# guxm2021/SVT_SpeechBrain

Hardware: AMD Instinct MI355X
Metric: 10s@16kHz clips/sec encoder+CTC forward, wav2vec2-base, 1/2/4/8 MI355X (higher is better)
Workload: dtype bf16; 1 GPU; wav2vec2-base audio-only AMT forward (encoder + 20-way head + frame decode), 32 x 10 s @16 kHz mono clips per GPU; global_batch=32, per_gpu_batch=32, samples_per_clip=160000, frames_per_clip=499, parallelism=clips sharded over 1 rank(s), streams=2, inputs=resident in HBM

## Files before the change

include/svt_mi355.h:

```cpp
#ifndef SVT_MI355_H
#define SVT_MI355_H

#include <stddef.h>
#include <stdint.h>

#ifdef __cplusplus
extern "C" {
#endif

#define SVT_ABI_VERSION 1
#define SVT_MAX_CONV_LAYERS 8

typedef enum {
  SVT_OK = 0,
  SVT_ERR_INVALID = -1,
  SVT_ERR_KEY = -2,
  SVT_ERR_STATE = -3,
  SVT_ERR_WORKSPACE = -4,
  SVT_ERR_HIP = -5,
  SVT_ERR_NO_DEVICE = -6
} svt_status;

typedef enum { SVT_PREC_FP32 = 0, SVT_PREC_BF16 = 1, SVT_PREC_BF16X3 = 2, SVT_PREC_FP16X3 = 3 } svt_precision;
typedef enum { SVT_NORM_GROUP = 0, SVT_NORM_LAYER = 1 } svt_feat_norm;
// ... 90 lines not shown
                          float* out_dev, void* workspace_dev, size_t workspace_bytes, void* stream);
int svt_rca_backward(svt_rca* r, const float* dout_dev, int32_t batch, int32_t t_audio, float* const* grads_dev, void* workspace_dev,
                     size_t workspace_bytes, void* stream);

int svt_ctc_greedy(const float* probs_dev, int32_t batch, int32_t t, int32_t v, const float* rel_lens_dev,
                   int32_t blank, int32_t* tokens_dev, int32_t* out_lens_dev, int device, void* stream);

int64_t svt_fbank_workspace_bytes(int32_t batch, int64_t n_samples, int32_t n_fft, int32_t hop, int32_t n_mels);
int svt_fbank(const float* wav_dev, int32_t batch, int64_t n_samples, int32_t sample_rate, int32_t n_fft,
              int32_t win_length, int32_t hop_length, int32_t n_mels, float f_min, float f_max, float top_db,
              float* out_dev, void* workspace_dev, size_t workspace_bytes, int device, void* stream);

#define SVT_NOISE_AMP_WORKGROUPS 256
#define SVT_NOISE_MIX_MAX_WORKGROUPS 2048
int64_t svt_noise_mix_workspace_bytes(int64_t n_samples, int32_t n_snr);
int svt_noise_mix(const float* clean_dev, const float* noise_dev, int64_t n_samples, const float* snr_db_host, int32_t n_snr,
                  float* out_dev, int64_t ld_out, double* amps_out_dev, void* workspace_dev, int64_t workspace_bytes, int device,
                  void* stream);

#define SVT_RESAMPLE_LDS_BYTES 65536
#define SVT_RESAMPLE_TILE_OUTPUTS 1024
#define SVT_RESAMPLE_MAX_WORKGROUPS 768
int64_t svt_resample_output_samples(int64_t n_in, int32_t orig_freq, int32_t new_freq);
int svt_resample(const float* in_dev, int32_t rows, int64_t n_in, int64_t ld_in, const float* weights_dev, const int32_t* first_dev,
                 int32_t P, int32_t W, int32_t S, float* out_dev, int64_t n_out, int64_t ld_out, int32_t downmix, int device,
                 void* stream);

int svt_debug_gemm(int32_t precision, const void* a_dev, const void* w_dev, void* c_dev, const float* bias_dev,
                   const float* resid_dev, int32_t m, int32_t n, int32_t k, int32_t a_rpb, int64_t a_bstride,
                   int64_t a_rstride, int64_t ldw, int32_t act, int32_t out_f32, int device, void* stream);

int svt_debug_gemm_pairs(int32_t precision, const float* a_dev, int64_t a_elems, const float* w_dev, float* c_dev, const float* bias_dev,
                         int32_t m, int32_t n, int32_t k, int32_t a_rpb, int64_t a_bstride, int64_t a_rstride, int32_t act,
                         int32_t out_kind, int device, void* stream, int32_t time_iters, float* ms_out);

typedef struct svt_debug_gemm_desc {
  int32_t struct_size;
  const void* a;
  const void* w;
  void* c;
  const float* bias;
  const float* resid;
  int32_t m, n, k;
  int32_t a_rpb;
  int64_t a_bstride, a_rstride;
  int64_t ldw, ldc;
  int32_t nz, nz2;
  int64_t a_z1, a_z2, w_z1, w_z2, c_z1, c_z2, bias_z2;
  float alpha;
  int32_t act, out_f32;
} svt_debug_gemm_desc;
int svt_debug_gemm_batched(int32_t precision, const svt_debug_gemm_desc* d, int device, void* stream);

typedef struct svt_debug_layernorm_desc {
  int32_t struct_size;
  int32_t form;
  int32_t prec, x_is_f32;
  int64_t rows;
  int32_t D, gelu;
  float eps;
  int32_t pair_kind;
  const float* gamma;
  const float* beta;
  const void* x;
  void* yT;
  float* yF;
  const float* add;
  float* sumF;
  void* yP;
  const void* addP;
  const void* branch;
  const void* rh;
  const void* rl;
  const float* x32;
  void* yh;
  void* yl;
  const float* parts;
  const float* pbias;
  int64_t part_stride;
  int32_t nparts;
} svt_debug_layernorm_desc;
int svt_debug_layernorm(const svt_debug_layernorm_desc* d, int device, void* stream);

typedef struct svt_video svt_video;
int svt_video_create(int32_t embed_dim, int32_t precision, int device, svt_video** out);
void svt_video_destroy(svt_video* v);
int svt_video_load_param(svt_video* v, const char* key, const void* data_host, int dtype, const int64_t* shape, int ndim);
int svt_video_finalize(svt_video* v);
int64_t svt_video_workspace_bytes(const svt_video* v, int32_t batch, int32_t t, int32_t h, int32_t w);
int svt_video_keep_workspace(svt_video* v, int keep);
int svt_video_forward(svt_video* v, const float* video_dev, int32_t batch, int32_t t, int32_t h, int32_t w, float* out_dev,
                      void* workspace_dev, size_t workspace_bytes, void* stream);
int svt_video_forward_ex(svt_video* v, const float* video_dev, int32_t batch, int32_t t, int32_t h, int32_t w, float* out_dev, int64_t out_ld,
                         int32_t zero_left, void* workspace_dev, size_t workspace_bytes, void* stream);
typedef struct svt_video_transform { double sub0, div0, mean, std; int32_t crop_h, crop_w; } svt_video_transform;
int svt_video_forward_u8(svt_video* v, const uint8_t* roi_dev, int32_t batch, int32_t t, int32_t h_in, int32_t w_in,
                         const svt_video_transform* tf, float* out_dev, int64_t out_ld, int32_t zero_left, void* workspace_dev,
                         size_t workspace_bytes, void* stream);

int svt_deltas(const float* x_dev, int64_t ldx, int32_t batch, int32_t t, int32_t c, int32_t window_length, float* out_dev,
               int64_t ldo, int device, void* stream);
int svt_context_window(const float* x_dev, int32_t batch, int32_t t, int32_t c, int32_t left_frames, int32_t right_frames,
                       float* out_dev, int device, void* stream);

int svt_bce_loss(const float* logits_dev, int64_t batch, int64_t t_pred, const float* targets_dev, int64_t t_tgt,
                 const float* rel_len_dev, const float* pos_weight_dev, int32_t allowed_len_diff, int32_t reduction,
                 float* out_dev, void* workspace_dev, size_t workspace_bytes, int device, void* stream);
int svt_nll_loss(const float* log_probs_dev, int64_t batch, int64_t t_pred, int32_t n_class, const int64_t* targets_dev,
                 int64_t t_tgt, const float* rel_len_dev, float label_smoothing, int32_t allowed_len_diff,
                 int32_t reduction, float* out_dev, void* workspace_dev, size_t workspace_bytes, int device, void* stream);
int svt_softmax(const float* x_dev, int64_t rows, int32_t n, int32_t apply_log, float* y_dev, int device, void* stream);

int svt_amt_objective_grad(const float* logits_dev, int64_t batch, int64_t t_pred, int32_t n_out, int32_t pitch_octave_num,
                           const float* onset_targets_dev, const float* offset_targets_dev, const int64_t* octave_targets_dev,
                           const int64_t* class_targets_dev, int64_t t_tgt, const float* rel_len_dev, float onset_pos_weight,
                           int32_t allowed_len_diff, float label_smoothing, float* terms_dev, float* terms_host, float* dlogits_dev,
                           void* workspace_dev, size_t* workspace_bytes, int device, void* stream);
int svt_linear_backward(const float* x_dev, const float* dy_dev, int64_t rows, int32_t in_features, int32_t out_features,
                        float* dweight_dev, float* dbias_dev, void* workspace_dev, size_t* workspace_bytes, int device, void* stream);
int svt_linear_backward_data(const float* dy_dev, const float* weight_dev, int64_t rows, int32_t in_features, int32_t out_features,
                             float* dx_dev, int device, void* stream);
int svt_clip_adadelta_step(int32_t n_tensors, float* const* params_dev, float* const* grads_dev, float* const* square_avg_dev,
                           float* const* acc_delta_dev, const int64_t* numels, float lr, double rho, float eps, float weight_decay,
                           int32_t maximize, float max_norm, float* total_norm_dev, void* workspace_dev, size_t* workspace_bytes,
                           int device, void* stream);

int svt_debug_attention(int32_t precision, const void* q, const void* k, const void* v, void* o, int32_t batch, int32_t t,
                        int32_t heads, int32_t head_dim, int64_t ldq, int64_t ldkv, int64_t ldo, float scale, int device,
                        void* stream);
int svt_debug_attention_bias(const void* q, const void* k, const void* v, void* o, int32_t batch, int32_t t, int32_t heads, int64_t ldq,
                             int64_t ldkv, int64_t ldo, float scale, const float* gate_dev, const float* pos_bias_dev, int device,
                             void* stream);
int svt_debug_attention_scores(int32_t precision, const void* q, const void* k, const void* v, void* o, int32_t batch, int32_t t,
                               int32_t heads, int32_t head_dim, int64_t ldq, int64_t ldkv, int64_t ldo, float scale,
                               const float* gate_dev, const float* pos_bias_dev, int device, void* stream);
int svt_debug_rca_wgrad(int32_t precision, const float* dy0, int64_t ldy0, const void* x0, const float* dy1, int64_t ldy1, const void* x1,
                        int64_t rows, int32_t n_out, int32_t n_in, float* dw, float* db, void* workspace_dev, size_t* workspace_bytes,
                        int device, void* stream);
int svt_debug_rca_attn_bwd(int32_t precision, const void* qkv, const void* qc, const void* o_self, const void* o_cross,
                           const float* dblend, float alpha, int32_t batch, int32_t t, int32_t heads, int32_t head_dim, float* dqkv,
                           float* dqc, void* workspace_dev, size_t* workspace_bytes, int device, void* stream);
int svt_debug_set(int key, int value);

int svt_prof_enable(int on);
int svt_prof_reset(void);
int svt_prof_read(int kind, int64_t* launches, double* total_ms, double* total_flops, double* total_bytes);
int svt_debug_clock(int64_t* out_dev, int device, void* stream);
int svt_debug_alloc(void** out, size_t bytes, int device);
int svt_debug_encoder_layout(const svt_encoder* e, int32_t batch, int64_t n_samples, int64_t* offsets, int n);
int svt_debug_free(void* p, int device);

#ifdef __cplusplus
}
#endif
#endif
```

svt_speechbrain_amd/_lib.py:

```python
from __future__ import annotations

import ctypes as C
import os
from typing import Optional

_HERE = os.path.dirname(os.path.abspath(__file__))
LIB_PATH = os.environ.get("SVT_LIB_PATH") or os.path.join(_HERE, "libsvt_mi355.so")
MAX_CONV = 8


class SvtError(RuntimeError):
    pass


class EncoderConfigC(C.Structure):
    _fields_ = [
        ("struct_size", C.c_int32),
        ("hidden_size", C.c_int32),
        ("num_layers", C.c_int32),
        ("num_heads", C.c_int32),
        ("intermediate_size", C.c_int32),
        ("num_conv_layers", C.c_int32),
        ("conv_dim", C.c_int32 * MAX_CONV),
        ("conv_kernel", C.c_int32 * MAX_CONV),
# ... 23 lines not shown
    _fields_ = [
        ("struct_size", C.c_int32),
        ("a", C.c_void_p), ("w", C.c_void_p), ("c", C.c_void_p), ("bias", C.c_void_p), ("resid", C.c_void_p),
        ("m", C.c_int32), ("n", C.c_int32), ("k", C.c_int32),
        ("a_rpb", C.c_int32),
        ("a_bstride", C.c_int64), ("a_rstride", C.c_int64),
        ("ldw", C.c_int64), ("ldc", C.c_int64),
        ("nz", C.c_int32), ("nz2", C.c_int32),
        ("a_z1", C.c_int64), ("a_z2", C.c_int64), ("w_z1", C.c_int64), ("w_z2", C.c_int64), ("c_z1", C.c_int64), ("c_z2", C.c_int64),
        ("bias_z2", C.c_int64),
        ("alpha", C.c_float),
        ("act", C.c_int32), ("out_f32", C.c_int32),
    ]


class LayerNormDescC(C.Structure):
    _fields_ = [
        ("struct_size", C.c_int32),
        ("form", C.c_int32),
        ("prec", C.c_int32), ("x_is_f32", C.c_int32),
        ("rows", C.c_int64),
        ("D", C.c_int32), ("gelu", C.c_int32),
        ("eps", C.c_float),
        ("pair_kind", C.c_int32),
        ("gamma", C.c_void_p), ("beta", C.c_void_p),
        ("x", C.c_void_p), ("yT", C.c_void_p), ("yF", C.c_void_p), ("add", C.c_void_p), ("sumF", C.c_void_p), ("yP", C.c_void_p), ("addP", C.c_void_p),
        ("branch", C.c_void_p), ("rh", C.c_void_p), ("rl", C.c_void_p), ("x32", C.c_void_p), ("yh", C.c_void_p), ("yl", C.c_void_p),
        ("parts", C.c_void_p), ("pbias", C.c_void_p),
        ("part_stride", C.c_int64),
        ("nparts", C.c_int32),
    ]


class FrameC(C.Structure):
    _fields_ = [("p_on", C.c_float), ("p_off", C.c_float), ("octave", C.c_int32), ("pitch_class", C.c_int32)]


_P = C.c_void_p
_I64P = C.POINTER(C.c_int64)
NORM_REDUCE_FN = C.CFUNCTYPE(C.c_int, C.c_void_p, C.c_int32, C.c_void_p, C.c_void_p)

SYMBOLS = {
    "svt_last_error": (C.c_char_p, []),
    "svt_abi_version": (C.c_int, []),
    "svt_device_count": (C.c_int, []),
    "svt_encoder_create": (C.c_int, [C.POINTER(EncoderConfigC), C.c_int, C.POINTER(_P)]),
    "svt_encoder_destroy": (None, [_P]),
    "svt_encoder_load_param": (C.c_int, [_P, C.c_char_p, _P, C.c_int, _I64P, C.c_int]),
    "svt_encoder_finalize": (C.c_int, [_P]),
    "svt_encoder_get_param": (C.c_int, [_P, C.c_char_p, _P, C.c_int64]),
    "svt_encoder_num_frames": (C.c_int64, [_P, C.c_int64]),
    "svt_encoder_workspace_bytes": (C.c_int64, [_P, C.c_int32, C.c_int64]),
    "svt_encoder_forward": (C.c_int, [_P, _P, C.c_int32, C.c_int64, _P, _P, C.c_size_t, _P]),
    "svt_encoder_forward_ex": (C.c_int, [_P, _P, C.c_int32, C.c_int64, _P, _P, C.c_size_t, _P, C.c_int32]),
    "svt_encoder_forward_head": (C.c_int, [_P, _P, _P, C.c_int32, C.c_int64, _P, _P, C.c_int32, C.c_int32, _P, C.c_size_t, _P, C.c_int32]),
    "svt_linear_create": (C.c_int, [C.c_int32, C.c_int32, C.c_int, C.c_int, C.POINTER(_P)]),
    "svt_linear_destroy": (None, [_P]),
    "svt_linear_load": (C.c_int, [_P, _P, _P]),
    "svt_linear_forward": (C.c_int, [_P, _P, C.c_int64, _P, _P]),
    "svt_decode_frames": (C.c_int, [_P, C.c_int64, C.c_int32, C.c_int32, C.c_int32, _P, C.c_int, _P]),
    "svt_rca_create": (C.c_int, [C.c_int32, C.c_int32, C.c_int32, C.c_float, C.c_int32, C.c_int32, C.c_int, C.POINTER(_P)]),
    "svt_rca_destroy": (None, [_P]),
    "svt_rca_load_param": (C.c_int, [_P, C.c_char_p, _P, C.c_int, _I64P, C.c_int]),
    "svt_rca_finalize": (C.c_int, [_P]),
    "svt_rca_workspace_bytes": (C.c_int64, [_P, C.c_int32, C.c_int32]),
    "svt_rca_forward": (C.c_int, [_P, _P, C.c_int32, _P, C.c_int32, C.c_int32, _P, _P, C.c_size_t, _P]),
    "svt_rca_refresh_params": (C.c_int, [_P, C.POINTER(_P), C.c_int32, _P]),
    "svt_rca_train_workspace_bytes": (C.c_int64, [_P, C.c_int32, C.c_int32]),
    "svt_rca_forward_train": (C.c_int, [_P, _P, C.c_int32, _P, C.c_int32, C.c_int32, _P, _P, C.c_size_t, _P]),
    "svt_rca_backward": (C.c_int, [_P, _P, C.c_int32, C.c_int32, C.POINTER(_P), _P, C.c_size_t, _P]),
    "svt_ctc_greedy": (C.c_int, [_P, C.c_int32, C.c_int32, C.c_int32, _P, C.c_int32, _P, _P, C.c_int, _P]),
    "svt_fbank_workspace_bytes": (C.c_int64, [C.c_int32, C.c_int64, C.c_int32, C.c_int32, C.c_int32]),
    "svt_fbank": (C.c_int, [_P, C.c_int32, C.c_int64, C.c_int32, C.c_int32, C.c_int32, C.c_int32, C.c_int32,
                            C.c_float, C.c_float, C.c_float, _P, _P, C.c_size_t, C.c_int, _P]),
    "svt_noise_mix_workspace_bytes": (C.c_int64, [C.c_int64, C.c_int32]),
    "svt_noise_mix": (C.c_int, [_P, _P, C.c_int64, C.POINTER(C.c_float), C.c_int32, _P, C.c_int64, _P, _P, C.c_int64, C.c_int, _P]),
    "svt_resample_output_samples": (C.c_int64, [C.c_int64, C.c_int32, C.c_int32]),
    "svt_resample": (C.c_int, [_P, C.c_int32, C.c_int64, C.c_int64, _P, _P, C.c_int32, C.c_int32, C.c_int32, _P, C.c_int64, C.c_int64,
                               C.c_int32, C.c_int, _P]),
    "svt_debug_gemm": (C.c_int, [C.c_int32, _P, _P, _P, _P, _P, C.c_int32, C.c_int32, C.c_int32, C.c_int32, C.c_int64,
                                 C.c_int64, C.c_int64, C.c_int32, C.c_int32, C.c_int, _P]),
    "svt_debug_gemm_batched": (C.c_int, [C.c_int32, C.POINTER(GemmDescC), C.c_int, _P]),
    "svt_debug_layernorm": (C.c_int, [C.POINTER(LayerNormDescC), C.c_int, _P]),
    "svt_debug_attention_scores": (C.c_int, [C.c_int32, _P, _P, _P, _P, C.c_int32, C.c_int32, C.c_int32, C.c_int32, C.c_int64, C.c_int64,
                                             C.c_int64, C.c_float, _P, _P, C.c_int, _P]),
    "svt_debug_gemm_pairs": (C.c_int, [C.c_int32, _P, C.c_int64, _P, _P, _P, C.c_int32, C.c_int32, C.c_int32, C.c_int32, C.c_int64,
                                       C.c_int64, C.c_int32, C.c_int32, C.c_int, _P, C.c_int32, C.POINTER(C.c_float)]),
    "svt_video_create": (C.c_int, [C.c_int32, C.c_int32, C.c_int, C.POINTER(C.c_void_p)]),
    "svt_video_destroy": (None, [C.c_void_p]),
    "svt_video_load_param": (C.c_int, [C.c_void_p, C.c_char_p, C.c_void_p, C.c_int, C.POINTER(C.c_int64), C.c_int]),
    "svt_video_finalize": (C.c_int, [C.c_void_p]),
    "svt_video_keep_workspace": (C.c_int, [C.c_void_p, C.c_int]),
    "svt_video_workspace_bytes": (C.c_int64, [C.c_void_p, C.c_int32, C.c_int32, C.c_int32, C.c_int32]),
    "svt_video_forward": (C.c_int, [C.c_void_p, C.c_void_p, C.c_int32, C.c_int32, C.c_int32, C.c_int32, C.c_void_p, C.c_void_p,
                                    C.c_size_t, C.c_void_p]),
    "svt_video_forward_ex": (C.c_int, [C.c_void_p, C.c_void_p, C.c_int32, C.c_int32, C.c_int32, C.c_int32, C.c_void_p, C.c_int64, C.c_int32,
                                       C.c_void_p, C.c_size_t, C.c_void_p]),
    "svt_video_forward_u8": (C.c_int, [C.c_void_p, C.c_void_p, C.c_int32, C.c_int32, C.c_int32, C.c_int32, C.POINTER(VideoTransformC),
                                       C.c_void_p, C.c_int64, C.c_int32, C.c_void_p, C.c_size_t, C.c_void_p]),
    "svt_deltas": (C.c_int, [C.c_void_p, C.c_int64, C.c_int32, C.c_int32, C.c_int32, C.c_int32, C.c_void_p, C.c_int64, C.c_int, C.c_void_p]),
    "svt_context_window": (C.c_int, [C.c_void_p, C.c_int32, C.c_int32, C.c_int32, C.c_int32, C.c_int32, C.c_void_p, C.c_int, C.c_void_p]),
    "svt_bce_loss": (C.c_int, [C.c_void_p, C.c_int64, C.c_int64, C.c_void_p, C.c_int64, C.c_void_p, C.c_void_p, C.c_int32,
                               C.c_int32, C.c_void_p, C.c_void_p, C.c_size_t, C.c_int, C.c_void_p]),
    "svt_nll_loss": (C.c_int, [C.c_void_p, C.c_int64, C.c_int64, C.c_int32, C.c_void_p, C.c_int64, C.c_void_p, C.c_float,
                               C.c_int32, C.c_int32, C.c_void_p, C.c_void_p, C.c_size_t, C.c_int, C.c_void_p]),
    "svt_softmax": (C.c_int, [C.c_void_p, C.c_int64, C.c_int32, C.c_int32, C.c_void_p, C.c_int, C.c_void_p]),
    "svt_amt_objective_grad": (C.c_int, [_P, C.c_int64, C.c_int64, C.c_int32, C.c_int32, _P, _P, _P, _P, C.c_int64, _P, C.c_float,
                                         C.c_int32, C.c_float, _P, C.POINTER(C.c_float), _P, _P, C.POINTER(C.c_size_t), C.c_int, _P]),
    "svt_linear_backward": (C.c_int, [_P, _P, C.c_int64, C.c_int32, C.c_int32, _P, _P, _P, C.POINTER(C.c_size_t), C.c_int, _P]),
    "svt_linear_backward_data": (C.c_int, [_P, _P, C.c_int64, C.c_int32, C.c_int32, _P, C.c_int, _P]),
    "svt_clip_adadelta_step": (C.c_int, [C.c_int32, C.POINTER(_P), C.POINTER(_P), C.POINTER(_P), C.POINTER(_P), _I64P, C.c_float,
                                         C.c_double, C.c_float, C.c_float, C.c_int32, C.c_float, _P, _P, C.POINTER(C.c_size_t), C.c_int,
                                         _P]),
    "svt_debug_attention": (C.c_int, [C.c_int32, C.c_void_p, C.c_void_p, C.c_void_p, C.c_void_p, C.c_int32, C.c_int32,
                                      C.c_int32, C.c_int32, C.c_int64, C.c_int64, C.c_int64, C.c_float, C.c_int, C.c_void_p]),
    "svt_debug_attention_bias": (C.c_int, [C.c_void_p, C.c_void_p, C.c_void_p, C.c_void_p, C.c_int32, C.c_int32, C.c_int32, C.c_int64,
                                           C.c_int64, C.c_int64, C.c_float, C.c_void_p, C.c_void_p, C.c_int, C.c_void_p]),
    "svt_debug_rca_wgrad": (C.c_int, [C.c_int32, _P, C.c_int64, _P, _P, C.c_int64, _P, C.c_int64, C.c_int32, C.c_int32, _P, _P, _P,
                                      C.POINTER(C.c_size_t), C.c_int, _P]),
    "svt_debug_rca_attn_bwd": (C.c_int, [C.c_int32, _P, _P, _P, _P, _P, C.c_float, C.c_int32, C.c_int32, C.c_int32, C.c_int32, _P, _P,
                                         _P, C.POINTER(C.c_size_t), C.c_int, _P]),
    "svt_debug_set": (C.c_int, [C.c_int, C.c_int]),
    "svt_debug_clock": (C.c_int, [C.c_void_p, C.c_int, C.c_void_p]),
    "svt_debug_encoder_layout": (C.c_int, [C.c_void_p, C.c_int32, C.c_int64, C.POINTER(C.c_int64), C.c_int]),
    "svt_operand_type": (C.c_int, []),
    "svt_encoder_set_norm_reduce": (C.c_int, [_P, C.c_void_p, C.c_void_p, C.c_int64]),
    "svt_frames_to_notes": (C.c_int, [C.c_void_p, C.c_int32, C.c_int64, C.c_void_p, C.c_float, C.c_float, C.c_double, C.c_int32, C.c_int32,
                                      C.c_void_p, C.c_void_p, C.c_void_p, C.c_void_p, C.c_void_p, C.c_int64, C.c_void_p]),
    "svt_debug_alloc": (C.c_int, [C.POINTER(C.c_void_p), C.c_size_t, C.c_int]),
    "svt_debug_free": (C.c_int, [C.c_void_p, C.c_int]),
    "svt_prof_enable": (C.c_int, [C.c_int]),
    "svt_prof_reset": (C.c_int, []),
    "svt_prof_read": (C.c_int, [C.c_int, _I64P, C.POINTER(C.c_double), C.POINTER(C.c_double), C.POINTER(C.c_double)]),
}

_lib: Optional[C.CDLL] = None
_libs: dict = {}


def load(variant: str = None) -> C.CDLL:
    global _lib
    key = variant or ""
    if key in _libs:
        return _libs[key]
    if not variant and os.environ.get("SVT_LIB_SUFFIX"):
        variant_path = LIB_PATH.replace("libsvt_mi355.so", f"libsvt_mi355_{os.environ['SVT_LIB_SUFFIX']}.so")
        if not os.path.exists(variant_path):
            raise SvtError(f"SVT_LIB_SUFFIX: {variant_path} not found")
        globals()["LIB_PATH"] = variant_path
    root, ext = os.path.splitext(LIB_PATH)
    path = LIB_PATH if not variant else f"{root}_{variant}{ext}"
    if not os.path.exists(path):
        raise SvtError(
            f"{path} not found: build it with `python -c 'import __graft_entry__ as g; g.build()'` "
            "(or `make -C svt_speechbrain_amd/csrc`). The MI355X path has no CPU fallback.")
    lib = C.CDLL(path)
    for name, (res, args) in SYMBOLS.items():
        fn = getattr(lib, name)
        fn.restype = res
        fn.argtypes = args
    if lib.svt_abi_version() != 1:
        raise SvtError(f"{os.path.basename(path)} ABI version mismatch")
    if lib.svt_operand_type() != (1 if variant == "f16" else 0):
        raise SvtError(f"{os.path.basename(path)} was built for another operand type")
    _libs[key] = lib
    if not variant:
# ... 35 lines not shown
```

svt_speechbrain_amd/csrc/api.hip:

```cpp
#include "../../include/svt_mi355.h"
#include "api.h"
#include "common.h"
#include "host.h"

#include <atomic>
#include <cmath>
#include <cstring>
#include <map>
#include <mutex>
#include <string>
#include <vector>

namespace svt {

int hip_fail(hipError_t e, const char* what, const char* file, int line) {
  set_error(std::string("HIP error ") + hipGetErrorName(e) + " (" + hipGetErrorString(e) + ") at " + file + ":" +
          std::to_string(line) + " in " + what);
  return SVT_ERR_HIP;
}

struct ProfState {
  bool on = false;
  int every = 1;
  unsigned tick = 0;
// ... 253 lines not shown
int svt_operand_type(void) {
#ifdef SVT_OPERAND_F16
  return 1;
#else
  return 0;
#endif
}
int svt_device_count(void) {
  int n = 0;
  if (hipGetDeviceCount(&n) != hipSuccess) return 0;
  int ok = 0;
  for (int i = 0; i < n; ++i) {
    hipDeviceProp_t prop;
    if (hipGetDeviceProperties(&prop, i) == hipSuccess && std::string(prop.gcnArchName).find("gfx950") != std::string::npos) ++ok;
  }
  return ok;
}

int svt_debug_gemm(int32_t precision, const void* a, const void* w, void* c, const float* bias, const float* resid,
                   int32_t m, int32_t n, int32_t k, int32_t a_rpb, int64_t a_bstride, int64_t a_rstride, int64_t ldw,
                   int32_t act, int32_t out_f32, int device, void* stream) {
  if (!a || !w || !c) { set_error("svt_debug_gemm: null argument"); return SVT_ERR_INVALID; }
  SVT_HIP(hipSetDevice(device));
  GemmArgs g;
  g.A = a; g.W = w; g.C = c; g.bias = bias; g.resid = resid;
  g.M = m; g.N = n; g.K = k; g.a_rpb = a_rpb; g.a_bstride = a_bstride; g.a_rstride = a_rstride;
  g.ldw = ldw; g.ldc = n; g.act = act; g.out_f32 = out_f32;
  static const void* s_kept = nullptr;
  const bool split = precision >= 2 && ldw == k && k % 32 == 0;
  if (split && !(g_debug_keep_split && s_kept == w)) {
    if (split_weights_register(w, n, k, precision, (hipStream_t)stream)) return SVT_ERR_HIP;
    s_kept = w;
  }
  const int rc = launch_gemm(precision, g, (hipStream_t)stream);
  if (split && !g_debug_keep_split) {
    SVT_HIP(hipStreamSynchronize((hipStream_t)stream));
    split_weights_forget(w);
    s_kept = nullptr;
  }
  return rc ? SVT_ERR_INVALID : SVT_OK;
}

int svt_debug_gemm_batched(int32_t precision, const svt_debug_gemm_desc* d, int device, void* stream) {
  if (!d || d->struct_size != (int32_t)sizeof(svt_debug_gemm_desc)) { set_error("svt_debug_gemm_batched: struct_size"); return SVT_ERR_INVALID; }
  if (!d->a || !d->w || !d->c) { set_error("svt_debug_gemm_batched: null argument"); return SVT_ERR_INVALID; }
  if (!valid_precision(precision)) { set_error("svt_debug_gemm_batched: precision"); return SVT_ERR_INVALID; }
  if (d->nz < 1 || d->nz2 < 1 || d->k < 1) { set_error("svt_debug_gemm_batched: nz, nz2 and k must be positive"); return SVT_ERR_INVALID; }
  SVT_HIP(hipSetDevice(device));
  GemmArgs g;
  g.A = d->a; g.W = d->w; g.C = d->c; g.bias = d->bias; g.resid = d->resid;
  g.M = d->m; g.N = d->n; g.K = d->k; g.a_rpb = d->a_rpb; g.a_bstride = d->a_bstride; g.a_rstride = d->a_rstride;
  g.ldw = d->ldw; g.ldc = d->ldc;
  g.nz = d->nz; g.nz2 = d->nz2;
  g.a_z1 = d->a_z1; g.a_z2 = d->a_z2; g.w_z1 = d->w_z1; g.w_z2 = d->w_z2; g.c_z1 = d->c_z1; g.c_z2 = d->c_z2; g.bias_z2 = d->bias_z2;
  g.alpha = d->alpha; g.act = d->act; g.out_f32 = d->out_f32;
  const bool split = precision >= 2 && d->ldw == d->k && d->k % 32 == 0 && d->w_z1 >= 0 && d->w_z2 >= 0;
  if (split) {
    const size_t last_z_row = d->nz > 1 ? ((size_t)(d->nz / d->nz2 - 1) * d->w_z1 + (size_t)(d->nz2 - 1) * d->w_z2) / (size_t)d->k : 0;
    if (split_weights_register(d->w, (long)last_z_row + d->n, d->k, precision, (hipStream_t)stream)) return SVT_ERR_HIP;
  }
  const int rc = launch_gemm(precision, g, (hipStream_t)stream);
  if (split) {
    SVT_HIP(hipStreamSynchronize((hipStream_t)stream));
    split_weights_forget(d->w);
  }
  return rc ? SVT_ERR_INVALID : SVT_OK;
}

int svt_debug_layernorm(const svt_debug_layernorm_desc* d, int device, void* stream) {
  auto refuse = [](const char* why) { set_error(std::string("svt_debug_layernorm: ") + why); return SVT_ERR_INVALID; };
  auto aligned = [](unsigned mask, auto... p) { return !((... | (uintptr_t)p) & mask); };
  if (!d || d->struct_size != (int32_t)sizeof(svt_debug_layernorm_desc)) return refuse("struct_size");
  if (d->form < 0 || d->form > 2) return refuse("form is 0, 1 or 2");
  if (d->rows < 1 || d->D < 1) return refuse("rows and D must be positive");
  if (!d->gamma || !d->beta) return refuse("null gamma / beta");
  const bool hilo_width = d->D == 512 || d->D == 768 || d->D == 1024;
  if (d->form == 0) {
    if (!d->x) return refuse("null x");
    if (!d->prec && !d->x_is_f32) return refuse("a 16-bit x needs prec 1");
    if (!aligned(15, d->gamma, d->beta, d->x, d->yT, d->yF, d->add, d->sumF) || !aligned(127, d->yP, d->addP))
      return refuse("every buffer 16-byte aligned, yP / addP 128-byte aligned");
  } else {
    if (!hilo_width) return refuse("the (hi, lo) forms need D in {512, 768, 1024}");
    if (!d->yh || !d->yl) return refuse("null yh / yl");
    if (!aligned(15, d->gamma, d->beta, d->branch, d->rh, d->rl, d->x32, d->yh, d->yl, d->yF, d->parts, d->pbias))
      return refuse("every buffer 16-byte aligned");
    if (d->form == 1 && !(d->x32 ? !d->rh && !d->rl : d->rh && d->rl)) return refuse("form 1 takes exactly one of x32 and (rh, rl)");
    if (d->form == 2 && (!d->rh || !d->rl)) return refuse("form 2 needs rh and rl");
    if (d->form == 2 && (d->nparts < 1 || (d->nparts > 1 && d->part_stride < d->rows * d->D))) return refuse("nparts >= 1, parts rows * D elements apart or more");
  }
  if (int r = check_device(device)) return r;
  SVT_HIP(hipSetDevice(device));
  hipStream_t s = (hipStream_t)stream;
  int rc;
  if (d->form == 0) {
    LnArgs a;
    a.prec = d->prec; a.x = d->x; a.x_is_f32 = d->x_is_f32; a.rows = d->rows; a.D = d->D; a.gamma = d->gamma; a.beta = d->beta;
    a.eps = d->eps; a.gelu = d->gelu; a.yT = d->yT; a.yF = d->yF; a.add = d->add; a.sumF = d->sumF; a.yP = d->yP;
    a.pair_kind = d->pair_kind; a.addP = d->addP;
    rc = launch_layernorm(a, s);
  } else if (d->form == 1) {
    rc = launch_layernorm_hilo((const bf16_t*)d->branch, (const bf16_t*)d->rh, (const bf16_t*)d->rl, d->x32, d->rows, d->D, d->gamma,
                               d->beta, d->eps, (bf16_t*)d->yh, (bf16_t*)d->yl, d->yF, s);
  } else {
    rc = launch_layernorm_hilo_parts(d->parts, d->nparts, (long)d->part_stride, d->pbias, (const bf16_t*)d->rh, (const bf16_t*)d->rl,
                                     d->rows, d->D, d->gamma, d->beta, d->eps, (bf16_t*)d->yh, (bf16_t*)d->yl, d->yF, s);
  }
  return rc ? SVT_ERR_INVALID : SVT_OK;
}

int svt_debug_gemm_pairs(int32_t precision, const float* a, int64_t a_elems, const float* w, float* c, const float* bias, int32_t m,
                         int32_t n, int32_t k, int32_t a_rpb, int64_t a_bstride, int64_t a_rstride, int32_t act, int32_t out_kind,
                         int device, void* stream, int32_t time_iters, float* ms_out) {
  if (!a || !w || !c) { set_error("svt_debug_gemm_pairs: null argument"); return SVT_ERR_INVALID; }
  if ((precision != SVT_PREC_BF16X3 && precision != SVT_PREC_FP16X3) || !valid_precision(precision)) {
    set_error("svt_debug_gemm_pairs: split-operand precisions only (they live in libsvt_mi355.so, not in the IEEE-half build)"); return SVT_ERR_INVALID; }
  if (out_kind < 0 || out_kind > 2 || a_elems % 32 || ((int64_t)m * n) % 32) { set_error("svt_debug_gemm_pairs: out_kind / sizes"); return SVT_ERR_INVALID; }
  SVT_HIP(hipSetDevice(device));
  hipStream_t s = (hipStream_t)stream;
  void *ap = nullptr, *cp = nullptr;
  hipEvent_t e0 = nullptr, e1 = nullptr;
  static std::mutex s_mu;
  static const void* s_kept = nullptr;
  std::lock_guard<std::mutex> lock(s_mu);
  bool registered = false;
  auto hip_ok = [](hipError_t e, const char* what) -> int {
    if (e == hipSuccess) return 0;
    set_error(std::string(what) + ": " + hipGetErrorString(e));
    return 1;
  };
  int rc = dev_alloc(&ap, (size_t)a_elems * 4);
  if (!rc && out_kind) rc = dev_alloc(&cp, (size_t)m * n * 4);
  if (!rc) rc = launch_f32_to_pairs(precision, a, ap, a_elems, s);
  if (!rc && !(g_debug_keep_split && s_kept == w)) {
    rc = split_weights_register(w, n, k, precision, s);
    if (!rc) { s_kept = w; registered = true; }
  } else if (!rc) {
    registered = true;
  }
  if (!rc) {
    GemmArgs g;
    g.A = ap; g.W = w; g.C = out_kind == 1 ? cp : (void*)c; g.bias = bias;
    g.M = m; g.N = n; g.K = k; g.a_rpb = a_rpb; g.a_bstride = a_bstride; g.a_rstride = a_rstride;
    g.ldw = k; g.ldc = n; g.act = act; g.out_f32 = 1; g.a_pairs = 1; g.c_pairs = out_kind == 1;
    if (out_kind == 2) { g.planes = (unsigned short*)cp; g.plane_stride = (long)m * n; }
    rc = launch_gemm(precision, g, s);
    if (!rc && time_iters > 0 && ms_out) {
      rc = hip_ok(hipEventCreate(&e0), "hipEventCreate") || hip_ok(hipEventCreate(&e1), "hipEventCreate") ||
           hip_ok(hipEventRecord(e0, s), "hipEventRecord");
      for (int i = 0; i < time_iters && !rc; ++i) rc = launch_gemm(precision, g, s);
      float ms = 0.f;
      if (!rc) rc = hip_ok(hipEventRecord(e1, s), "hipEventRecord") || hip_ok(hipEventSynchronize(e1), "hipEventSynchronize") ||
                    hip_ok(hipEventElapsedTime(&ms, e0, e1), "hipEventElapsedTime");
      if (!rc) *ms_out = ms / (float)time_iters;
    }
  }
  if (!rc && out_kind == 1) rc = launch_pairs_to_f32(precision, cp, nullptr, c, (int64_t)m * n, s);
  if (!rc && out_kind == 2) rc = launch_pairs_to_f32(precision, cp, (const unsigned short*)cp + (size_t)m * n, c, (int64_t)m * n, s);
  (void)hipStreamSynchronize(s);
  if (e0) (void)hipEventDestroy(e0);
  if (e1) (void)hipEventDestroy(e1);
  if (registered && !g_debug_keep_split) { split_weights_forget(w); s_kept = nullptr; }
  if (ap) dev_free(ap);
  if (cp) dev_free(cp);
  return rc ? SVT_ERR_INVALID : SVT_OK;
}

int svt_debug_attention(int32_t precision, const void* q, const void* k, const void* v, void* o, int32_t batch, int32_t t,
                        int32_t heads, int32_t head_dim, int64_t ldq, int64_t ldkv, int64_t ldo, float scale, int device,
                        void* stream) {
  if (!q || !k || !v || !o) { set_error("svt_debug_attention: null argument"); return SVT_ERR_INVALID; }
  if (!(precision >= 1 && precision <= 3) || !(head_dim == 64 || head_dim == 128)) {
    set_error("svt_debug_attention: only the fused kernels (bf16, or the split-operand modes on fp32 inputs; head_dim 64 / 128) are exposed"); return SVT_ERR_INVALID; }
  if (int r = check_device(device)) return r;
  SVT_HIP(hipSetDevice(device));
  if (precision >= 2) {
    const long D = (long)heads * head_dim, rows = (long)batch * t;
    if ((const float*)k != (const float*)q + D || (const float*)v != (const float*)q + 2 * D || ldq != 3 * D || ldkv != 3 * D) {
      set_error("svt_debug_attention: the split-operand kernel is exposed for a packed q|k|v projection"); return SVT_ERR_INVALID; }
    void* planes = nullptr;
    if (int r = dev_alloc(&planes, (size_t)rows * 3 * D * 4)) return r;
    AttnBufs ab{};
    ab.pl_qkv = planes;
    const int rc = attention_scores_path(0, q, ldq, k, v, ldkv, batch, t, heads, head_dim, scale, ab, false, o, ldo, (hipStream_t)stream,
                                         nullptr, nullptr, precision);
    (void)hipStreamSynchronize((hipStream_t)stream);
    dev_free(planes);
    return rc ? SVT_ERR_INVALID : SVT_OK;
  }
  if (launch_flash_attention(q, ldq, (long)t * ldq, k, v, ldkv, (long)t * ldkv, o, ldo, (long)t * ldo, batch, t, heads,
                             head_dim, scale, (hipStream_t)stream)) return SVT_ERR_INVALID;
// ... 13 lines not shown
}

int svt_debug_attention_scores(int32_t precision, const void* q, const void* k, const void* v, void* o, int32_t batch, int32_t t,
                               int32_t heads, int32_t head_dim, int64_t ldq, int64_t ldkv, int64_t ldo, float scale,
                               const float* gate_dev, const float* pos_bias_dev, int device, void* stream) {
  if (!q || !k || !v || !o) { set_error("svt_debug_attention_scores: null argument"); return SVT_ERR_INVALID; }
  if (!valid_precision(precision)) { set_error("svt_debug_attention_scores: precision"); return SVT_ERR_INVALID; }
  if (batch < 1 || t < 1 || heads < 1 || head_dim < 1) { set_error("svt_debug_attention_scores: batch, t, heads and head_dim must be positive"); return SVT_ERR_INVALID; }
  if (!gate_dev != !pos_bias_dev) { set_error("svt_debug_attention_scores: gate and pos_bias come together"); return SVT_ERR_INVALID; }
  if (use_flash(precision, head_dim, gate_dev != nullptr, t)) {
    set_error("svt_debug_attention_scores: this geometry runs the fused kernel (svt_debug_attention / svt_debug_attention_bias)"); return SVT_ERR_INVALID; }
  if (int r = check_device(device)) return r;
  SVT_HIP(hipSetDevice(device));
  hipStream_t s = (hipStream_t)stream;
  const int prec = storage_prec(precision);
  const int Tp = attn_tp(precision, head_dim, t, gate_dev != nullptr);
  const size_t bh = (size_t)batch * heads;
  const size_t bytes[3] = {bh * t * Tp * 4, bh * t * Tp * esize(prec), bh * head_dim * Tp * esize(prec)};
  void* buf[3] = {nullptr, nullptr, nullptr};
  int rc = 0;
  for (int i = 0; i < 3 && !rc; ++i) {
    rc = dev_alloc(&buf[i], bytes[i]);
    if (!rc && hipMemsetAsync(buf[i], 0xFF, bytes[i], s) != hipSuccess) { set_error("svt_debug_attention_scores: hipMemsetAsync"); rc = SVT_ERR_HIP; }
  }
  if (!rc) {
    AttnBufs ab{};
    ab.S = (float*)buf[0]; ab.P = buf[1]; ab.Vt = buf[2];
    rc = attention_scores_path(prec, q, ldq, k, v, ldkv, batch, t, heads, head_dim, scale, ab, false, o, ldo, s, gate_dev, pos_bias_dev,
                               precision) ? SVT_ERR_INVALID : SVT_OK;
  }
  (void)hipStreamSynchronize(s);
  for (int i = 0; i < 3; ++i) dev_free(buf[i]);
  return rc;
}

int svt_debug_set(int key, int value) {
  if (key == 0) g_gemm_dbg = value;
  else if (key == 1) g_gemm_force_bm = value;
  else if (key == 2) g_gemm_ring = value;
  else if (key == 3) g_gemm_variant = value;
  else if (key == 5) {  }
  else if (key == 6) g_gemm_skinny = value;
  else if (key == 7) g_gemm_skinny_max_tiles = value;
  else if (key == 8) g_flash_wide = value;
  else if (key == 9) g_conv_ln_bf16 = value;
  else if (key == 10) {  }
  else if (key == 11) g_gemm_x3 = value;
  else if (key == 12) g_debug_keep_split = value;
  else if (key == 13) g_guard_alloc = value;
  else if (key == 15) g_stamp_ends = value;
  else if (key == 16) {  }
  else if (key == 18) {  }
  else if (key == 19) g_x3_pairs = value;
  else if (key == 20) g_ln_two_rows = value;
  else if (key == 21) {
    if (value != 0 && value != 3) { set_error("svt_debug_set(21): the attention A/B arms are retired"); return SVT_ERR_INVALID; }
  }
  else if (key == 22) g_conv0_mfma = value;
  else if (key == 23) g_conv3x3_c64 = value;
  else if (key == 24) return g_conv3x3_c64_launches;
  else if (key == 25) g_conv3x3_c64_form = value;
  else if (key == 26) g_stem_pool_fused = value;
  else if (key == 27) g_conv_down_fused = value;
  else if (key == 28) {
    if (value != 0) { set_error("svt_debug_set(28): the two-slot schedule is retired"); return SVT_ERR_INVALID; }
  }
  else if (key == 29) g_gemm_p1w = value;
  else if (key == 30) {
#ifndef SVT_DIAG
    if (value != 0) { set_error("svt_debug_set(30): gemm_p1x_kernel is built by `make DIAG=1` only"); return SVT_ERR_INVALID; }
#endif
    g_gemm_p1x = value;
  }
  else if (key == 31) return g_dev_frees.load(std::memory_order_relaxed);
  else if (key == 32) return set_ticket_fenced(value);
  else if (key == 33) g_gemm_skinny_small_tiles = value;
  else if (key == 34) g_gemm_walk = value;
  else if (key == 35) g_conv_kperm = value;
  else if (key == 36) g_ffn2_ksplit = value;
  else if (key == 37) { if (value < 8 || value > 256 || value % 8) { set_error("svt_debug_set(37): 8 .. 256, a multiple of 8"); return SVT_ERR_INVALID; } g_gemm_persist_wgs = value; }
  else if (key == 38) return g_flash_kernel_id;
  else if (key == 39) return g_gemm_kernel_id;
  else if (key == 40) return g_ln_kernel_id;
  else { set_error("svt_debug_set: unknown key"); return SVT_ERR_INVALID; }
  return SVT_OK;
}

int svt_debug_alloc(void** out, size_t bytes, int device) {
  if (!out) { set_error("svt_debug_alloc: null argument"); return SVT_ERR_INVALID; }
  if (int r = check_device(device)) return r;
  SVT_HIP(hipSetDevice(device));
  return dev_alloc(out, bytes);
}
int svt_debug_free(void* p, int device) {
  if (int r = check_device(device)) return r;
  SVT_HIP(hipSetDevice(device));
  dev_free(p);
  return SVT_OK;
}

int svt_debug_clock(int64_t* out_dev, int device, void* stream) {
  if (!out_dev) { set_error("svt_debug_clock: null argument"); return SVT_ERR_INVALID; }
  SVT_HIP(hipSetDevice(device));
  return launch_clock_stamp((long long*)out_dev, (hipStream_t)stream) ? SVT_ERR_HIP : SVT_OK;
}

int svt_prof_enable(int on) { g_prof.on = on != 0; g_prof.every = on > 1 ? on : 1; g_prof.tick = 0; return SVT_OK; }
int svt_prof_reset(void) {
  g_prof.used = 0;
  for (int k = 0; k < 3; ++k) g_prof.flops[k] = g_prof.bytes[k] = 0;
  return SVT_OK;
}
int svt_prof_read(int kind, int64_t* launches, double* total_ms, double* total_flops, double* total_bytes) {
  if (kind < 0 || kind > 2) { set_error("svt_prof_read: kind must be 0..2"); return SVT_ERR_INVALID; }
  double ms = 0;
  int64_t n = 0;
  for (size_t i = 0; i < g_prof.used; ++i) {
    if (g_prof.kind[i] != kind) continue;
    SVT_HIP(hipEventSynchronize(g_prof.ev[i].second));
    float t = 0;
    SVT_HIP(hipEventElapsedTime(&t, g_prof.ev[i].first, g_prof.ev[i].second));
    ms += t;
    ++n;
  }
  if (launches) *launches = n;
  if (total_ms) *total_ms = ms;
  if (total_flops) *total_flops = g_prof.flops[kind];
  if (total_bytes) *total_bytes = g_prof.bytes[kind];
  return SVT_OK;
}

}
```

svt_speechbrain_amd/csrc/api_encoder.hip:

```cpp
#include "../../include/svt_mi355.h"
#include "api.h"
#include "common.h"
#include "host.h"

#include <cmath>
#include <cstring>
#include <string>
#include <vector>

using namespace svt;

int svt::g_conv_ln_bf16 = 1;

struct ConvLayerW {
  DevBuf w;
  DevBuf w_kperm;
  DevBuf bias;
  DevBuf gamma, beta;
};
struct EncLayerW {
  DevBuf wqkv, bqkv, wo, bo, ln1g, ln1b, w1, b1, w2, b2, ln2g, ln2b;
  DevBuf g_wab, g_bab, g_const;
};

struct svt_encoder {
  svt_encoder_config cfg;
  int device = 0;
  bool finalized = false;
  bool uploaded = false;
  ParamMap params;
  std::vector<ConvLayerW> conv;
  DevBuf fp_g, fp_b, proj_w, proj_b, pos_w, pos_b, enc_g, enc_b;
  DevBuf pos_bn_sc, pos_bn_sh;
  DevBuf pos_wP, pos_bP;
  int pos_P = 0;
  std::vector<DevBuf> pos_ws, pos_bs;
  DevBuf rel_embed;
  DevBuf ones, zeros;
  std::vector<EncLayerW> layers;
  svt_norm_reduce_fn reduce_fn = nullptr;
  void* reduce_user = nullptr;
  int64_t reduce_global_clips = 0;
};

static bool reduced_mode(const svt_encoder_config& c) { return c.precision != SVT_PREC_FP32; }

static int64_t conv_frames(const svt_encoder_config& c, int64_t n_samples, int64_t* frames = nullptr) {
  int64_t t = n_samples;
  for (int i = 0; i < c.num_conv_layers; ++i) {
    if (t < c.conv_kernel[i]) return 0;
    t = (t - c.conv_kernel[i]) / c.conv_stride[i] + 1;
    if (frames) frames[i] = t;
  }
  return t;
}

namespace {

int finalize_conv_stack(svt_encoder* e) {
  const svt_encoder_config& c = e->cfg;
  const ParamMap& P = e->params;
  if ((int)e->conv.size() != c.num_conv_layers) { e->conv.clear(); e->conv.resize(c.num_conv_layers); }
  int cin = 1;
  for (int i = 0; i < c.num_conv_layers; ++i) {
    const std::string pre = "feature_extractor.conv_layers." + std::to_string(i) + ".";
    const int co = c.conv_dim[i], k = c.conv_kernel[i];
    const Param* p = nullptr;
    if (int r = need(P, pre + "conv.weight", {co, cin, k}, &p)) return r;
    ConvLayerW& L = e->conv[i];
    if (i == 0) {
      if (int r = upload_f32(L.w, p->v.data(), p->v.size())) return r;
    } else {
      const std::vector<float> wt = tap_major(p->v.data(), co, cin, k);
      if (int r = upload_weight(c.precision, L.w, wt.data(), (size_t)co, (size_t)k * cin)) return r;
      if (storage_prec(c.precision) && k == 3 && cin % 64 == 0 && c.conv_stride[i] == 2) {
        const std::vector<float> wp = tap_minor_slabs(wt.data(), co, cin, k);
        if (int r = upload_weight(c.precision, L.w_kperm, wp.data(), (size_t)co, (size_t)k * cin)) return r;
      } else L.w_kperm.release();
    }
    if (c.conv_bias)
      if (int r = upload_vec(P, pre + "conv.bias", co, &L.bias)) return r;
    if (c.feat_extract_norm == SVT_NORM_LAYER || i == 0) {
      if (int r = upload_vec(P, pre + "layer_norm.weight", co, &L.gamma)) return r;
      if (int r = upload_vec(P, pre + "layer_norm.bias", co, &L.beta)) return r;
    }
    cin = co;
  }
  return SVT_OK;
}

int finalize_projection(svt_encoder* e) {
  const svt_encoder_config& c = e->cfg;
  const ParamMap& P = e->params;
  const int cin = c.conv_dim[c.num_conv_layers > 0 ? c.num_conv_layers - 1 : 0];
  if (c.feat_proj_layer_norm) {
// ... 300 lines not shown
  }
  if (c.num_conv_layers == 0) max_act = rows * c.conv_dim[0] * es;
  w.act[0] = cv.take(max_act);
  w.act[1] = cv.take(max_act);
  w.convF = c.feat_extract_norm == SVT_NORM_LAYER ? (float*)cv.take(max_f) : nullptr;
  w.xln = cv.take(rows * p.C * es);
  w.hF = (float*)cv.take(rows * D * 4);
  w.preF = (float*)cv.take(rows * D * 4);
  w.xb = cv.take(rows * D * es);
  w.xF = p.reduced ? (float*)cv.take(rows * D * 4) : (float*)w.xb;
  w.xlo = p.sp ? cv.take(rows * D * 2) : nullptr;
  w.posg = cv.take(B * p.pos_Tp * D * es);
  w.posy = p.Pf ? cv.take(B * p.pos_Tq * p.Pf * D * es) : nullptr;
  w.qkv = cv.take(rows * 3 * D * es);
  const bool scores = !(p.flash || p.planes);
  w.ab.S = scores ? (float*)cv.take(B * H * T * p.attn_Tp * 4) : nullptr;
  w.ab.P = scores ? cv.take(B * H * T * p.attn_Tp * es) : nullptr;
  w.ab.Vt = cv.take(B * H * p.dh * p.attn_Tp * es);
  w.ab.pl_qkv = p.planes ? cv.take(rows * 3 * D * 4) : nullptr;
  w.attn_o = cv.take(rows * D * es);
  w.ffn = cv.take(rows * p.F * es);
  w.gate = p.rel ? (float*)cv.take(B * H * T * 4) : nullptr;
  w.relpb = p.rel ? (float*)cv.take(H * (2 * T - 1) * 4) : nullptr;
  w.dots = (float*)cv.take(rows * 32 * 4);
  w.ksplit = p.ksplit_ws ? (float*)cv.take((size_t)4 * rows * D * 4) : nullptr;
  w.total = cv.off;
  return w;
}

struct TailSpec {
  float* feats = nullptr;
  const svt_linear* head = nullptr;
  float* logits = nullptr;
  svt_frame* frames = nullptr;
  int n_oct = 0, n_cls = 0;
};

}

extern "C" {

int svt_debug_encoder_layout(const svt_encoder* e, int32_t batch, int64_t n_samples, int64_t* offsets, int n) {
  if (!e || batch < 1 || !offsets || n < 1) { set_error("svt_debug_encoder_layout: bad argument"); return SVT_ERR_INVALID; }
  EncPlan p;
  if (!plan_encoder(e, batch, n_samples, &p)) { set_error("waveform shorter than the receptive field"); return SVT_ERR_INVALID; }
  char* const fake = (char*)(uintptr_t)(1ull << 40);
  const EncWs w = carve_encoder(e, p, fake);
  const void* r[24] = {w.mom, w.coef, w.c0tab, w.act[0], w.act[1], w.convF, w.xln, w.hF, w.preF, w.xb, w.xF, w.xlo, w.posg, w.posy, w.qkv,
                       w.ab.S, w.ab.P, w.ab.Vt, w.ab.pl_qkv, w.attn_o, w.ffn, w.gate, w.relpb, w.dots};
  int k = 0;
  for (; k < 24 && k < n; ++k) offsets[k] = r[k] == nullptr ? -1 : (int64_t)((const char*)r[k] - fake);
  if (k < n) offsets[k++] = (int64_t)w.total;
  return k;
}

int64_t svt_encoder_workspace_bytes(const svt_encoder* e, int32_t batch, int64_t n_samples) {
  if (!e || batch < 1) { set_error("workspace_bytes: bad argument"); return -1; }
  EncPlan p;
  if (!plan_encoder(e, batch, n_samples, &p)) { set_error("waveform shorter than the receptive field"); return -1; }
  return (int64_t)carve_encoder(e, p, nullptr).total;
}

}

namespace {

struct ReduceCtx { const svt_encoder* e; double* mom; hipStream_t s; };
int reduce_now(void* a) {
  ReduceCtx* rc = (ReduceCtx*)a;
  if (rc->e->reduce_fn(rc->mom, 2, (void*)rc->s, rc->e->reduce_user)) { set_error("encoder_forward: the norm-reduce callback reported an error"); return SVT_ERR_INVALID; }
  return 0;
}

struct EncRun {
  const svt_encoder* e;
  const svt_encoder_config& c;
  const EncPlan& p;
  EncWs w;
  hipStream_t s;
  int cpg = 0, groups = 1;
  double* wav_mom = nullptr;
  double* out_mom = nullptr;
  double* win_mom = nullptr;
  int64_t n_wav = 0;
  bool global_norm = false;
  ReduceCtx rctx{nullptr, nullptr, nullptr};
  int pk_front = 0, pk_enc = 0;
  float* resid = nullptr;
};

LnArgs ln_f32(const EncRun& x, const void* in, int64_t rows, int D, const DevBuf& gamma, const DevBuf& beta, float eps) {
  LnArgs a;
  a.prec = x.p.sp; a.x = in; a.rows = rows; a.D = D; a.gamma = gamma.as<float>(); a.beta = beta.as<float>(); a.eps = eps;
  return a;
}

int check_norm_groups(EncRun& x, int32_t clips_per_norm_group) {
  const svt_encoder_config& c = x.c;
  x.cpg = clips_per_norm_group > 0 ? clips_per_norm_group : x.p.B;
  if (x.p.B % x.cpg) { set_error("encoder_forward: batch must be a multiple of clips_per_norm_group"); return SVT_ERR_INVALID; }
  x.groups = x.p.B / x.cpg;
  if (x.groups > 1 && c.num_conv_layers > 0 && (x.p.L & 3)) {
    set_error("encoder_forward: norm groups need a waveform length that is a multiple of 4 samples");
    return SVT_ERR_INVALID;
  }
  if (x.groups > 1 && c.num_conv_layers == 0 && c.normalize_wav) {
    set_error("encoder_forward: features-in mode has no input norm to group");
    return SVT_ERR_INVALID;
  }
  return SVT_OK;
}

int input_statistics(EncRun& x, const float* wav) {
  const svt_encoder_config& c = x.c;
  const EncWs& w = x.w;
  const size_t B = (size_t)x.p.B;
  if (launch_zero_bytes(w.mom, w.mom_zero, x.s)) return SVT_ERR_HIP;
  x.wav_mom = c.normalize_wav ? w.mom : nullptr;
  x.out_mom = w.mom + 2 * B;
  x.win_mom = w.mom + 4 * B;
  x.n_wav = (int64_t)x.cpg * x.p.L;
  if (c.normalize_wav)
    if (int r = launch_moments(wav, x.n_wav, x.wav_mom, (char*)w.mom + w.mom_scr[0], x.p.B, x.s, x.groups)) return r;
  x.rctx = ReduceCtx{x.e, nullptr, x.s};
  x.global_norm = x.e->reduce_fn != nullptr;
  if (x.global_norm) {
    if (x.groups != 1) { set_error("encoder_forward: the cross-rank norm reduction applies to whole-batch norms (clips_per_norm_group = 0)"); return SVT_ERR_INVALID; }
    if (x.e->reduce_global_clips < x.p.B) { set_error("encoder_forward: global_clips of the norm reduction is smaller than this batch"); return SVT_ERR_INVALID; }
    if (c.normalize_wav) {
      x.rctx.mom = x.wav_mom;
      if (int r = reduce_now(&x.rctx)) return r;
      x.n_wav = x.e->reduce_global_clips * x.p.L;
    }
  }
  return SVT_OK;
}

bool x3q_fits(const void* A, int M, int N, int K, int a_rpb, long a_bstride, long a_rstride, const void* Wp, int c_pairs, long ldc) {
  GemmArgs g;
  g.A = A; g.W = Wp; g.C = const_cast<void*>(A); g.M = M; g.N = N; g.K = K; g.a_rpb = a_rpb; g.a_bstride = a_bstride; g.a_rstride = a_rstride;
  g.ldw = K; g.ldc = ldc; g.a_pairs = 1; g.c_pairs = c_pairs;
  return gemm_x3q_eligible(g);
}

void choose_pair_rows(EncRun& x) {
  const svt_encoder_config& c = x.c;
  const EncPlan& p = x.p;
  const EncWs& w = x.w;
  const svt_encoder* e = x.e;
  const int B = p.B, D = p.D, F = p.F, rows = (int)p.rows;
  const int pk_mode = (p.gp >= 2 && g_x3_pairs && g_gemm_x3) ? p.gp : 0;
  bool front = pk_mode != 0 && c.num_conv_layers >= 2 && c.conv_dim[0] % 32 == 0 && c.conv_dim[0] <= 512 && c.conv_stride[0] <= 5;
  for (int i = 1; i < c.num_conv_layers && front; ++i) {
    const int cin = c.conv_dim[i - 1], co = c.conv_dim[i], k = c.conv_kernel[i], st = c.conv_stride[i];
    const int64_t ti = p.frames[i - 1], to = p.frames[i];
    front = (int64_t)B * to <= 2147483647LL &&
            x3q_fits(w.act[0], (int)((int64_t)B * to), co, k * cin, (int)to, ti * cin, (long)st * cin, e->conv[i].w.p, 1, co) &&
            (c.feat_extract_norm != SVT_NORM_LAYER || co == 512 || co == 768 || co == 1024);
  }
  front = front && x3q_fits(w.xln, rows, D, p.C, rows, 0, p.C, e->proj_w.p, 0, D) &&
          (!c.feat_proj_layer_norm || p.C == 512 || p.C == 768 || p.C == 1024);
  x.pk_front = front ? pk_mode : 0;
  const bool enc = pk_mode != 0 && p.planes && c.num_layers > 0 && (D == 512 || D == 768 || D == 1024) && p.dh % 32 == 0 &&
                   x3q_fits(w.xb, rows, 3 * D, D, rows, 0, D, e->layers[0].wqkv.p, 0, 3 * D) &&
                   x3q_fits(w.attn_o, rows, D, D, rows, 0, D, e->layers[0].wo.p, 0, D) &&
                   x3q_fits(w.xb, rows, F, D, rows, 0, D, e->layers[0].w1.p, 1, F) &&
                   x3q_fits(w.ffn, rows, D, F, rows, 0, F, e->layers[0].w2.p, 0, D);
  x.pk_enc = enc ? pk_mode : 0;
  x.resid = (!p.sp && !x.pk_enc) ? (float*)w.xb : w.xF;
}

int conv_layer0(const EncRun& x, const float* wav) {
  const svt_encoder_config& c = x.c;
  const EncWs& w = x.w;
  const int B = x.p.B, k = c.conv_kernel[0], st = c.conv_stride[0], C0 = c.conv_dim[0], prec = x.p.sp;
  const int64_t L = x.p.L, t1 = x.p.t1;
  const ConvLayerW& c0 = x.e->conv[0];
  const float* b0 = c.conv_bias ? c0.bias.as<float>() : nullptr;
  const bool mfma = conv0_mfma_ok(prec, x.pk_front, k, st, C0) && w.c0tab;
  if (c.feat_extract_norm == SVT_NORM_GROUP) {
    if (int r = launch_conv0_window_moments(wav, B, L, k, st, t1, x.win_mom, (char*)w.mom + w.mom_scr[2], x.s)) return r;
    if (int r = launch_conv0_group_coef(x.wav_mom, x.n_wav, x.win_mom, B, t1, C0, k, c0.w.as<float>(), b0, c0.gamma.as<float>(),
                                        c0.beta.as<float>(), 1e-5f, 1e-5f, w.coef, x.s, x.cpg)) return r;
    if (mfma) return launch_conv0_mfma_group(wav, B, L, st, t1, w.coef, w.c0tab, w.act[0], x.s, x.pk_front);
    return launch_conv0_group_apply(prec, wav, B, L, k, st, t1, C0, w.coef, w.act[0], x.s, x.pk_front);
  }
  if (mfma)
    return launch_conv0_mfma_layer(wav, B, L, st, t1, x.wav_mom, x.n_wav, 1e-5f, c0.w.as<float>(), b0, c0.gamma.as<float>(),
                                   c0.beta.as<float>(), 1e-5f, w.c0tab, w.act[0], x.s, x.cpg, x.pk_front);
  return launch_conv0_layer(prec, wav, B, L, k, st, t1, C0, x.wav_mom, x.n_wav, 1e-5f, c0.w.as<float>(), b0, c0.gamma.as<float>(),
                            c0.beta.as<float>(), 1e-5f, w.act[0], x.s, x.cpg, x.pk_front);
}

int conv_stack(const EncRun& x, int* cur_out) {
  const svt_encoder_config& c = x.c;
  const EncWs& w = x.w;
  const int prec = x.p.sp, gp = x.p.gp, pk = x.pk_front;
  const bool layer_norm = c.feat_extract_norm == SVT_NORM_LAYER;
  int cur = 0;
  for (int i = 1; i < c.num_conv_layers; ++i) {
    const int cin = c.conv_dim[i - 1], co = c.conv_dim[i], k = c.conv_kernel[i], st = c.conv_stride[i];
    const int64_t tin = x.p.frames[i - 1], tout = x.p.frames[i], rows = (int64_t)x.p.B * tout;
    const ConvLayerW& Lw = x.e->conv[i];
    void* const out = w.act[cur ^ 1];
    if (rows > 2147483647LL) { set_error("encoder_forward: batch*frames exceeds 2^31"); return SVT_ERR_INVALID; }
    GemmArgs g;
    g.A = w.act[cur]; g.W = Lw.w.p;
    g.M = (int)rows; g.N = co; g.K = k * cin;
    g.a_rpb = (int)tout; g.a_bstride = tin * cin; g.a_rstride = (long)st * cin;
    g.ldw = g.K; g.ldc = co;
    if (Lw.w_kperm.p) { g.W_kperm = Lw.w_kperm.p; g.kperm_taps = k; g.kperm_cin = cin; }
    g.bias = c.conv_bias ? Lw.bias.as<float>() : nullptr;
    g.a_pairs = pk ? 1 : 0;
    const bool pairs_out = pk && !(i + 1 == c.num_conv_layers && c.feat_proj_layer_norm);
    LnArgs n = ln_f32(x, w.convF, rows, co, Lw.gamma, Lw.beta, 1e-5f);
    n.gelu = 1;
    if (pk && layer_norm) {
      g.C = w.convF; g.out_f32 = 1; g.act = ACT_NONE;
      if (int r = launch_gemm(gp, g, x.s)) return r;
      (pairs_out ? n.yP : n.yT) = out; n.pair_kind = pk;
      if (int r = launch_layernorm(n, x.s)) return r;
    } else if (pk) {
      g.C = out; g.act = ACT_GELU; g.out_f32 = 1; g.c_pairs = pairs_out ? 1 : 0;
      if (int r = launch_gemm(gp, g, x.s)) return r;
    } else if (layer_norm && prec && co == 512 && g_conv_ln_bf16) {
      g.C = out; g.out_f32 = 0; g.act = ACT_NONE;
      if (int r = launch_gemm(gp, g, x.s)) return r;
      n.x = out; n.x_is_f32 = 0; n.yT = out;
      if (int r = launch_layernorm(n, x.s)) return r;
    } else if (layer_norm) {
      g.C = w.convF; g.out_f32 = 1; g.act = ACT_NONE;
      if (int r = launch_gemm(gp, g, x.s)) return r;
      n.yT = out;
      if (int r = launch_layernorm(n, x.s)) return r;
    } else {
      g.C = out; g.act = ACT_GELU;
      if (int r = launch_gemm(gp, g, x.s)) return r;
    }
    cur ^= 1;
  }
  *cur_out = cur;
  return SVT_OK;
}

int feature_projection(const EncRun& x, int cur) {
  const svt_encoder_config& c = x.c;
  const EncWs& w = x.w;
  const int C = x.p.C, D = x.p.D, rows = (int)x.p.rows, pk = x.pk_front;
  const void* proj_in = w.act[cur];
  if (c.feat_proj_layer_norm) {
    LnArgs n = ln_f32(x, w.act[cur], rows, C, x.e->fp_g, x.e->fp_b, c.layer_norm_eps);
    n.x_is_f32 = x.p.sp ? 0 : 1;
    (pk ? n.yP : n.yT) = w.xln; n.pair_kind = pk;
    if (int r = launch_layernorm(n, x.s)) return r;
    proj_in = w.xln;
  }
  GemmArgs g;
  g.A = proj_in; g.W = x.e->proj_w.p; g.C = w.hF; g.bias = x.e->proj_b.as<float>();
  g.M = rows; g.N = D; g.K = C; g.a_rpb = rows; g.a_rstride = C; g.ldw = C; g.ldc = D; g.out_f32 = 1;
  g.a_pairs = pk ? 1 : 0;
  return launch_gemm(x.p.gp, g, x.s);
}

GemmArgs posconv_gemm(const EncRun& x, const DevBuf& W, const DevBuf& bias) {
  const int T = (int)x.p.T, D = x.p.D, G = x.c.pos_conv_groups, cg = D / G, kp = x.c.pos_conv_kernel;
  GemmArgs g;
  g.A = x.w.posg; g.W = W.p; g.C = x.w.preF; g.bias = bias.as<float>();
  g.M = T; g.N = cg; g.K = kp * cg;
  g.a_rpb = T; g.a_rstride = cg;
  g.ldw = g.K; g.ldc = D;
  g.nz = x.p.B * G; g.nz2 = G;
  g.a_z1 = (long)G * (T + kp) * cg; g.a_z2 = (long)(T + kp) * cg;
  g.w_z1 = 0; g.w_z2 = (long)cg * g.K;
  g.c_z1 = (long)T * D; g.c_z2 = cg; g.bias_z2 = cg;
  g.out_f32 = 1;
  return g;
}

int positional_conv(const EncRun& x) {
  const svt_encoder_config& c = x.c;
  const svt_encoder* e = x.e;
  const EncWs& w = x.w;
  const int prec = x.p.sp, gp = x.p.gp, B = x.p.B, T = (int)x.p.T, D = x.p.D, kp = c.pos_conv_kernel, G = c.pos_conv_groups, cg = D / G;
  const float* bn_sc = c.pos_conv_batch_norm ? e->pos_bn_sc.as<float>() : nullptr;
  const float* bn_sh = c.pos_conv_batch_norm ? e->pos_bn_sh.as<float>() : nullptr;
  if (c.pos_conv_depth > 1) {
    const float* cur = w.hF;
    float* lnout = w.xF;
    for (int i = 0; i < c.pos_conv_depth; ++i) {
      if (int r = launch_posconv_gather(prec, cur, B, T, D, G, kp, T + kp, w.posg, x.s)) return r;
      GemmArgs g = posconv_gemm(x, e->pos_ws[i], e->pos_bs[i]);
      g.act = ACT_NONE;
      if (int r = launch_gemm(gp, g, x.s)) return r;
      LnArgs n = ln_f32(x, w.preF, x.p.rows, D, e->ones, e->zeros, 1e-5f);
      n.gelu = 1; n.yF = lnout;
      if (int r = launch_layernorm(n, x.s)) return r;
      cur = lnout;
    }
    return launch_add_f32(w.hF, cur, w.preF, x.p.rows * (int64_t)D, x.s);
  }
  if (x.p.pos_multi) {
    const int Pf = x.p.Pf, Tq = (int)x.p.pos_Tq, Tp = (int)x.p.pos_Tp;
    if (int r = launch_posconv_gather(prec, w.hF, B, T, D, G, kp, Tp, w.posg, x.s, bn_sc, bn_sh)) return r;
    GemmArgs g;
    g.A = w.posg; g.W = e->pos_wP.p; g.C = w.posy; g.bias = e->pos_bP.as<float>();
    g.M = B * Tq; g.N = Pf * cg; g.K = (kp + Pf - 1) * cg;
    g.a_rpb = Tq; g.a_bstride = (long)G * Tp * cg; g.a_rstride = (long)Pf * cg;
    g.ldw = g.K; g.ldc = g.N;
    g.nz = G; g.nz2 = G;
    g.a_z2 = (long)Tp * cg; g.w_z2 = (long)g.N * g.K; g.c_z2 = (long)B * Tq * g.N; g.bias_z2 = g.N;
    g.act = ACT_GELU; g.out_f32 = 0;
    if (int r = launch_gemm(gp, g, x.s)) return r;
    return launch_posconv_scatter_add(w.hF, w.posy, B, T, D, G, Pf, Tq, w.preF, x.s, prec ? 0 : 1);
  }
  if (int r = launch_posconv_gather(prec, w.hF, B, T, D, G, kp, T + kp, w.posg, x.s, bn_sc, bn_sh)) return r;
  GemmArgs g = posconv_gemm(x, e->pos_w, e->pos_b);
  g.resid = w.hF; g.act = ACT_GELU;
  return launch_gemm(gp, g, x.s);
}

struct LayerForm {
  int branch_f32 = 1;
  int ffn1_f32 = 0;
  int ffn1_pairs = 0;
  bool ffn2_ksplit = false;
};

int rows_gemm(const EncRun& x, const void* A, int K, const DevBuf& W, const DevBuf& bias, int N, void* Cout, int out_f32, int act,
              unsigned short* planes = nullptr, int c_pairs = 0) {
  const int rows = (int)x.p.rows;
  GemmArgs g;
  g.A = A; g.W = W.p; g.C = Cout; g.bias = bias.as<float>();
  g.M = rows; g.N = N; g.K = K; g.a_rpb = rows; g.a_rstride = K; g.ldw = K; g.ldc = N;
  g.out_f32 = out_f32; g.act = act;
  g.planes = planes; g.plane_stride = (long)rows * N;
  g.a_pairs = x.pk_enc ? 1 : 0; g.c_pairs = c_pairs;
  return launch_gemm(x.p.gp, g, x.s);
}

int attention_block(const EncRun& x, const EncLayerW& Lw, const LayerForm& f) {
  const EncPlan& p = x.p;
  const EncWs& w = x.w;
  const int D = p.D;
  if (int r = rows_gemm(x, w.xb, D, Lw.wqkv, Lw.bqkv, 3 * D, w.qkv, 0, ACT_NONE, p.planes ? (unsigned short*)w.ab.pl_qkv : nullptr)) return r;
  const float* gate = nullptr;
  if (p.rel) {
    if (int r = launch_relpos_gate(p.sp, w.xb, p.rows, (int)p.T, p.H, p.dh, Lw.g_wab.as<float>(), Lw.g_bab.as<float>(),
                                   Lw.g_const.as<float>(), w.gate, x.s)) return r;
    gate = w.gate;
  }
  if (int r = attention_scores_path(p.sp, w.qkv, 3L * D, (const char*)w.qkv + (size_t)D * esize(p.sp),
                                    (const char*)w.qkv + (size_t)2 * D * esize(p.sp), 3L * D, p.B, (int)p.T, p.H, p.dh,
                                    1.0f / std::sqrt((float)p.dh), w.ab, p.planes, w.attn_o, D, x.s, gate, w.relpb, p.gp, x.pk_enc ? 1 : 0)) return r;
  return rows_gemm(x, w.attn_o, D, Lw.wo, Lw.bo, D, w.hF, f.branch_f32, ACT_NONE);
}

int ffn_block(const EncRun& x, const EncLayerW& Lw, const LayerForm& f) {
  const EncWs& w = x.w;
  const int D = x.p.D, F = x.p.F, rows = (int)x.p.rows;
  if (int r = rows_gemm(x, w.xb, D, Lw.w1, Lw.b1, F, w.ffn, f.ffn1_f32, ACT_GELU, nullptr, f.ffn1_pairs)) return r;
  if (!f.ffn2_ksplit) return rows_gemm(x, w.ffn, F, Lw.w2, Lw.b2, D, w.hF, f.branch_f32, ACT_NONE);
  GemmArgs g;
  g.A = w.ffn; g.W = Lw.w2.p; g.C = w.ksplit; g.M = rows; g.N = D; g.K = F; g.a_rpb = rows; g.a_rstride = F; g.ldw = F; g.ldc = D;
  g.out_f32 = 1; g.ksplit = 4; g.ksplit_stride = (long)rows * D;
  return launch_gemm_skinny(g, x.s);
}

template <class Ln0, class Ln>
int post_ln_layers(const EncRun& x, const LayerForm& f, Ln0&& ln0, Ln&& ln) {
  if (int r = ln0()) return r;
  for (int l = 0; l < x.c.num_layers; ++l) {
    const EncLayerW& Lw = x.e->layers[l];
    if (int r = attention_block(x, Lw, f)) return r;
    if (int r = ln(Lw, false, false)) return r;
    if (int r = ffn_block(x, Lw, f)) return r;
    if (int r = ln(Lw, true, l + 1 == x.c.num_layers)) return r;
  }
  return SVT_OK;
}

bool ffn2_ksplit_ok(const EncRun& x) {
  const int D = x.p.D, F = x.p.F, rows = (int)x.p.rows;
  if (!(g_ffn2_ksplit && x.w.ksplit && x.p.gp == 1 && F % 256 == 0 && F >= 2048 && g_ln_two_rows)) return false;
  GemmArgs g;
  g.A = x.w.ffn; g.W = x.e->layers[0].w2.p; g.C = x.w.hF; g.M = rows; g.N = D; g.K = F; g.a_rpb = rows; g.a_rstride = F; g.ldw = F; g.ldc = D;
  return g_gemm_skinny && gemm_skinny_eligible(g) && (long)((x.p.rows + 31) / 32) * (D / 32) <= 256;
}

int post_ln_hilo(const EncRun& x) {
  const EncWs& w = x.w;
  const int64_t rows = x.p.rows;
  const int D = x.p.D;
  const float eps = x.c.layer_norm_eps;
  bf16_t* const xh = (bf16_t*)w.xb;
  bf16_t* const xl = (bf16_t*)w.xlo;
  LayerForm f;
  f.branch_f32 = 0;
  f.ffn2_ksplit = ffn2_ksplit_ok(x);
  return post_ln_layers(x, f,
    [&] { return launch_layernorm_hilo(nullptr, nullptr, nullptr, w.preF, rows, D, x.e->enc_g.as<float>(), x.e->enc_b.as<float>(), eps, xh, xl, nullptr, x.s); },
    [&](const EncLayerW& Lw, bool second, bool last) {
      const float *g = (second ? Lw.ln2g : Lw.ln1g).as<float>(), *b = (second ? Lw.ln2b : Lw.ln1b).as<float>();
      float* const yF = last ? x.resid : nullptr;
      if (second && f.ffn2_ksplit)
        return launch_layernorm_hilo_parts(w.ksplit, 4, (long)rows * D, Lw.b2.as<float>(), xh, xl, rows, D, g, b, eps, xh, xl, yF, x.s);
      return launch_layernorm_hilo((const bf16_t*)w.hF, xh, xl, nullptr, rows, D, g, b, eps, xh, xl, yF, x.s);
    });
}

int post_ln_pairs(const EncRun& x) {
  const EncWs& w = x.w;
  const bool pair_resid = x.pk_enc == 3;
  LayerForm f;
  f.branch_f32 = 1; f.ffn1_f32 = 1; f.ffn1_pairs = 1;
  return post_ln_layers(x, f,
    [&] {
      LnArgs n = ln_f32(x, w.preF, x.p.rows, x.p.D, x.e->enc_g, x.e->enc_b, x.c.layer_norm_eps);
      n.yP = w.xb; n.pair_kind = x.pk_enc; n.yF = pair_resid ? nullptr : x.resid;
      return launch_layernorm(n, x.s);
    },
    [&](const EncLayerW& Lw, bool second, bool last) {
      LnArgs n = ln_f32(x, w.hF, x.p.rows, x.p.D, second ? Lw.ln2g : Lw.ln1g, second ? Lw.ln2b : Lw.ln1b, x.c.layer_norm_eps);
      n.yP = w.xb; n.pair_kind = x.pk_enc;
      if (pair_resid) { n.addP = w.xb; n.yF = last ? x.resid : nullptr; }
      else { n.add = x.resid; n.yF = x.resid; }
      return launch_layernorm(n, x.s);
    });
}

int post_ln_plain(const EncRun& x, int branch_f32) {
  const EncWs& w = x.w;
  LayerForm f;
  f.branch_f32 = branch_f32;
  auto out = [&](LnArgs n) { n.yT = w.xb; n.yF = x.p.sp ? x.resid : nullptr; return launch_layernorm(n, x.s); };
  return post_ln_layers(x, f,
    [&] { return out(ln_f32(x, w.preF, x.p.rows, x.p.D, x.e->enc_g, x.e->enc_b, x.c.layer_norm_eps)); },
    [&](const EncLayerW& Lw, bool second, bool) {
      LnArgs n = ln_f32(x, w.hF, x.p.rows, x.p.D, second ? Lw.ln2g : Lw.ln1g, second ? Lw.ln2b : Lw.ln1b, x.c.layer_norm_eps);
      n.x_is_f32 = branch_f32; n.add = x.resid;
      return out(n);
    });
}

int pre_ln_layers(const EncRun& x, int branch_f32, float** final_x) {
  const EncWs& w = x.w;
  float* const h = w.preF;
  LayerForm f;
  f.branch_f32 = branch_f32; f.ffn1_pairs = x.pk_enc ? 1 : 0;
  auto ln_add = [&](const DevBuf& g_, const DevBuf& b_, const void* branch, void* y_op, float* y_f32) -> int {
    LnArgs n = ln_f32(x, h, x.p.rows, x.p.D, g_, b_, x.c.layer_norm_eps);
    n.sumF = (branch && y_op) ? h : nullptr;
    if (x.pk_enc && y_op) {
      n.add = (const float*)branch; n.yP = y_op; n.pair_kind = x.pk_enc;
    } else if (!branch) {
      n.yT = y_op; n.yF = y_f32;
    } else if (!branch_f32) {
      n.x = branch; n.x_is_f32 = 0; n.add = h; n.yT = y_op; n.yF = y_f32;
    } else {
      n.add = (const float*)branch;
      if (y_op) n.yT = y_op; else { n.prec = 0; n.yT = y_f32; }
    }
    return launch_layernorm(n, x.s);
  };
  const void* pending = nullptr;
  for (int l = 0; l < x.c.num_layers; ++l) {
    const EncLayerW& Lw = x.e->layers[l];
    if (int r = ln_add(Lw.ln1g, Lw.ln1b, pending, w.xb, nullptr)) return r;
    if (int r = attention_block(x, Lw, f)) return r;
    if (int r = ln_add(Lw.ln2g, Lw.ln2b, w.hF, w.xb, nullptr)) return r;
    if (int r = ffn_block(x, Lw, f)) return r;
    pending = w.hF;
  }
  *final_x = (float*)w.qkv;
  return ln_add(x.e->enc_g, x.e->enc_b, pending, nullptr, *final_x);
}

int encoder_layers(const EncRun& x, float** final_x) {
  const EncPlan& p = x.p;
  if (p.rel)
    if (int r = launch_relpos_table(x.e->rel_embed.as<float>(), p.H, (int)p.T, x.c.rel_pos_buckets, x.c.rel_pos_max_distance, x.w.relpb, x.s)) return r;
  const bool vecD = (p.D == 512 || p.D == 768 || p.D == 1024);
  const int branch_f32 = (p.sp && vecD) ? 0 : 1;
  if (x.c.stable_layer_norm) return pre_ln_layers(x, branch_f32, final_x);
  *final_x = x.resid;
  if (p.hilo) return post_ln_hilo(x);
  if (x.pk_enc) return post_ln_pairs(x);
  return post_ln_plain(x, branch_f32);
}

// ... 87 lines not shown
```

svt_speechbrain_amd/csrc/common.h:

```cpp
#pragma once
#include <hip/hip_runtime.h>
#include <stdint.h>
#include <string>

typedef __bf16 real_bf16x8 __attribute__((ext_vector_type(8)));
#ifdef SVT_OPERAND_F16
typedef _Float16 bf16_t;
#define SVT_MFMA_16x16x32(a, b, c) __builtin_amdgcn_mfma_f32_16x16x32_f16(a, b, c, 0, 0, 0)
#define SVT_MFMA_32x32x16(a, b, c) __builtin_amdgcn_mfma_f32_32x32x16_f16(a, b, c, 0, 0, 0)
#else
typedef __bf16 bf16_t;
#define SVT_MFMA_16x16x32(a, b, c) __builtin_amdgcn_mfma_f32_16x16x32_bf16(a, b, c, 0, 0, 0)
#define SVT_MFMA_32x32x16(a, b, c) __builtin_amdgcn_mfma_f32_32x32x16_bf16(a, b, c, 0, 0, 0)
#endif
typedef bf16_t bf16x8 __attribute__((ext_vector_type(8)));
typedef bf16_t bf16x4 __attribute__((ext_vector_type(4)));
typedef float f32x4 __attribute__((ext_vector_type(4)));

namespace svt {

#if defined(__HIPCC__)
__device__ __forceinline__ float gelu_fast(float x) {
  const float z = fabsf(x) * 0.70710678118654752440f;
  const float t = __builtin_amdgcn_rcpf(fmaf(0.3275911f, z, 1.0f));
// ... 161 lines not shown
  long a_e1 = 0, a_e2 = 0;
  int kseg = 0;
  long kseg_stride = 0;
  int c_d1 = 1, c_d2 = 1;
  long c_e1 = 0, c_e2 = 0, c_base = 0;
  int c_nsplit = 0;
  long c_nstride = 0;
  const float* slope = nullptr;
  int resid_first = 0;
  int resid_op_type = 0;
  unsigned short* planes = nullptr;
  long plane_stride = 0;
  int planes_f16 = 0;
  int a_pairs = 0;
  int c_pairs = 0;
  int stamp_ends = 0;
  long long* trace = nullptr;
};

int launch_gemm(int prec, const GemmArgs& a, hipStream_t s);
int launch_gemm_skinny(const GemmArgs& a, hipStream_t s);

bool gemm_dma_eligible(const GemmArgs& a);
bool gemm_pps_eligible(const GemmArgs& a);
int launch_gemm_pps(const GemmArgs& a, int bm, hipStream_t s);
int launch_gemm_p1w(const GemmArgs& a, int bm, hipStream_t s);
bool gemm_skinny_eligible(const GemmArgs& a);
int split_weights_register(const void* w_f32_dev, long n_rows, int K, int kind, hipStream_t s);
void split_weights_forget(const void* w_f32_dev);
bool gemm_x3p_eligible(const GemmArgs& a);
int launch_gemm_x3p(int kind, const GemmArgs& a, const void* packed, hipStream_t s);
bool gemm_x3q_eligible(const GemmArgs& a);
int launch_gemm_x3q(int kind, const GemmArgs& a, const void* packed, int bm, hipStream_t s);
int launch_gemm_p1x(int kind, const GemmArgs& a, const void* packed, int bm, hipStream_t s);
#pragma GCC visibility push(hidden)
int launch_gemm_staged(int prec, const GemmArgs& a, int bn, hipStream_t s);
int launch_gemm_pp8(const GemmArgs& a, int bm, int bn, hipStream_t s);
int launch_gemm_pers(const GemmArgs& a, int bm, hipStream_t s);
int launch_gemm_skinny_tile(const GemmArgs& a, int tile, hipStream_t s);
const void* split_weights_find(const void* W, int kind, int K, long rows_needed);
int launch_gemm_x3s(int kind, const GemmArgs& a, const void* packed, int nbs, int form, hipStream_t s);
inline bool tile_span_fits(const GemmArgs& a) {
  const unsigned long clips = 255 / (unsigned long)(a.a_rpb > 0 ? a.a_rpb : 1) + 1;
  const unsigned long bs = (unsigned long)(a.a_bstride > 0 ? a.a_bstride : 0), rs = (unsigned long)(a.a_rstride > 0 ? a.a_rstride : 0);
  return a.a_bstride >= 0 && a.a_rstride > 0 && (clips * bs + 256ul * rs + (unsigned long)a.K) * 4 < 0xF0000000ul &&
         (unsigned long)a.N * a.K * 4 < 0xF0000000ul;
}
inline int persistent_blocks(int ntiles, int cap) { return ntiles < cap ? ((ntiles + 7) / 8) * 8 : cap; }
#pragma GCC visibility pop

__device__ __forceinline__ void tile_walk(int logical, int tiles_m, int tiles_n, int pm, int& tile_m, int& tile_n) {
  if (pm <= 0) { tile_n = logical % tiles_n; tile_m = logical / tiles_n; return; }
  const int per_panel = pm * tiles_n;
  const int pnl = logical / per_panel, rem = logical - pnl * per_panel;
  const int rows = min(pm, tiles_m - pnl * pm);
  tile_n = rem / rows;
  tile_m = pnl * pm + (rem - tile_n * rows);
}

extern int g_gemm_dbg;
extern int g_gemm_force_bm;
extern int g_gemm_ring;
extern int g_gemm_variant;
extern int g_gemm_skinny;
extern int g_gemm_skinny_max_tiles;
extern int g_gemm_x3;
extern int g_stamp_ends;
extern int g_x3_pairs;
extern int g_gemm_p1w;
extern int g_gemm_p1x;
extern int g_gemm_skinny_small_tiles;
extern int g_gemm_walk;
extern int g_conv_kperm;
extern int g_gemm_persist_wgs;
extern int g_gemm_kernel_id;

extern int g_ln_two_rows;
extern int g_ln_kernel_id;
extern int g_flash_wide;
extern int g_flash_kernel_id;
extern int g_ffn2_ksplit;
#pragma GCC visibility push(hidden)
extern int g_conv_ln_bf16;
extern int g_debug_keep_split;
extern int g_conv_down_fused;
#pragma GCC visibility pop

int ensure_dyn_lds(const void* kernel, int bytes);

int dev_alloc(void** out, size_t bytes);
void dev_free(void* p);
extern int g_guard_alloc;

void prof_begin(hipStream_t s);
void prof_end(hipStream_t s, double flops, double bytes, int kind = 1);

int set_ticket_fenced(int on);
int launch_moments(const float* x, int64_t n, double* moments, void* scratch, int groups_max, hipStream_t s, int groups = 1);
size_t moments_scratch_bytes(int groups_max);
int launch_global_norm(const float* x, float* y, int64_t n, const double* moments, float eps, hipStream_t s, int groups = 1,
                       double n_stat = 0);
int launch_conv0_window_moments(const float* wav, int B, int64_t L, int k, int stride, int64_t T1,
                                double* wm , void* scratch , hipStream_t s);
size_t conv0_window_moments_scratch_bytes(int B, int64_t T1);
int launch_conv0_group_coef(const double* wav_moments , int64_t n_wav, const double* wm, int B,
                            int64_t T1, int C, int k, const float* w0 , const float* b0 ,
                            const float* gamma, const float* beta, float eps_wav, float eps_gn,
                            float* coef , hipStream_t s, int clips_per_norm_group);
struct FrameOut { float p_on, p_off; int32_t octave, pitch_class; };
int launch_head_fused(const float* x, int64_t rows, int K, const float* w, const float* wsum, const float* b, int N, float* dots,
                      double* mom, int64_t rows_per_group, float eps, float* logits, FrameOut* frames, int n_oct, int n_cls,
                      hipStream_t s,
                      double n_stat = 0, int (*between)(void*) = nullptr, void* between_arg = nullptr, void* scratch = nullptr);
size_t head_scratch_bytes(int64_t rows, int groups_max);

struct LnArgs {
  int prec = 0;
  const void* x = nullptr;
  int x_is_f32 = 1;
  int64_t rows = 0;
  int D = 0;
  const float* gamma = nullptr;
  const float* beta = nullptr;
  float eps = 1e-5f;
  int gelu = 0;
  void* yT = nullptr;
  float* yF = nullptr;
  const float* add = nullptr;
  float* sumF = nullptr;
  void* yP = nullptr;
  int pair_kind = 0;
  const void* addP = nullptr;
};
int launch_layernorm(const LnArgs& a, hipStream_t s);
bool layernorm_hilo_ok(int D);
int launch_layernorm_hilo_parts(const float* parts, int nparts, long part_stride, const float* pbias, const bf16_t* rh, const bf16_t* rl, int64_t rows,
                                int D, const float* gamma, const float* beta, float eps, bf16_t* yh, bf16_t* yl, float* yF, hipStream_t s);
int launch_layernorm_hilo(const bf16_t* branch, const bf16_t* rh, const bf16_t* rl, const float* x32, int64_t rows, int D,
                          const float* gamma, const float* beta, float eps, bf16_t* yh, bf16_t* yl, float* yF, hipStream_t s);

int launch_conv0_group_apply(int prec, const float* wav, int B, int64_t L, int k, int stride, int64_t T1, int C,
                             const float* coef, void* out , hipStream_t s, int pair_kind = 0);
int launch_conv0_layer(int prec, const float* wav, int B, int64_t L, int k, int stride, int64_t T1, int C,
                       const double* wav_moments, int64_t n_wav, float eps_wav, const float* w0, const float* b0,
                       const float* gamma, const float* beta, float eps, void* out, hipStream_t s, int clips_per_norm_group,
                       int pair_kind = 0);
int launch_f32_to_pairs(int kind, const float* x, void* out, int64_t n, hipStream_t s);
int launch_pairs_to_f32(int kind, const void* in, const void* lo_plane, float* y, int64_t n, hipStream_t s);

bool conv0_mfma_ok(int prec, int pair_kind, int k, int stride, int C);
size_t conv0_mfma_table_bytes(int B);
int launch_conv0_mfma_group(const float* wav, int B, int64_t L, int stride, int64_t T1, const float* coef, void* table_ws, void* out,
                            hipStream_t s, int pair_kind = 0);
int launch_conv0_mfma_layer(const float* wav, int B, int64_t L, int stride, int64_t T1, const double* wav_moments, int64_t n_wav,
                            float eps_wav, const float* w0, const float* b0, const float* gamma, const float* beta, float eps, void* table_ws,
                            void* out, hipStream_t s, int clips_per_norm_group, int pair_kind = 0);
extern int g_conv0_mfma;

int launch_f32_to_bf16(const float* in, bf16_t* out, int64_t n, hipStream_t s);
int launch_zero_bytes(void* p, size_t bytes, hipStream_t s);
int launch_copy_f32(const float* in, float* out, int64_t n, hipStream_t s);
int launch_zero_cols(float* p, int64_t rows, int cols, int64_t ld, hipStream_t s);
int launch_posconv_gather(int prec, const float* h, int B, int T, int D, int G, int kp, int Tp, void* out, hipStream_t s,
                          const float* sc = nullptr, const float* sh = nullptr);
int launch_posconv_scatter_add(const float* h, const void* y, int B, int T, int D, int G, int P, int Tq, float* pre, hipStream_t s,
                               int y_f32 = 0);
int launch_softmax_rows(int prec, const float* S, int64_t rows, int T, int Tp, void* P, hipStream_t s);
int launch_transpose_v(int prec, const void* qkv, int B, int T, int H, int dh, long ld, long voff, int Tp,
                       void* Vt, hipStream_t s);
int launch_axpby(int prec, const void* x, const void* y, float a, float b, void* out, int64_t n, hipStream_t s);
int launch_add_pe(int prec, const float* x, int B, int T, int Tsrc, int D, const float* pe, float* outF, void* outT,
                  hipStream_t s);
int launch_add_f32(const float* a, const float* b, float* out, int64_t n, hipStream_t s);
int launch_relpos_table(const float* embed, int H, int T, int num_buckets, int max_distance, float* pb, hipStream_t s);
int launch_relpos_gate(int prec, const void* u, int64_t rows, int T, int H, int dh, const float* wab, const float* bab,
                       const float* cst, float* gate, hipStream_t s);
int launch_scores_add_relbias(float* S, int64_t BH, int H, int T, int Tp, const float* gate, const float* pb, hipStream_t s);
int launch_clock_stamp(long long* out16, hipStream_t s);

int launch_flash_attention(const void* Q, long ldq, long q_bstride, const void* K, const void* V, long ldk, long k_bstride,
                           void* O, long ldo, long o_bstride, int B, int T, int H, int dh, float scale, hipStream_t s,
                           const float* gate = nullptr, const float* pb = nullptr);

int launch_split_planes(int kind, const float* src, long ld_src, long rows, int cols, void* dst, long ld_dst, long plane, hipStream_t s);
bool flash_attention_x3_ok(int dh);
int launch_flash_attention_x3(int kind, const void* Q, long ldq, long q_bstride, long q_plane, const void* K, const void* V, long ldk,
                              long k_bstride, long k_plane, float* O, long ldo, long o_bstride, int B, int T, int H, int dh, float scale,
                              hipStream_t s, int o_pairs = 0);

int launch_linear_f32(const float* x, int64_t rows, int K, const float* w, const float* b, int N, float* y,
                      hipStream_t s);
bool linear_head_eligible(int K, int N);
int launch_linear_head(const float* x, int64_t rows, int K, const float* w, const float* b, int N, float* y, hipStream_t s);
int launch_bce_loss(const float* x, int64_t B, int64_t t_pred, const float* y, int64_t t_tgt, int64_t T, const float* rel_len,
                    const float* pos_weight, float* per_frame, double* sums, hipStream_t s);
int launch_nll_loss(const float* logp, int64_t B, int64_t t_pred, int C, const int64_t* tgt, int64_t t_tgt, int64_t T,
                    const float* rel_len, float* per_frame, double* sums, int* bad_target, hipStream_t s);
int launch_loss_reduce(const double* sums, int B, int reduction, float smoothing, float* out, hipStream_t s);
int launch_softmax_small(const float* x, int64_t rows, int n, int apply_log, float* y, hipStream_t s);
int launch_deltas(const float* x, long ldx, int B, int T, int C, int n, float inv_denom, float* out, long ldo, hipStream_t s);
int launch_context_window(const float* x, int B, int T, int C, int ctx, int lag, int pad, float* out, hipStream_t s);
int launch_fbank_frames(const float* wav, int B, int64_t L, int n_fft, int hop, int64_t nframes, const float* window,
                        float* frames , hipStream_t s);
int launch_power_spectrum(const float* reim , int64_t rows, int nb,
                          int imoff, int ld, float* power , int ldp, hipStream_t s);
int launch_fbank_db(float* fb, int B, int64_t per_seq, float top_db, hipStream_t s);
int launch_decode_frames(const float* logits, int64_t rows, int n_out, int n_oct, int n_cls, FrameOut* out,
                         hipStream_t s);
int launch_ctc_greedy(const float* probs, int B, int T, int V, const float* rel_lens, int blank, int32_t* tokens,
                      int32_t* out_lens, hipStream_t s);

size_t noise_mix_scratch_bytes();
int launch_noise_mix(const float* clean, const float* noise, int64_t n, const double* factors, int n_snr, float* out, int64_t ld,
                     double* amps_out, void* scratch, hipStream_t s);
int resample_units_per_tile(int P, int W, int S, bool downmix);
int launch_resample(const float* in, int rows_out, int64_t n_in, int64_t ld_in, const float* w, const int32_t* first, int P, int W, int S,
                    float* out, int64_t n_out, int64_t ld_out, bool downmix, hipStream_t s);
int launch_video_pad(int prec, const float* v, int B, int T, int H, int W, int Hp, int Wp, void* out, hipStream_t s);
struct VideoTransform { double sub0, div0, mean, std; };
int launch_video_pad_u8(int prec, const unsigned char* v, int B, int T, int Hin, int Win, int dy, int dx, int H, int W, int Hp, int Wp,
                        const VideoTransform& tf, void* out, hipStream_t s);
int launch_conv3d_front(int prec, const void* vp, const void* w, const float* bias, const float* slope, long F, int T, int Hp,
                        int Wp, int H0, int W0, void* out, hipStream_t s);
int launch_maxpool_3x3s2(int prec, const void* in, long F, int H0, int W0, int C, int H1, int W1, void* out, hipStream_t s);
extern int g_stem_pool_fused;
bool conv3d_front_pool_ok(int prec, int Hp, int Wp, int W0);
int launch_conv3d_front_pool(const void* vp, const void* w, const float* bias, const float* slope, long F, int T, int Hp, int Wp, int H0,
                             int W0, int H1, int W1, void* out, hipStream_t s);
int launch_zero_halo(int prec, void* buf, long F, int Hp, int Wp, int C, hipStream_t s);
int launch_avgpool_interior(int prec, const void* in, long F, int H, int W, int C, void* out, hipStream_t s);
extern int g_conv3x3_c64, g_conv3x3_c64_launches, g_conv3x3_c64_form;
bool conv3x3_c64_ok(int prec, int Hs, int Ws);
int launch_conv3x3_c64(const void* in, const void* wimg, const float* bias, const float* slope, const void* resid, void* out, long F,
                       int Hs, int Ws, hipStream_t s);
bool conv3x3_c128_ok(int prec, int Hs, int Ws);
int launch_conv3x3_c128(const void* in, const void* wimg, const float* bias, const float* slope, const void* resid, void* out, long F,
                        int Hs, int Ws, hipStream_t s);
int launch_amt_objective_grad(const float* x, int64_t B, int64_t t_pred, int n_out, int n_oct_cols, const float* on_t,
                              const float* off_t, const int64_t* oct_t, const int64_t* cls_t, int64_t t_tgt, int64_t T,
                              const float* rel_len, float pos_weight, float smoothing, float* dx, float* terms, void* ws,
// ... 59 lines not shown
```

svt_speechbrain_amd/csrc/conv0_mfma.hip:

```cpp
#include "common.h"

namespace svt {
namespace {

constexpr int K0 = 10, C0 = 512, TBL16 = 2048;

template <int PK> struct C0T { typedef bf16_t piece; };
template <> struct C0T<2> { typedef __bf16 piece; };
template <> struct C0T<3> { typedef _Float16 piece; };
template <int PK> __device__ __forceinline__ f32x4 c0_mma(const typename C0T<PK>::piece __attribute__((ext_vector_type(8))) & a, const uint4& b, const f32x4& c) {
  typedef typename C0T<PK>::piece P;
  typedef P P8 __attribute__((ext_vector_type(8)));
  if constexpr (PK == 3) return __builtin_amdgcn_mfma_f32_16x16x32_f16(a, __builtin_bit_cast(P8, b), c, 0, 0, 0);
  else if constexpr (PK == 2) return __builtin_amdgcn_mfma_f32_16x16x32_bf16(a, __builtin_bit_cast(P8, b), c, 0, 0, 0);
  else return SVT_MFMA_16x16x32(a, __builtin_bit_cast(P8, b), c);
}
template <int PK> __device__ __forceinline__ void c0_store8(void* out, int64_t e, f32x2_t (&p)[4]) {
  typedef typename C0T<PK>::piece P;
  typedef P P8 __attribute__((ext_vector_type(8)));
  if constexpr (PK == 0) {
    gelu_bf16x2_x4(p);
    P8 o;
#pragma unroll
    for (int i = 0; i < 4; ++i) { o[2 * i] = (P)p[i].x; o[2 * i + 1] = (P)p[i].y; }
    *(P8*)((P*)out + e) = o;
  } else {
    P8 hi, lo;
#pragma unroll
    for (int i = 0; i < 4; ++i) {
      const f32x2_t y = gelu_fast2(p[i]);
      hi[2 * i] = (P)y.x; lo[2 * i] = (P)(y.x - (float)hi[2 * i]);
      hi[2 * i + 1] = (P)y.y; lo[2 * i + 1] = (P)(y.y - (float)hi[2 * i + 1]);
    }
    char* d = (char*)out + (e >> 5) * 128 + (e & 31) * 2;
    *(P8*)d = hi;
    *(P8*)(d + 64) = lo;
  }
}

__global__ __launch_bounds__(256) void conv0_coef_exp_kernel(const float* __restrict__ coef, int* __restrict__ exps) {
  const int b = blockIdx.x;
  float mx = 0.f;
  for (int i = threadIdx.x; i < C0 * K0; i += 256) mx = fmaxf(mx, fabsf(coef[((long)b * C0 + i / K0) * (K0 + 1) + i % K0]));
#pragma unroll
  for (int o = 32; o > 0; o >>= 1) mx = fmaxf(mx, __shfl_xor(mx, o, 64));
  __shared__ float part[4];
  if ((threadIdx.x & 63) == 0) part[threadIdx.x >> 6] = mx;
  __syncthreads();
  if (threadIdx.x == 0) {
    mx = fmaxf(fmaxf(part[0], part[1]), fmaxf(part[2], part[3]));
    int e = 0;
    if (mx > 0.f && mx < 3e38f) (void)frexpf(mx, &e);
    exps[b] = e > 100 ? 100 : (e < -100 ? -100 : e);
  }
}

template <int PK>
__global__ void conv0_table_kernel(const float* __restrict__ w, long w_clip_stride, int w_row, const float* __restrict__ bias,
                                   void* __restrict__ table_, const int* __restrict__ tap_exp) {
  typedef typename C0T<PK>::piece bf16_t;
  typedef bf16_t bf16x8 __attribute__((ext_vector_type(8)));
  bf16_t* table = (bf16_t*)table_;
  const int b = blockIdx.y;
  const int idx = blockIdx.x * blockDim.x + threadIdx.x;
  if (idx >= TBL16) return;
  const int blk = idx >> 6, lane = idx & 63, q = blk >> 3, nb = blk & 7, g = lane >> 4, j = lane & 15;
  const int c = 128 * q + 8 * j + nb;
  const float* wc = w + (long)b * w_clip_stride + (long)c * w_row;
  const float bv = bias ? bias[c] : (w_row == K0 + 1 ? wc[K0] : 0.f);
  const float tap_scale = tap_exp ? ldexpf(1.f, -tap_exp[b]) : 1.f;
  bf16x8 o;
#pragma unroll
  for (int i = 0; i < 8; ++i) {
    const int k = 8 * g + i;
    const float src = k < 30 ? wc[k % 10] * tap_scale : bv;
    const bf16_t hi = (bf16_t)src;
    const bf16_t lo = (bf16_t)(src - (float)hi);
    o[i] = (k < 20 || k == 30) ? hi : lo;
  }
  *(bf16x8*)(table + ((long)b * TBL16 + idx) * 8) = o;
}

template <int MODE, int PK = 0>
__global__ __launch_bounds__(256) void conv0_mfma_kernel(const float* __restrict__ wav, int64_t L, int stride, int64_t T1,
                                                         const void* __restrict__ table_, long table_clip_stride,
                                                         const double* __restrict__ wav_mom, int64_t n_wav, float eps_wav,
                                                         const float* __restrict__ gamma, const float* __restrict__ beta, float eps, int cpg,
                                                         void* __restrict__ out, const int* __restrict__ tap_exp) {
  typedef typename C0T<PK>::piece bf16_t;
  typedef bf16_t bf16x8 __attribute__((ext_vector_type(8)));
  const bf16_t* table = (const bf16_t*)table_;
  constexpr int FPW = 64;
  __shared__ __attribute__((aligned(16))) uint4 tbl[TBL16];
  __shared__ float xs[4][FPW * 5 + 16];
  const int tid = threadIdx.x, lane = tid & 63, wave = tid >> 6;
  const int b = blockIdx.y;
  {
    const uint4* tg = (const uint4*)(table + (long)b * table_clip_stride);
    for (int i = tid; i < TBL16; i += 256) tbl[i] = tg[i];
  }
  float mu = 0.f, rn = 1.f, xscale = 1.f, bscale = 1.f;
  if (MODE == 1 && wav_mom) {
    const double* wm = wav_mom + 2 * (b / cpg);
    const double m = wm[0] / (double)n_wav;
    const double var = wm[1] / (double)n_wav - m * m;
    mu = (float)m;
    rn = (float)(1.0 / sqrt(var + (double)eps_wav));
  }
  const int64_t t0 = ((int64_t)blockIdx.x * 4 + wave) * FPW;
  const int64_t left = T1 - t0;
  const int nfr = left >= FPW ? FPW : (left > 0 ? (int)left : 0);
  if (nfr > 0) {
    const float* x = wav + (int64_t)b * L + t0 * stride;
    const int ns = (nfr - 1) * stride + K0;
    float amax = 0.f;
    for (int i = lane; i < ns; i += 64) {
      const float v = MODE == 1 ? (x[i] - mu) * rn : x[i];
      xs[wave][i] = v;
      amax = fmaxf(amax, fabsf(v));
    }
    if constexpr (MODE == 0) {
#pragma unroll
      for (int o = 32; o > 0; o >>= 1) amax = fmaxf(amax, __shfl_xor(amax, o, 64));
      int e = 0;
      if (amax > 0.f && amax < 3e38f) { (void)frexpf(amax, &e); }
      e = e > 100 ? 100 : (e < -100 ? -100 : e);
      int tot = -e - (tap_exp ? tap_exp[b] : 0);
      tot = tot > 15 ? 15 : (tot < -14 ? -14 : tot);
      xscale = ldexpf(1.f, -e);
      bscale = ldexpf(1.f, tot);
      xscale = ldexpf(1.f, tot + (tap_exp ? tap_exp[b] : 0));
    }
  }
  __syncthreads();
  if (nfr <= 0) return;
  const float unscale = 1.f / bscale;
  const int g = lane >> 4, j = lane & 15;
  const bf16_t one = (bf16_t)bscale;
  for (int chunk = 0; chunk * 16 < nfr; ++chunk) {
    bf16x8 a;
    {
      int f = chunk * 16 + j;
      if (f > nfr - 1) f = nfr - 1;
      const float* xp = &xs[wave][f * stride];
      bf16_t h[K0], l[K0];
#pragma unroll
      for (int i = 0; i < K0; ++i) {
        const float v = xp[i] * xscale;
        h[i] = (bf16_t)v;
        l[i] = (bf16_t)(v - (float)h[i]);
      }
      const bf16x8 a0 = {h[0], h[1], h[2], h[3], h[4], h[5], h[6], h[7]};
      const bf16x8 a1 = {h[8], h[9], l[0], l[1], l[2], l[3], l[4], l[5]};
      const bf16x8 a2 = {l[6], l[7], l[8], l[9], h[0], h[1], h[2], h[3]};
      const bf16x8 a3 = {h[4], h[5], h[6], h[7], h[8], h[9], one, one};
      a = g == 0 ? a0 : (g == 1 ? a1 : (g == 2 ? a2 : a3));
    }
    const int64_t e0 = ((int64_t)b * T1 + t0 + chunk * 16 + 4 * g) * C0 + 8 * j;
    const int fr0 = chunk * 16 + 4 * g;
    if constexpr (MODE == 0) {
#pragma unroll 1
      for (int q = 0; q < 4; ++q) {
        f32x4 acc[8];
// ... 5 lines not shown
#pragma unroll
        for (int r = 0; r < 4; ++r) {
          f32x2_t p[4];
#pragma unroll
          for (int i = 0; i < 4; ++i) p[i] = f32x2_t{acc[2 * i][r], acc[2 * i + 1][r]} * unscale;
          if (fr0 + r < nfr) c0_store8<PK>(out, e0 + (int64_t)r * C0 + 128 * q, p);
        }
      }
    } else {
      f32x4 acc[32];
#pragma unroll
      for (int blk = 0; blk < 32; ++blk) {
        acc[blk] = f32x4{0.f, 0.f, 0.f, 0.f};
        acc[blk] = c0_mma<PK>(a, tbl[blk * 64 + lane], acc[blk]);
      }
      float mean[4], rstd[4];
#pragma unroll
      for (int r = 0; r < 4; ++r) {
        float s = 0.f;
#pragma unroll
        for (int blk = 0; blk < 32; ++blk) s += acc[blk][r];
#pragma unroll
        for (int o = 8; o > 0; o >>= 1) s += __shfl_xor(s, o, 64);
        mean[r] = s * (1.f / C0);
      }
#pragma unroll
      for (int r = 0; r < 4; ++r) {
        float qq = 0.f;
#pragma unroll
        for (int blk = 0; blk < 32; ++blk) { const float d = acc[blk][r] - mean[r]; qq = fmaf(d, d, qq); }
#pragma unroll
        for (int o = 8; o > 0; o >>= 1) qq += __shfl_xor(qq, o, 64);
        rstd[r] = rsqrtf(qq * (1.f / C0) + eps);
      }
#pragma unroll
      for (int q = 0; q < 4; ++q) {
        __builtin_amdgcn_sched_barrier(0);
        const float4 g0 = *(const float4*)(gamma + 128 * q + 8 * j), g1 = *(const float4*)(gamma + 128 * q + 8 * j + 4);
        const float4 b0 = *(const float4*)(beta + 128 * q + 8 * j), b1 = *(const float4*)(beta + 128 * q + 8 * j + 4);
        const float gg[8] = {g0.x, g0.y, g0.z, g0.w, g1.x, g1.y, g1.z, g1.w}, bb[8] = {b0.x, b0.y, b0.z, b0.w, b1.x, b1.y, b1.z, b1.w};
#pragma unroll
        for (int r = 0; r < 4; ++r) {
          f32x2_t p[4];
#pragma unroll
          for (int i = 0; i < 4; ++i)
            p[i] = f32x2_t{fmaf((acc[q * 8 + 2 * i][r] - mean[r]) * rstd[r], gg[2 * i], bb[2 * i]),
                           fmaf((acc[q * 8 + 2 * i + 1][r] - mean[r]) * rstd[r], gg[2 * i + 1], bb[2 * i + 1])};
          if (fr0 + r < nfr) c0_store8<PK>(out, e0 + (int64_t)r * C0 + 128 * q, p);
        }
      }
    }
  }
}

}

int g_conv0_mfma = 1;

bool conv0_mfma_ok(int prec, int pair_kind, int k, int stride, int C) {
  return g_conv0_mfma && (prec == 1 || pair_kind == 2 || pair_kind == 3) && k == K0 && stride >= 1 && stride <= 5 && C == C0;
}
size_t conv0_mfma_table_bytes(int B) { return (size_t)B * TBL16 * 16 + (((size_t)B * 4 + 255) & ~(size_t)255); }

#define SVT_C0_DISPATCH(PKV, STMT)                 \
  if ((PKV) == 3) { constexpr int PK_ = 3; STMT }  \
  else if ((PKV) == 2) { constexpr int PK_ = 2; STMT } \
  else { constexpr int PK_ = 0; STMT }

int launch_conv0_mfma_group(const float* wav, int B, int64_t L, int stride, int64_t T1, const float* coef, void* table_ws, void* out,
                            hipStream_t s, int pair_kind) {
  if (((uintptr_t)table_ws & 15) || ((uintptr_t)out & 127)) { set_error("conv0_mfma: alignment"); return -1; }
  dim3 grid((unsigned)((T1 + 255) / 256), B);
  int* exps = (int*)((char*)table_ws + (size_t)B * TBL16 * 16);
  hipLaunchKernelGGL(conv0_coef_exp_kernel, dim3(B), dim3(256), 0, s, coef, exps);
  SVT_C0_DISPATCH(pair_kind,
    hipLaunchKernelGGL((conv0_table_kernel<PK_>), dim3(TBL16 / 256, B), dim3(256), 0, s, coef, (long)C0 * (K0 + 1), K0 + 1, (const float*)nullptr,
                       table_ws, (const int*)exps);
    hipLaunchKernelGGL((conv0_mfma_kernel<0, PK_>), grid, dim3(256), 0, s, wav, L, stride, T1, (const void*)table_ws, (long)TBL16 * 8,
                       (const double*)nullptr, (int64_t)1, 0.f, (const float*)nullptr, (const float*)nullptr, 0.f, 1, out, (const int*)exps);)
  SVT_LAUNCH_CHECK();
  return 0;
}

int launch_conv0_mfma_layer(const float* wav, int B, int64_t L, int stride, int64_t T1, const double* wav_moments, int64_t n_wav,
                            float eps_wav, const float* w0, const float* b0, const float* gamma, const float* beta, float eps, void* table_ws,
                            void* out, hipStream_t s, int cpg, int pair_kind) {
  if (((uintptr_t)table_ws & 15) || ((uintptr_t)out & 127) || ((uintptr_t)gamma & 15) || ((uintptr_t)beta & 15)) { set_error("conv0_mfma: alignment"); return -1; }
  dim3 grid((unsigned)((T1 + 255) / 256), B);
  SVT_C0_DISPATCH(pair_kind,
    hipLaunchKernelGGL((conv0_table_kernel<PK_>), dim3(TBL16 / 256, 1), dim3(256), 0, s, w0, 0L, K0, b0, table_ws, (const int*)nullptr);
    hipLaunchKernelGGL((conv0_mfma_kernel<1, PK_>), grid, dim3(256), 0, s, wav, L, stride, T1, (const void*)table_ws, 0L, wav_moments, n_wav,
                       eps_wav, gamma, beta, eps, cpg, out, (const int*)nullptr);)
  SVT_LAUNCH_CHECK();
  return 0;
}
#undef SVT_C0_DISPATCH

}
```

svt_speechbrain_amd/csrc/device_util.h:

```cpp
#pragma once
#include "common.h"

namespace svt {
namespace {

template <typename V>
__device__ __forceinline__ V wave_sum(V v) {
#pragma unroll
  for (int o = 32; o > 0; o >>= 1) v += __shfl_xor(v, o, 64);
  return v;
}
__device__ __forceinline__ float wave_max(float v) {
#pragma unroll
  for (int o = 32; o > 0; o >>= 1) v = fmaxf(v, __shfl_xor(v, o, 64));
  return v;
}

typedef const void __attribute__((address_space(1)))* gptr_t;
typedef void __attribute__((address_space(3)))* lptr_t;
__device__ __forceinline__ unsigned lds_base(uint4* lds) { return __builtin_amdgcn_readfirstlane((unsigned)(size_t)(lptr_t)lds); }

template <typename T> __device__ __forceinline__ float ld(const T* p, long i);
template <> __device__ __forceinline__ float ld<float>(const float* p, long i) { return p[i]; }
template <> __device__ __forceinline__ float ld<bf16_t>(const bf16_t* p, long i) { return (float)p[i]; }
template <typename T> __device__ __forceinline__ void st(T* p, long i, float v);
template <> __device__ __forceinline__ void st<float>(float* p, long i, float v) { p[i] = v; }
template <> __device__ __forceinline__ void st<bf16_t>(bf16_t* p, long i, float v) { p[i] = (bf16_t)v; }

template <int PK> __device__ __forceinline__ void cut_piece(float x, unsigned short& hi, unsigned short& lo) {
  if constexpr (PK == 3) {
    const _Float16 a = (_Float16)x, b = (_Float16)(x - (float)a);
    hi = __builtin_bit_cast(unsigned short, a); lo = __builtin_bit_cast(unsigned short, b);
  } else {
    const __bf16 a = (__bf16)x, b = (__bf16)(x - (float)a);
    hi = __builtin_bit_cast(unsigned short, a); lo = __builtin_bit_cast(unsigned short, b);
  }
}
template <int PK, int N> __device__ __forceinline__ void store_pairs(void* base, int64_t e, const float (&v)[N]) {
  static_assert(N == 4 || N == 8, "pieces of 4 or 8 elements");
  unsigned short h[N], l[N];
#pragma unroll
  for (int i = 0; i < N; ++i) cut_piece<PK>(v[i], h[i], l[i]);
  char* d = (char*)base + (e >> 5) * 128 + (e & 31) * 2;
  if constexpr (N == 8) {
    *(uint4*)d = uint4{(unsigned)h[0] | ((unsigned)h[1] << 16), (unsigned)h[2] | ((unsigned)h[3] << 16), (unsigned)h[4] | ((unsigned)h[5] << 16), (unsigned)h[6] | ((unsigned)h[7] << 16)};
    *(uint4*)(d + 64) = uint4{(unsigned)l[0] | ((unsigned)l[1] << 16), (unsigned)l[2] | ((unsigned)l[3] << 16), (unsigned)l[4] | ((unsigned)l[5] << 16), (unsigned)l[6] | ((unsigned)l[7] << 16)};
  } else {
    *(uint2*)d = uint2{(unsigned)h[0] | ((unsigned)h[1] << 16), (unsigned)h[2] | ((unsigned)h[3] << 16)};
    *(uint2*)(d + 64) = uint2{(unsigned)l[0] | ((unsigned)l[1] << 16), (unsigned)l[2] | ((unsigned)l[3] << 16)};
  }
}

constexpr int K0 = 10;
constexpr int NWM = K0 + K0 * (K0 + 1) / 2;

inline int grid_for(int64_t n, int block = 256, int cap = 8192) {
  int64_t g = (n + block - 1) / block;
  if (g > cap) g = cap;
  if (g < 1) g = 1;
  return (int)g;
}
template <class... P> inline bool aligned(unsigned mask, P... p) { return !((... | (uintptr_t)p) & mask); }

}
}
```

svt_speechbrain_amd/csrc/layernorm.hip:

```cpp
#include "device_util.h"
#include <type_traits>

namespace svt {
namespace {
template <typename TI, typename TO>
__global__ __launch_bounds__(256) void layernorm_kernel(const TI* x, const float* add, float* sumF, int64_t rows, int D,
                                                        const float* gamma, const float* beta, float eps, int gelu,
                                                        TO* yT, float* yF) {
  const int lane = threadIdx.x & 63;
  const int64_t row = (int64_t)blockIdx.x * 4 + (threadIdx.x >> 6);
  if (row >= rows) return;
  const TI* xr = x + row * D;
  const float* ar = add ? add + row * D : nullptr;
  float s = 0.f;
  for (int i = lane; i < D; i += 64) s += ld<TI>(xr, i) + (ar ? ar[i] : 0.f);
  const float mean = wave_sum(s) / (float)D;
  float q = 0.f;
  for (int i = lane; i < D; i += 64) { const float d = ld<TI>(xr, i) + (ar ? ar[i] : 0.f) - mean; q += d * d; }
  const float rstd = rsqrtf(wave_sum(q) / (float)D + eps);
  for (int i = lane; i < D; i += 64) {
    const float xv = ld<TI>(xr, i) + (ar ? ar[i] : 0.f);
    if (sumF) sumF[row * D + i] = xv;
    float v = (xv - mean) * rstd * gamma[i] + beta[i];
    if (gelu) v = gelu_erf(v);
// ... 109 lines not shown
    for (int i = 0; i < 8; ++i) { v[j][i] -= mean; q = fmaf(v[j][i], v[j][i], q); }
#pragma unroll
  for (int o = 16; o > 0; o >>= 1) q += __shfl_xor(q, o, 64);
  const float rstd = rsqrtf(q * (1.f / D) + eps);
#pragma unroll
  for (int j = 0; j < NC; ++j) {
    const int c = (sub + 32 * j) * 8;
    const float4 g0 = *(const float4*)(gamma + c), g1 = *(const float4*)(gamma + c + 4);
    const float4 b0 = *(const float4*)(beta + c), b1 = *(const float4*)(beta + c + 4);
    const float gg[8] = {g0.x, g0.y, g0.z, g0.w, g1.x, g1.y, g1.z, g1.w}, bb[8] = {b0.x, b0.y, b0.z, b0.w, b1.x, b1.y, b1.z, b1.w};
    f32x2_t o2[4];
#pragma unroll
    for (int i = 0; i < 4; ++i) o2[i] = f32x2_t{fmaf(v[j][2 * i] * rstd, gg[2 * i], bb[2 * i]), fmaf(v[j][2 * i + 1] * rstd, gg[2 * i + 1], bb[2 * i + 1])};
    if (gelu) gelu_bf16x2_x4(o2);
    bf16x8 ob;
#pragma unroll
    for (int i = 0; i < 4; ++i) { ob[2 * i] = (bf16_t)o2[i].x; ob[2 * i + 1] = (bf16_t)o2[i].y; }
    *(bf16x8*)(y + row * D + c) = ob;
  }
}

template <class F> void ln_width(int D, F&& f) {
  if (D == 512) f(std::integral_constant<int, 8>{});
  else if (D == 768) f(std::integral_constant<int, 12>{});
  else f(std::integral_constant<int, 16>{});
}
}
int g_ln_two_rows = 1;
int g_ln_kernel_id = 0;
int launch_layernorm(const LnArgs& a, hipStream_t s) {
  const int prec = a.prec, x_is_f32 = a.x_is_f32, D = a.D, gelu = a.gelu, pair_kind = a.pair_kind;
  const void *const x = a.x, *const addP = a.addP;
  const int64_t rows = a.rows;
  const float *const gamma = a.gamma, *const beta = a.beta, *const add = a.add;
  const float eps = a.eps;
  void *const yT = a.yT, *const yP = a.yP;
  float *const yF = a.yF, *const sumF = a.sumF;
  if (addP && !yP) { set_error("layernorm: a pair-row addend needs the pair-row output form"); return -1; }
  const dim3 grid((unsigned)((rows + 3) / 4)), grid2((unsigned)((rows + 7) / 8)), block(256);
  const bool wide = D == 512 || D == 768 || D == 1024;
  if (yP) {
    if (prec || !x_is_f32 || yT || !wide || (pair_kind != 2 && pair_kind != 3) || !aligned(15, x, yF, add, sumF, gamma, beta) || !aligned(127, yP)) { set_error("layernorm: the pair-row output needs an fp32 input, D in {512, 768, 1024} and aligned buffers"); return -1; }
    g_ln_kernel_id = pair_kind == 3 ? 2300 : 2200;
    ln_width(D, [&](auto vpt) {
      constexpr int VPT = decltype(vpt)::value;
      if (pair_kind == 3) hipLaunchKernelGGL((layernorm_f32_vec_kernel<VPT, float, float, 3>), grid, block, 0, s, (const float*)x, add, sumF, rows, gamma, beta, eps, gelu, (float*)nullptr, yF, yP, addP);
      else hipLaunchKernelGGL((layernorm_f32_vec_kernel<VPT, float, float, 2>), grid, block, 0, s, (const float*)x, add, sumF, rows, gamma, beta, eps, gelu, (float*)nullptr, yF, yP, addP);
    });
  } else if (prec && !x_is_f32 && wide && yT && !yF && !add && !sumF && g_ln_two_rows && aligned(15, x, yT, gamma, beta)) {
    g_ln_kernel_id = 3000;
    ln_width(D, [&](auto vpt) {
      hipLaunchKernelGGL((layernorm_op16_rows2_kernel<64 * decltype(vpt)::value>), grid2, block, 0, s, (const bf16_t*)x, rows, gamma, beta, eps, gelu, (bf16_t*)yT);
    });
  } else if (prec && !x_is_f32 && wide && aligned(7, x) && aligned(15, yT, yF, add, sumF)) {
    g_ln_kernel_id = 2011;
    ln_width(D, [&](auto vpt) {
      hipLaunchKernelGGL((layernorm_f32_vec_kernel<decltype(vpt)::value, bf16_t, bf16_t>), grid, block, 0, s, (const bf16_t*)x, add, sumF, rows, gamma, beta, eps, gelu, (bf16_t*)yT, yF);
    });
  } else if (add && !x_is_f32) {
    set_error("layernorm: the addend form needs an fp32 input (or bf16 with D in {512,768,1024})");
    return -1;
  } else if (x_is_f32 && wide && aligned(15, x, yT, yF, gamma, beta, add, sumF)) {
    g_ln_kernel_id = prec ? 2001 : 2000;
    ln_width(D, [&](auto vpt) {
      constexpr int VPT = decltype(vpt)::value;
      if (prec) hipLaunchKernelGGL((layernorm_f32_vec_kernel<VPT, bf16_t>), grid, block, 0, s, (const float*)x, add, sumF, rows, gamma, beta, eps, gelu, (bf16_t*)yT, yF);
      else hipLaunchKernelGGL((layernorm_f32_vec_kernel<VPT, float>), grid, block, 0, s, (const float*)x, add, sumF, rows, gamma, beta, eps, gelu, (float*)yT, yF);
    });
  } else if (!prec) {
    g_ln_kernel_id = 1000;
    hipLaunchKernelGGL((layernorm_kernel<float, float>), grid, block, 0, s, (const float*)x, add, sumF, rows, D, gamma, beta, eps, gelu, (float*)yT, yF);
  } else if (x_is_f32) {
    g_ln_kernel_id = 1001;
    hipLaunchKernelGGL((layernorm_kernel<float, bf16_t>), grid, block, 0, s, (const float*)x, add, sumF, rows, D, gamma, beta, eps, gelu, (bf16_t*)yT, yF);
  } else {
    g_ln_kernel_id = 1011;
    hipLaunchKernelGGL((layernorm_kernel<bf16_t, bf16_t>), grid, block, 0, s, (const bf16_t*)x, add, sumF, rows, D, gamma, beta, eps, gelu, (bf16_t*)yT, yF);
  }
  SVT_LAUNCH_CHECK();
  return 0;
}

namespace {
template <int VPT>
__global__ __launch_bounds__(256) void layernorm_hilo_kernel(const bf16_t* branch, const bf16_t* rh, const bf16_t* rl,
                                                             int64_t rows, const float* gamma, const float* beta, float eps,
                                                             bf16_t* yh, bf16_t* yl, float* yF) {
  constexpr int D = 64 * VPT, NV = VPT / 4;
  const int lane = threadIdx.x & 63;
  const int64_t row = (int64_t)blockIdx.x * 4 + (threadIdx.x >> 6);
  if (row >= rows) return;
  float v[VPT];
  float s = 0.f;
#pragma unroll
  for (int j = 0; j < NV; ++j) {
    const long o = row * D + (lane + 64 * j) * 4;
    const bf16x4 h = *(const bf16x4*)(rh + o), l = *(const bf16x4*)(rl + o);
    float4 t = float4{(float)h[0] + (float)l[0], (float)h[1] + (float)l[1], (float)h[2] + (float)l[2], (float)h[3] + (float)l[3]};
    if (branch) {
      const bf16x4 a = *(const bf16x4*)(branch + o);
      t.x += (float)a[0]; t.y += (float)a[1]; t.z += (float)a[2]; t.w += (float)a[3];
    }
    v[4 * j] = t.x; v[4 * j + 1] = t.y; v[4 * j + 2] = t.z; v[4 * j + 3] = t.w;
    s += (t.x + t.y) + (t.z + t.w);
  }
  const float mean = wave_sum(s) * (1.f / D);
  float q = 0.f;
#pragma unroll
  for (int i = 0; i < VPT; ++i) { v[i] -= mean; q = fmaf(v[i], v[i], q); }
  const float rstd = rsqrtf(wave_sum(q) * (1.f / D) + eps);
#pragma unroll
  for (int j = 0; j < NV; ++j) {
    const int c = (lane + 64 * j) * 4;
    const float4 g = *(const float4*)(gamma + c), b = *(const float4*)(beta + c);
    const float o[4] = {fmaf(v[4 * j] * rstd, g.x, b.x), fmaf(v[4 * j + 1] * rstd, g.y, b.y),
                        fmaf(v[4 * j + 2] * rstd, g.z, b.z), fmaf(v[4 * j + 3] * rstd, g.w, b.w)};
    bf16x4 oh, ol;
#pragma unroll
    for (int i = 0; i < 4; ++i) { oh[i] = (bf16_t)o[i]; ol[i] = (bf16_t)(o[i] - (float)oh[i]); }
    *(bf16x4*)(yh + row * D + c) = oh;
    *(bf16x4*)(yl + row * D + c) = ol;
    if (yF) *(float4*)(yF + row * D + c) = float4{o[0], o[1], o[2], o[3]};
  }
}

template <int D, bool PARTS = false>
__global__ __launch_bounds__(256) void layernorm_hilo2_kernel(const bf16_t* branch, const bf16_t* rh, const bf16_t* rl,
                                                              int64_t rows, const float* gamma, const float* beta, float eps,
                                                              bf16_t* yh, bf16_t* yl, float* yF, const float* parts = nullptr, int nparts = 0,
                                                              long part_stride = 0, const float* pbias = nullptr) {
  constexpr int NC = D / 256;
  const int lane = threadIdx.x & 63, sub = lane & 31;
  const int64_t row = (int64_t)blockIdx.x * 8 + (threadIdx.x >> 6) * 2 + (lane >> 5);
  if (row >= rows) return;
  float v[NC][8];
  float s = 0.f;
#pragma unroll
  for (int j = 0; j < NC; ++j) {
    const long o = row * D + (sub + 32 * j) * 8;
    const bf16x8 h = *(const bf16x8*)(rh + o), l = *(const bf16x8*)(rl + o);
#pragma unroll
    for (int i = 0; i < 8; ++i) v[j][i] = (float)h[i] + (float)l[i];
    if constexpr (PARTS) {
      float a[8];
      {
        const float4 t0 = *(const float4*)(parts + o), t1 = *(const float4*)(parts + o + 4);
        a[0] = t0.x; a[1] = t0.y; a[2] = t0.z; a[3] = t0.w; a[4] = t1.x; a[5] = t1.y; a[6] = t1.z; a[7] = t1.w;
      }
      for (int k = 1; k < nparts; ++k) {
        const float4 t0 = *(const float4*)(parts + k * part_stride + o), t1 = *(const float4*)(parts + k * part_stride + o + 4);
        a[0] += t0.x; a[1] += t0.y; a[2] += t0.z; a[3] += t0.w; a[4] += t1.x; a[5] += t1.y; a[6] += t1.z; a[7] += t1.w;
      }
      const int c = (sub + 32 * j) * 8;
      const float4 b0 = *(const float4*)(pbias + c), b1 = *(const float4*)(pbias + c + 4);
      const float bb[8] = {b0.x, b0.y, b0.z, b0.w, b1.x, b1.y, b1.z, b1.w};
#pragma unroll
      for (int i = 0; i < 8; ++i) v[j][i] += (float)(bf16_t)(a[i] + bb[i]);
    } else if (branch) {
      const bf16x8 a = *(const bf16x8*)(branch + o);
#pragma unroll
      for (int i = 0; i < 8; ++i) v[j][i] += (float)a[i];
    }
    s += ((v[j][0] + v[j][1]) + (v[j][2] + v[j][3])) + ((v[j][4] + v[j][5]) + (v[j][6] + v[j][7]));
  }
#pragma unroll
  for (int o = 16; o > 0; o >>= 1) s += __shfl_xor(s, o, 64);
  const float mean = s * (1.f / D);
  float q = 0.f;
#pragma unroll
  for (int j = 0; j < NC; ++j)
#pragma unroll
    for (int i = 0; i < 8; ++i) { v[j][i] -= mean; q = fmaf(v[j][i], v[j][i], q); }
#pragma unroll
  for (int o = 16; o > 0; o >>= 1) q += __shfl_xor(q, o, 64);
  const float rstd = rsqrtf(q * (1.f / D) + eps);
#pragma unroll
  for (int j = 0; j < NC; ++j) {
    const int c = (sub + 32 * j) * 8;
    const float4 g0 = *(const float4*)(gamma + c), g1 = *(const float4*)(gamma + c + 4);
    const float4 b0 = *(const float4*)(beta + c), b1 = *(const float4*)(beta + c + 4);
    const float gg[8] = {g0.x, g0.y, g0.z, g0.w, g1.x, g1.y, g1.z, g1.w}, bb[8] = {b0.x, b0.y, b0.z, b0.w, b1.x, b1.y, b1.z, b1.w};
    float o[8];
    bf16x8 oh, ol;
#pragma unroll
    for (int i = 0; i < 8; ++i) {
      o[i] = fmaf(v[j][i] * rstd, gg[i], bb[i]);
      oh[i] = (bf16_t)o[i];
      ol[i] = (bf16_t)(o[i] - (float)oh[i]);
    }
    *(bf16x8*)(yh + row * D + c) = oh;
    *(bf16x8*)(yl + row * D + c) = ol;
    if (yF) {
      *(float4*)(yF + row * D + c) = float4{o[0], o[1], o[2], o[3]};
      *(float4*)(yF + row * D + c + 4) = float4{o[4], o[5], o[6], o[7]};
    }
  }
}
template <int VPT>
__global__ __launch_bounds__(256) void layernorm_f32_to_hilo_kernel(const float* x, int64_t rows, const float* gamma,
                                                                    const float* beta, float eps, bf16_t* yh, bf16_t* yl) {
  constexpr int D = 64 * VPT, NV = VPT / 4;
  const int lane = threadIdx.x & 63;
  const int64_t row = (int64_t)blockIdx.x * 4 + (threadIdx.x >> 6);
  if (row >= rows) return;
  float v[VPT];
  float s = 0.f;
#pragma unroll
  for (int j = 0; j < NV; ++j) {
    const float4 t = ((const float4*)(x + row * D))[lane + 64 * j];
    v[4 * j] = t.x; v[4 * j + 1] = t.y; v[4 * j + 2] = t.z; v[4 * j + 3] = t.w;
    s += (t.x + t.y) + (t.z + t.w);
  }
  const float mean = wave_sum(s) * (1.f / D);
  float q = 0.f;
#pragma unroll
  for (int i = 0; i < VPT; ++i) { v[i] -= mean; q = fmaf(v[i], v[i], q); }
  const float rstd = rsqrtf(wave_sum(q) * (1.f / D) + eps);
#pragma unroll
  for (int j = 0; j < NV; ++j) {
    const int c = (lane + 64 * j) * 4;
    const float4 g = *(const float4*)(gamma + c), b = *(const float4*)(beta + c);
    const float o[4] = {fmaf(v[4 * j] * rstd, g.x, b.x), fmaf(v[4 * j + 1] * rstd, g.y, b.y),
                        fmaf(v[4 * j + 2] * rstd, g.z, b.z), fmaf(v[4 * j + 3] * rstd, g.w, b.w)};
    bf16x4 oh, ol;
#pragma unroll
    for (int i = 0; i < 4; ++i) { oh[i] = (bf16_t)o[i]; ol[i] = (bf16_t)(o[i] - (float)oh[i]); }
    *(bf16x4*)(yh + row * D + c) = oh;
    *(bf16x4*)(yl + row * D + c) = ol;
  }
}
}
bool layernorm_hilo_ok(int D) { return D == 512 || D == 768 || D == 1024; }
int launch_layernorm_hilo_parts(const float* parts, int nparts, long part_stride, const float* pbias, const bf16_t* rh, const bf16_t* rl, int64_t rows,
                                int D, const float* gamma, const float* beta, float eps, bf16_t* yh, bf16_t* yl, float* yF, hipStream_t s) {
  if (!parts || nparts < 1 || !pbias || !(D == 512 || D == 768 || D == 1024) || (part_stride & 3) || !aligned(15, parts, pbias, rh, rl, yh, yl, yF, gamma, beta)) { set_error("layernorm (K-split branch): D in {512, 768, 1024} and 16-byte aligned buffers"); return -1; }
  const dim3 grid2((unsigned)((rows + 7) / 8)), block(256);
  g_ln_kernel_id = 5001;
  ln_width(D, [&](auto vpt) {
    hipLaunchKernelGGL((layernorm_hilo2_kernel<64 * decltype(vpt)::value, true>), grid2, block, 0, s, nullptr, rh, rl, rows, gamma, beta, eps, yh, yl, yF, parts, nparts, part_stride, pbias);
  });
  SVT_LAUNCH_CHECK();
  return 0;
}
int launch_layernorm_hilo(const bf16_t* branch, const bf16_t* rh, const bf16_t* rl, const float* x32, int64_t rows, int D,
                          const float* gamma, const float* beta, float eps, bf16_t* yh, bf16_t* yl, float* yF, hipStream_t s) {
  const dim3 grid((unsigned)((rows + 3) / 4)), grid2((unsigned)((rows + 7) / 8)), block(256);
  g_ln_kernel_id = x32 ? 6000 : g_ln_two_rows && aligned(15, branch, rh, rl, yh, yl, yF, gamma, beta) ? 5000 : 4000;
  ln_width(D, [&](auto vpt) {
    constexpr int VPT = decltype(vpt)::value;
    if (x32) hipLaunchKernelGGL((layernorm_f32_to_hilo_kernel<VPT>), grid, block, 0, s, x32, rows, gamma, beta, eps, yh, yl);
    else if (g_ln_two_rows && aligned(15, branch, rh, rl, yh, yl, yF, gamma, beta)) hipLaunchKernelGGL((layernorm_hilo2_kernel<64 * VPT>), grid2, block, 0, s, branch, rh, rl, rows, gamma, beta, eps, yh, yl, yF);
    else hipLaunchKernelGGL((layernorm_hilo_kernel<VPT>), grid, block, 0, s, branch, rh, rl, rows, gamma, beta, eps, yh, yl, yF);
  });
  SVT_LAUNCH_CHECK();
  return 0;
}

}
```

svt_speechbrain_amd/csrc/stats.hip:

```cpp
#include "device_util.h"

namespace svt {
namespace {
__device__ __forceinline__ void st_partial(double* p, double v) {
  __hip_atomic_store((unsigned long long*)p, __builtin_bit_cast(unsigned long long, v), __ATOMIC_RELAXED, __HIP_MEMORY_SCOPE_AGENT);
}
__device__ int d_ticket_fenced = 0;
__device__ __forceinline__ bool last_workgroup(unsigned* ticket, unsigned n_groups) {
  __shared__ unsigned s_last;
  asm volatile("s_waitcnt vmcnt(0)" ::: "memory");
  __syncthreads();
  if (threadIdx.x == 0) {
    const unsigned t = d_ticket_fenced ? __hip_atomic_fetch_add(ticket, 1u, __ATOMIC_ACQ_REL, __HIP_MEMORY_SCOPE_AGENT)
                                       : __hip_atomic_fetch_add(ticket, 1u, __ATOMIC_RELAXED, __HIP_MEMORY_SCOPE_AGENT);
    s_last = t == n_groups - 1 ? 1u : 0u;
    if (s_last) __hip_atomic_store(ticket, 0u, __ATOMIC_RELAXED, __HIP_MEMORY_SCOPE_AGENT);
  }
  __syncthreads();
  return s_last != 0;
}
__device__ __forceinline__ double ld_partial(const double* p) {
  return __builtin_bit_cast(double, __hip_atomic_load((const unsigned long long*)p, __ATOMIC_RELAXED, __HIP_MEMORY_SCOPE_AGENT));
}
}
int set_ticket_fenced(int on) {
  const int v = on ? 1 : 0;
  SVT_HIP(hipMemcpyToSymbol(HIP_SYMBOL(d_ticket_fenced), &v, sizeof(int)));
  return 0;
}

namespace {
__global__ __launch_bounds__(256) void moments_kernel(const float* x, int64_t n, double* mom, double* part, unsigned* ticket) {
  __shared__ double sh[2][4];
  x += (int64_t)blockIdx.y * n;
  mom += 2 * blockIdx.y;
  part += (size_t)blockIdx.y * gridDim.x * 2;
  double s = 0.0, ss = 0.0;
  const int64_t n4 = n >> 2;
  const float4* x4 = (const float4*)x;
  int64_t i = (int64_t)blockIdx.x * blockDim.x + threadIdx.x;
  const int64_t stride = (int64_t)gridDim.x * blockDim.x;
  for (; i < n4; i += stride) {
    const float4 v = x4[i];
    const float a = (v.x + v.y) + (v.z + v.w);
    const float b = (v.x * v.x + v.y * v.y) + (v.z * v.z + v.w * v.w);
    s += (double)a;
    ss += (double)b;
  }
  if (blockIdx.x == 0 && threadIdx.x == 0) {
    for (int64_t j = n4 << 2; j < n; ++j) { s += (double)x[j]; ss += (double)x[j] * (double)x[j]; }
  }
  s = wave_sum(s);
  ss = wave_sum(ss);
  const int lane = threadIdx.x & 63, wave = threadIdx.x >> 6;
  if (lane == 0) { sh[0][wave] = s; sh[1][wave] = ss; }
  __syncthreads();
  if (threadIdx.x == 0) {
    st_partial(part + blockIdx.x * 2, sh[0][0] + sh[0][1] + sh[0][2] + sh[0][3]);
    st_partial(part + blockIdx.x * 2 + 1, sh[1][0] + sh[1][1] + sh[1][2] + sh[1][3]);
  }
  if (!last_workgroup(ticket + blockIdx.y, gridDim.x)) return;
  s = 0.0; ss = 0.0;
  for (unsigned b = threadIdx.x; b < gridDim.x; b += 256) { s += ld_partial(part + b * 2); ss += ld_partial(part + b * 2 + 1); }
  s = wave_sum(s);
  ss = wave_sum(ss);
  if (lane == 0) { sh[0][wave] = s; sh[1][wave] = ss; }
  __syncthreads();
  if (threadIdx.x == 0) {
    mom[0] = sh[0][0] + sh[0][1] + sh[0][2] + sh[0][3];
    mom[1] = sh[1][0] + sh[1][1] + sh[1][2] + sh[1][3];
  }
}

__global__ void global_norm_kernel(const float* x, float* y, int64_t n, const double* mom, float eps, double n_stat) {
  x += (int64_t)blockIdx.y * n;
  y += (int64_t)blockIdx.y * n;
  mom += 2 * blockIdx.y;
  const double mean = mom[0] / n_stat;
  const double var = mom[1] / n_stat - mean * mean;
  const float mu = (float)mean;
  const float rs = (float)(1.0 / sqrt(var + (double)eps));
  const int64_t n4 = n >> 2;
  int64_t i = (int64_t)blockIdx.x * blockDim.x + threadIdx.x;
  const int64_t stride = (int64_t)gridDim.x * blockDim.x;
  for (; i < n4; i += stride) {
    float4 v = ((const float4*)x)[i];
    v.x = (v.x - mu) * rs; v.y = (v.y - mu) * rs; v.z = (v.z - mu) * rs; v.w = (v.w - mu) * rs;
    ((float4*)y)[i] = v;
  }
  if (blockIdx.x == 0 && threadIdx.x == 0)
    for (int64_t j = n4 << 2; j < n; ++j) y[j] = (x[j] - mu) * rs;
}
}
static int moments_grid(int64_t n, int groups) {
  return groups > 1 ? grid_for(n / 4 + 1, 256, 512 / (groups < 64 ? groups : 64) + 1) : grid_for(n / 4 + 1, 256, 512);
}
static size_t moments_ticket_bytes(int groups) { return ((size_t)groups * 4 + 255) & ~(size_t)255; }
size_t moments_scratch_bytes(int groups_max) {
  const size_t wgs = (size_t)(groups_max < 64 ? 512 + groups_max : 576) + 9 * (size_t)groups_max;
  return moments_ticket_bytes(groups_max) + wgs * 2 * sizeof(double);
}

int launch_moments(const float* x, int64_t n, double* moments, void* scratch, int groups_max, hipStream_t s, int groups) {
  if (groups > 1 && (n & 3)) { set_error("moments: per-group length must be a multiple of 4 elements"); return -1; }
  if (groups > groups_max || !scratch || ((uintptr_t)scratch & 7)) { set_error("moments: scratch"); return -1; }
  const int gx = moments_grid(n, groups);
  if (moments_ticket_bytes(groups_max) + (size_t)gx * groups * 2 * sizeof(double) > moments_scratch_bytes(groups_max)) { set_error("moments: scratch too small"); return -1; }
  unsigned* ticket = (unsigned*)scratch;
  double* part = (double*)((char*)scratch + moments_ticket_bytes(groups_max));
  hipLaunchKernelGGL(moments_kernel, dim3(gx, groups), dim3(256), 0, s, x, n, moments, part, ticket);
  SVT_LAUNCH_CHECK();
  return 0;
}

int launch_global_norm(const float* x, float* y, int64_t n, const double* moments, float eps, hipStream_t s, int groups, double n_stat) {
  if (groups > 1 && (n & 3)) { set_error("global_norm: per-group length must be a multiple of 4 elements"); return -1; }
  hipLaunchKernelGGL(global_norm_kernel, dim3(grid_for(n / 4 + 1), groups), dim3(256), 0, s, x, y, n, moments, eps,
                     n_stat > 0 ? n_stat : (double)n);
  SVT_LAUNCH_CHECK();
  return 0;
}

namespace {
__global__ __launch_bounds__(256) void conv0_window_moments_kernel(const float* wav, int64_t L, int stride, int64_t T1,
                                                                   double* wm, double* part, unsigned* ticket) {
  __shared__ double sh[4][NWM];
  const int b = blockIdx.y;
  const float* x = wav + (int64_t)b * L;
  double acc[NWM];
#pragma unroll
  for (int i = 0; i < NWM; ++i) acc[i] = 0.0;
  constexpr int WPT = 8;
  const int64_t t0 = ((int64_t)blockIdx.x * blockDim.x + threadIdx.x) * WPT;
  for (int w = 0; w < WPT; ++w) {
    const int64_t t = t0 + w;
    if (t >= T1) break;
    float v[K0];
#pragma unroll
    for (int j = 0; j < K0; ++j) v[j] = x[t * stride + j];
    int idx = K0;
#pragma unroll
    for (int j = 0; j < K0; ++j) {
      acc[j] += (double)v[j];
#pragma unroll
      for (int j2 = j; j2 < K0; ++j2) acc[idx++] += (double)(v[j] * v[j2]);
    }
  }
  const int lane = threadIdx.x & 63, wave = threadIdx.x >> 6;
#pragma unroll
  for (int i = 0; i < NWM; ++i) {
    const double r = wave_sum(acc[i]);
    if (lane == 0) sh[wave][i] = r;
  }
  __syncthreads();
  part += (size_t)b * gridDim.x * NWM;
  if (threadIdx.x < NWM)
    st_partial(part + blockIdx.x * NWM + threadIdx.x, sh[0][threadIdx.x] + sh[1][threadIdx.x] + sh[2][threadIdx.x] + sh[3][threadIdx.x]);
  if (!last_workgroup(ticket + b, gridDim.x)) return;
  if (threadIdx.x < NWM) {
    double t = 0.0;
    unsigned k = 0;
    for (; k + 8 <= gridDim.x; k += 8) {
      double v[8];
#pragma unroll
      for (int j = 0; j < 8; ++j) v[j] = ld_partial(part + (k + j) * NWM + threadIdx.x);
#pragma unroll
      for (int j = 0; j < 8; ++j) t += v[j];
    }
    for (; k < gridDim.x; ++k) t += ld_partial(part + k * NWM + threadIdx.x);
    wm[b * NWM + threadIdx.x] = t;
  }
}

__global__ void conv0_group_coef_kernel(const double* wav_mom, int64_t n_wav, const double* wm, int64_t T1, int C,
                                        const float* w0, const float* b0, const float* gamma, const float* beta,
                                        float eps_wav, float eps_gn, float* coef, int cpg) {
  const int b = blockIdx.y;
  if (wav_mom) wav_mom += 2 * (b / cpg);
  const int c = blockIdx.x * blockDim.x + threadIdx.x;
  if (c >= C) return;
  double mu = 0.0, r = 1.0;
  if (wav_mom) {
    mu = wav_mom[0] / (double)n_wav;
    const double var = wav_mom[1] / (double)n_wav - mu * mu;
    r = 1.0 / sqrt(var + (double)eps_wav);
  }
  const double* m = wm + b * NWM;
  const double invT = 1.0 / (double)T1;
  double w[K0], mn[K0];
  double wsum = 0.0;
  for (int j = 0; j < K0; ++j) { w[j] = (double)w0[c * K0 + j]; wsum += w[j]; mn[j] = r * (m[j] * invT - mu); }
  const double bias = b0 ? (double)b0[c] : 0.0;
  double dot = 0.0;
  for (int j = 0; j < K0; ++j) dot += w[j] * mn[j];
  double quad = 0.0;
  int idx = K0;
  for (int j = 0; j < K0; ++j)
    for (int j2 = j; j2 < K0; ++j2) {
      const double R = r * r * (m[idx] * invT - mu * m[j] * invT - mu * m[j2] * invT + mu * mu);
      quad += (j == j2 ? 1.0 : 2.0) * w[j] * w[j2] * R;
      ++idx;
    }
  const double mean = dot + bias;
  const double e2 = quad + 2.0 * bias * dot + bias * bias;
  double var = e2 - mean * mean;
  if (var < 0.0) var = 0.0;
  const double a = (double)gamma[c] / sqrt(var + (double)eps_gn);
  const double shift = (double)beta[c] - mean * a;
  float* o = coef + ((int64_t)b * C + c) * (K0 + 1);
  for (int j = 0; j < K0; ++j) o[j] = (float)(a * r * w[j]);
  o[K0] = (float)(a * (bias - r * mu * wsum) + shift);
}
}
size_t conv0_window_moments_scratch_bytes(int B, int64_t T1) {
  const size_t gx = (size_t)((T1 + 2047) / 2048);
  return moments_ticket_bytes(B) + (size_t)B * gx * NWM * sizeof(double);
}

int launch_conv0_window_moments(const float* wav, int B, int64_t L, int k, int stride, int64_t T1, double* wm, void* scratch,
                                hipStream_t s) {
  if (k != K0) { set_error("conv layer 0 kernel size must be 10"); return -1; }
  if (!scratch || ((uintptr_t)scratch & 7)) { set_error("conv0 window moments: scratch"); return -1; }
  const int per_block = 256 * 8;
  dim3 grid((unsigned)((T1 + per_block - 1) / per_block), B);
  unsigned* ticket = (unsigned*)scratch;
  double* part = (double*)((char*)scratch + moments_ticket_bytes(B));
  hipLaunchKernelGGL(conv0_window_moments_kernel, grid, dim3(256), 0, s, wav, L, stride, T1, wm, part, ticket);
  SVT_LAUNCH_CHECK();
  return 0;
}

int launch_conv0_group_coef(const double* wav_moments, int64_t n_wav, const double* wm, int B, int64_t T1, int C,
                            int k, const float* w0, const float* b0, const float* gamma, const float* beta,
                            float eps_wav, float eps_gn, float* coef, hipStream_t s, int cpg) {
  if (k != K0) { set_error("conv layer 0 kernel size must be 10"); return -1; }
  dim3 grid((C + 63) / 64, B);
  hipLaunchKernelGGL(conv0_group_coef_kernel, grid, dim3(64), 0, s, wav_moments, n_wav, wm, T1, C, w0, b0, gamma, beta,
                     eps_wav, eps_gn, coef, cpg);
  SVT_LAUNCH_CHECK();
  return 0;
}

namespace {
template <int KC>
__global__ __launch_bounds__(256) void head_dots_kernel(const float* __restrict__ x, int64_t rows, const float* __restrict__ w, int N,
                                                        float* __restrict__ dots, double* __restrict__ mom, int64_t rows_per_group,
                                                        double* __restrict__ slots, unsigned* __restrict__ ticket, int slots_per_group) {
  constexpr int K = KC * 256;
  extern __shared__ __attribute__((aligned(16))) float wl[];
  for (int i = threadIdx.x * 4; i < N * K; i += 1024) *(float4*)(wl + i) = *(const float4*)(w + i);
  __syncthreads();
  const int lane = threadIdx.x & 63, wave = threadIdx.x >> 6;
  const bool hi32 = (lane & 32) != 0, hi16 = (lane & 16) != 0;
  const int myrow = (hi32 ? 2 : 0) + (hi16 ? 1 : 0);
  const int NW = (int)gridDim.x * 4, W = (int)blockIdx.x * 4 + wave;
  int64_t cur_g = -1, g_end = 0;
  float la = 0.f, lq = 0.f;
  auto flush = [&]() {
    if (cur_g < 0) return;
    const double sa = wave_sum((double)la), sq = wave_sum((double)lq);
    if (lane == 0) {
      const int64_t ja = (cur_g * rows_per_group) >> 2;
      const int p = (int)(((W - ja) % NW + NW) % NW);
      double* sl = slots + ((size_t)cur_g * slots_per_group + p) * 2;
      st_partial(sl, sa);
      st_partial(sl + 1, sq);
    }
    la = 0.f; lq = 0.f;
  };
  for (int64_t r0 = ((int64_t)blockIdx.x * 4 + wave) * 4; r0 < rows; r0 += (int64_t)gridDim.x * 16) {
    float4 xv[4][KC];
#pragma unroll
    for (int rr = 0; rr < 4; ++rr) {
      const int64_t row = r0 + rr < rows ? r0 + rr : rows - 1;
      const auto xrs = __builtin_amdgcn_make_buffer_rsrc((void*)x, 0, 0x7FFFFFF0, 0x00020000);
#pragma unroll
      for (int c = 0; c < KC; ++c) {
        typedef float f4v __attribute__((ext_vector_type(4)));
        const f4v t = __builtin_bit_cast(f4v, __builtin_amdgcn_raw_buffer_load_b128(xrs, (unsigned)((row * K + c * 256 + lane * 4) * 4), 0, 0));
        xv[rr][c] = float4{t[0], t[1], t[2], t[3]};
      }
    }
    if (mom) {
#pragma unroll
      for (int rr = 0; rr < 4; ++rr) {
        if (r0 + rr >= rows) break;
        if (r0 + rr >= g_end || cur_g < 0) {
          flush();
          cur_g = (r0 + rr) / rows_per_group;
          g_end = (cur_g + 1) * rows_per_group;
        }
        float a = 0.f, q = 0.f;
#pragma unroll
        for (int c = 0; c < KC; ++c) {
          const float4 v = xv[rr][c];
          a += (v.x + v.y) + (v.z + v.w);
          q += (v.x * v.x + v.y * v.y) + (v.z * v.z + v.w * v.w);
        }
        la += a;
        lq += q;
      }
    }
    float out0 = 0.f, out1 = 0.f;
    for (int n = 0; n < N; ++n) {
      float sacc[4] = {0.f, 0.f, 0.f, 0.f};
#pragma unroll
      for (int c = 0; c < KC; ++c) {
        const float4 wv = *(const float4*)(wl + n * K + c * 256 + lane * 4);
#pragma unroll
        for (int rr = 0; rr < 4; ++rr) {
// ... 144 lines not shown
```

Measured before the change: 6277 clips/s.

## Fuse waveform stats, conv0 coef+table, posconv add into LN, skip last LN planes

Four independent launch-reduction fusions, each behind a debug flag that defaults on. The waveform moments and the conv0 window moments are computed in one launch. Conv0 group coefficients and the MFMA weight table are built in one kernel. The positional-conv scatter-add is folded into the first encoder layernorm. The last layer's layernorm no longer writes the bf16 hi/lo planes. These cut kernel launches and memory round-trips in a small-batch forward, in exchange for more complex kernels and extra fallback branches.

```diff
diff --git a/include/svt_mi355.h b/include/svt_mi355.h
--- a/include/svt_mi355.h
+++ b/include/svt_mi355.h
@@ -196,6 +196,10 @@
 } svt_debug_layernorm_desc;
 int svt_debug_layernorm(const svt_debug_layernorm_desc* d, int device, void* stream);
 
+int svt_debug_posconv_layernorm(const float* h_dev, const void* y_dev, int32_t batch, int32_t t, int32_t d, int32_t groups,
+                                int32_t frames_per_row, int32_t rows_per_clip, float* pre_dev, const float* gamma_dev, const float* beta_dev,
+                                float eps, void* yh_dev, void* yl_dev, int device, void* stream);
+
 typedef struct svt_video svt_video;
 int svt_video_create(int32_t embed_dim, int32_t precision, int device, svt_video** out);
 void svt_video_destroy(svt_video* v);
diff --git a/svt_speechbrain_amd/_lib.py b/svt_speechbrain_amd/_lib.py
--- a/svt_speechbrain_amd/_lib.py
+++ b/svt_speechbrain_amd/_lib.py
@@ -129,6 +129,8 @@
                                  C.c_int64, C.c_int64, C.c_int32, C.c_int32, C.c_int, _P]),
     "svt_debug_gemm_batched": (C.c_int, [C.c_int32, C.POINTER(GemmDescC), C.c_int, _P]),
     "svt_debug_layernorm": (C.c_int, [C.POINTER(LayerNormDescC), C.c_int, _P]),
+    "svt_debug_posconv_layernorm": (C.c_int, [_P, _P, C.c_int32, C.c_int32, C.c_int32, C.c_int32, C.c_int32, C.c_int32, _P, _P, _P, C.c_float, _P, _P,
+                                    C.c_int, _P]),
     "svt_debug_attention_scores": (C.c_int, [C.c_int32, _P, _P, _P, _P, C.c_int32, C.c_int32, C.c_int32, C.c_int32, C.c_int64, C.c_int64,
                                              C.c_int64, C.c_float, _P, _P, C.c_int, _P]),
     "svt_debug_gemm_pairs": (C.c_int, [C.c_int32, _P, C.c_int64, _P, _P, _P, C.c_int32, C.c_int32, C.c_int32, C.c_int32, C.c_int64,
diff --git a/svt_speechbrain_amd/csrc/api.hip b/svt_speechbrain_amd/csrc/api.hip
--- a/svt_speechbrain_amd/csrc/api.hip
+++ b/svt_speechbrain_amd/csrc/api.hip
@@ -359,7 +359,7 @@
       return refuse("every buffer 16-byte aligned, yP / addP 128-byte aligned");
   } else {
     if (!hilo_width) return refuse("the (hi, lo) forms need D in {512, 768, 1024}");
-    if (!d->yh || !d->yl) return refuse("null yh / yl");
+    if ((!d->yh || !d->yl) && (d->yh || d->yl || !d->yF || d->x32)) return refuse("null yh / yl");
     if (!aligned(15, d->gamma, d->beta, d->branch, d->rh, d->rl, d->x32, d->yh, d->yl, d->yF, d->parts, d->pbias))
       return refuse("every buffer 16-byte aligned");
     if (d->form == 1 && !(d->x32 ? !d->rh && !d->rl : d->rh && d->rl)) return refuse("form 1 takes exactly one of x32 and (rh, rl)");
@@ -384,6 +384,17 @@
                                      d->rows, d->D, d->gamma, d->beta, d->eps, (bf16_t*)d->yh, (bf16_t*)d->yl, d->yF, s);
   }
   return rc ? SVT_ERR_INVALID : SVT_OK;
+}
+
+int svt_debug_posconv_layernorm(const float* h, const void* y, int32_t batch, int32_t t, int32_t d, int32_t groups, int32_t frames_per_row,
+                                int32_t rows_per_clip, float* pre, const float* gamma, const float* beta, float eps, void* yh, void* yl,
+                                int device, void* stream) {
+  if (!h || !y || !pre || !gamma || !beta || !yh || !yl || batch < 1 || t < 1 || groups < 1 || frames_per_row < 1 || rows_per_clip < 1) {
+    set_error("svt_debug_posconv_layernorm: null or non-positive argument"); return SVT_ERR_INVALID; }
+  if (int r = check_device(device)) return r;
+  SVT_HIP(hipSetDevice(device));
+  return launch_posconv_add_layernorm_hilo(h, (const bf16_t*)y, batch, t, d, groups, frames_per_row, rows_per_clip, pre, gamma, beta, eps,
+                                           (bf16_t*)yh, (bf16_t*)yl, (hipStream_t)stream) ? SVT_ERR_INVALID : SVT_OK;
 }
 
 int svt_debug_gemm_pairs(int32_t precision, const float* a, int64_t a_elems, const float* w, float* c, const float* bias, int32_t m,
@@ -563,6 +574,10 @@
   else if (key == 38) return g_flash_kernel_id;
   else if (key == 39) return g_gemm_kernel_id;
   else if (key == 40) return g_ln_kernel_id;
+  else if (key == 41) g_last_ln_storeless = value;
+  else if (key == 42) g_pos_ln_fused = value;
+  else if (key == 43) g_conv0_chain_fused = value;
+  else if (key == 44) g_stats_one_launch = value;
   else { set_error("svt_debug_set: unknown key"); return SVT_ERR_INVALID; }
   return SVT_OK;
 }
diff --git a/svt_speechbrain_amd/csrc/api_encoder.hip b/svt_speechbrain_amd/csrc/api_encoder.hip
--- a/svt_speechbrain_amd/csrc/api_encoder.hip
+++ b/svt_speechbrain_amd/csrc/api_encoder.hip
@@ -11,6 +11,8 @@
 using namespace svt;
 
 int svt::g_conv_ln_bf16 = 1;
+int svt::g_stats_one_launch = 1;
+int svt::g_last_ln_storeless = 1;
 
 struct ConvLayerW {
   DevBuf w;
@@ -477,6 +479,7 @@
   double* wav_mom = nullptr;
   double* out_mom = nullptr;
   double* win_mom = nullptr;
+  bool win_mom_done = false;
   int64_t n_wav = 0;
   bool global_norm = false;
   ReduceCtx rctx{nullptr, nullptr, nullptr};
@@ -515,8 +518,14 @@
   x.out_mom = w.mom + 2 * B;
   x.win_mom = w.mom + 4 * B;
   x.n_wav = (int64_t)x.cpg * x.p.L;
-  if (c.normalize_wav)
+  if (g_stats_one_launch && c.num_conv_layers > 0) {
+    const bool group0 = c.feat_extract_norm == SVT_NORM_GROUP;
+    if (int r = launch_waveform_statistics(wav, x.p.B, x.p.L, c.conv_kernel[0], c.conv_stride[0], x.p.t1, group0 ? x.win_mom : nullptr,
+                                           (char*)w.mom + w.mom_scr[2], x.n_wav, x.wav_mom, (char*)w.mom + w.mom_scr[0], x.p.B, x.groups, x.s)) return r;
+    x.win_mom_done = group0;
+  } else if (c.normalize_wav) {
     if (int r = launch_moments(wav, x.n_wav, x.wav_mom, (char*)w.mom + w.mom_scr[0], x.p.B, x.s, x.groups)) return r;
+  }
   x.rctx = ReduceCtx{x.e, nullptr, x.s};
   x.global_norm = x.e->reduce_fn != nullptr;
   if (x.global_norm) {
@@ -574,10 +583,12 @@
   const float* b0 = c.conv_bias ? c0.bias.as<float>() : nullptr;
   const bool mfma = conv0_mfma_ok(prec, x.pk_front, k, st, C0) && w.c0tab;
   if (c.feat_extract_norm == SVT_NORM_GROUP) {
-    if (int r = launch_conv0_window_moments(wav, B, L, k, st, t1, x.win_mom, (char*)w.mom + w.mom_scr[2], x.s)) return r;
+    if (!x.win_mom_done)
+      if (int r = launch_conv0_window_moments(wav, B, L, k, st, t1, x.win_mom, (char*)w.mom + w.mom_scr[2], x.s)) return r;
+    if (mfma) return launch_conv0_mfma_group_stats(wav, B, L, st, t1, x.wav_mom, x.n_wav, x.win_mom, c0.w.as<float>(), b0, c0.gamma.as<float>(),
+                                                   c0.beta.as<float>(), 1e-5f, 1e-5f, x.cpg, w.coef, w.c0tab, w.act[0], x.s, x.pk_front);
     if (int r = launch_conv0_group_coef(x.wav_mom, x.n_wav, x.win_mom, B, t1, C0, k, c0.w.as<float>(), b0, c0.gamma.as<float>(),
                                         c0.beta.as<float>(), 1e-5f, 1e-5f, w.coef, x.s, x.cpg)) return r;
-    if (mfma) return launch_conv0_mfma_group(wav, B, L, st, t1, w.coef, w.c0tab, w.act[0], x.s, x.pk_front);
     return launch_conv0_group_apply(prec, wav, B, L, k, st, t1, C0, w.coef, w.act[0], x.s, x.pk_front);
   }
   if (mfma)
@@ -672,6 +683,8 @@
   return g;
 }
 
+bool pos_add_in_ln0(const EncRun& x) { return x.p.pos_multi && x.p.hilo && x.c.pos_conv_depth <= 1; }
+
 int positional_conv(const EncRun& x) {
   const svt_encoder_config& c = x.c;
   const svt_encoder* e = x.e;
@@ -706,6 +719,7 @@
     g.a_z2 = (long)Tp * cg; g.w_z2 = (long)g.N * g.K; g.c_z2 = (long)B * Tq * g.N; g.bias_z2 = g.N;
     g.act = ACT_GELU; g.out_f32 = 0;
     if (int r = launch_gemm(gp, g, x.s)) return r;
+    if (pos_add_in_ln0(x)) return SVT_OK;
     return launch_posconv_scatter_add(w.hF, w.posy, B, T, D, G, Pf, Tq, w.preF, x.s, prec ? 0 : 1);
   }
   if (int r = launch_posconv_gather(prec, w.hF, B, T, D, G, kp, T + kp, w.posg, x.s, bn_sc, bn_sh)) return r;
@@ -793,13 +807,20 @@
   f.branch_f32 = 0;
   f.ffn2_ksplit = ffn2_ksplit_ok(x);
   return post_ln_layers(x, f,
-    [&] { return launch_layernorm_hilo(nullptr, nullptr, nullptr, w.preF, rows, D, x.e->enc_g.as<float>(), x.e->enc_b.as<float>(), eps, xh, xl, nullptr, x.s); },
+    [&] {
+      if (pos_add_in_ln0(x))
+        return launch_posconv_add_layernorm_hilo(w.hF, (const bf16_t*)w.posy, x.p.B, (int)x.p.T, D, x.c.pos_conv_groups, x.p.Pf, (int)x.p.pos_Tq, w.preF,
+                                                 x.e->enc_g.as<float>(), x.e->enc_b.as<float>(), eps, xh, xl, x.s);
+      return launch_layernorm_hilo(nullptr, nullptr, nullptr, w.preF, rows, D, x.e->enc_g.as<float>(), x.e->enc_b.as<float>(), eps, xh, xl, nullptr, x.s);
+    },
     [&](const EncLayerW& Lw, bool second, bool last) {
       const float *g = (second ? Lw.ln2g : Lw.ln1g).as<float>(), *b = (second ? Lw.ln2b : Lw.ln1b).as<float>();
       float* const yF = last ? x.resid : nullptr;
+      const bool planes = !(last && g_last_ln_storeless);
+      bf16_t *const yh = planes ? xh : nullptr, *const yl = planes ? xl : nullptr;
       if (second && f.ffn2_ksplit)
-        return launch_layernorm_hilo_parts(w.ksplit, 4, (long)rows * D, Lw.b2.as<float>(), xh, xl, rows, D, g, b, eps, xh, xl, yF, x.s);
-      return launch_layernorm_hilo((const bf16_t*)w.hF, xh, xl, nullptr, rows, D, g, b, eps, xh, xl, yF, x.s);
+        return launch_layernorm_hilo_parts(w.ksplit, 4, (long)rows * D, Lw.b2.as<float>(), xh, xl, rows, D, g, b, eps, yh, yl, yF, x.s);
+      return launch_layernorm_hilo((const bf16_t*)w.hF, xh, xl, nullptr, rows, D, g, b, eps, yh, yl, yF, x.s);
     });
 }
 
diff --git a/svt_speechbrain_amd/csrc/common.h b/svt_speechbrain_amd/csrc/common.h
--- a/svt_speechbrain_amd/csrc/common.h
+++ b/svt_speechbrain_amd/csrc/common.h
@@ -267,6 +267,8 @@
 extern int g_ffn2_ksplit;
 #pragma GCC visibility push(hidden)
 extern int g_conv_ln_bf16;
+extern int g_stats_one_launch;
+extern int g_last_ln_storeless;
 extern int g_debug_keep_split;
 extern int g_conv_down_fused;
 #pragma GCC visibility pop
@@ -288,6 +290,8 @@
 int launch_conv0_window_moments(const float* wav, int B, int64_t L, int k, int stride, int64_t T1,
                                 double* wm , void* scratch , hipStream_t s);
 size_t conv0_window_moments_scratch_bytes(int B, int64_t T1);
+int launch_waveform_statistics(const float* wav, int B, int64_t L, int k, int stride, int64_t T1, double* wm, void* win_scratch, int64_t n,
+                               double* mom, void* mom_scratch, int groups_max, int groups, hipStream_t s);
 int launch_conv0_group_coef(const double* wav_moments , int64_t n_wav, const double* wm, int B,
                             int64_t T1, int C, int k, const float* w0 , const float* b0 ,
                             const float* gamma, const float* beta, float eps_wav, float eps_gn,
@@ -323,6 +327,9 @@
                                 int D, const float* gamma, const float* beta, float eps, bf16_t* yh, bf16_t* yl, float* yF, hipStream_t s);
 int launch_layernorm_hilo(const bf16_t* branch, const bf16_t* rh, const bf16_t* rl, const float* x32, int64_t rows, int D,
                           const float* gamma, const float* beta, float eps, bf16_t* yh, bf16_t* yl, float* yF, hipStream_t s);
+int launch_posconv_add_layernorm_hilo(const float* h, const bf16_t* y, int B, int T, int D, int G, int P, int Tq, float* pre,
+                                      const float* gamma, const float* beta, float eps, bf16_t* yh, bf16_t* yl, hipStream_t s);
+extern int g_pos_ln_fused;
 
 int launch_conv0_group_apply(int prec, const float* wav, int B, int64_t L, int k, int stride, int64_t T1, int C,
                              const float* coef, void* out , hipStream_t s, int pair_kind = 0);
@@ -340,7 +347,11 @@
 int launch_conv0_mfma_layer(const float* wav, int B, int64_t L, int stride, int64_t T1, const double* wav_moments, int64_t n_wav,
                             float eps_wav, const float* w0, const float* b0, const float* gamma, const float* beta, float eps, void* table_ws,
                             void* out, hipStream_t s, int clips_per_norm_group, int pair_kind = 0);
+int launch_conv0_mfma_group_stats(const float* wav, int B, int64_t L, int stride, int64_t T1, const double* wav_moments, int64_t n_wav,
+                                  const double* wm, const float* w0, const float* b0, const float* gamma, const float* beta, float eps_wav,
+                                  float eps_gn, int clips_per_norm_group, float* coef, void* table_ws, void* out, hipStream_t s, int pair_kind = 0);
 extern int g_conv0_mfma;
+extern int g_conv0_chain_fused;
 
 int launch_f32_to_bf16(const float* in, bf16_t* out, int64_t n, hipStream_t s);
 int launch_zero_bytes(void* p, size_t bytes, hipStream_t s);
diff --git a/svt_speechbrain_amd/csrc/conv0_mfma.hip b/svt_speechbrain_amd/csrc/conv0_mfma.hip
--- a/svt_speechbrain_amd/csrc/conv0_mfma.hip
+++ b/svt_speechbrain_amd/csrc/conv0_mfma.hip
@@ -1,9 +1,9 @@
-#include "common.h"
+#include "device_util.h"
 
 namespace svt {
 namespace {
 
-constexpr int K0 = 10, C0 = 512, TBL16 = 2048;
+constexpr int C0 = 512, TBL16 = 2048;
 
 template <int PK> struct C0T { typedef bf16_t piece; };
 template <> struct C0T<2> { typedef __bf16 piece; };
@@ -56,6 +56,26 @@
 }
 
 template <int PK>
+__device__ __forceinline__ typename C0T<PK>::piece __attribute__((ext_vector_type(8))) c0_table_entry(const float* wc, float bv, float tap_scale, int g) {
+  typedef typename C0T<PK>::piece bf16_t;
+  typedef bf16_t bf16x8 __attribute__((ext_vector_type(8)));
+  bf16x8 o;
+#pragma unroll
+  for (int i = 0; i < 8; ++i) {
+    const int k = 8 * g + i;
+    const float src = k < 30 ? wc[k % 10] * tap_scale : bv;
+    const bf16_t hi = (bf16_t)src;
+    const bf16_t lo = (bf16_t)(src - (float)hi);
+    o[i] = (k < 20 || k == 30) ? hi : lo;
+  }
+  return o;
+}
+__device__ __forceinline__ int c0_table_channel(int idx) {
+  const int blk = idx >> 6, lane = idx & 63, q = blk >> 3, nb = blk & 7, j = lane & 15;
+  return 128 * q + 8 * j + nb;
+}
+
+template <int PK>
 __global__ void conv0_table_kernel(const float* __restrict__ w, long w_clip_stride, int w_row, const float* __restrict__ bias,
                                    void* __restrict__ table_, const int* __restrict__ tap_exp) {
   typedef typename C0T<PK>::piece bf16_t;
@@ -64,21 +84,46 @@
   const int b = blockIdx.y;
   const int idx = blockIdx.x * blockDim.x + threadIdx.x;
   if (idx >= TBL16) return;
-  const int blk = idx >> 6, lane = idx & 63, q = blk >> 3, nb = blk & 7, g = lane >> 4, j = lane & 15;
-  const int c = 128 * q + 8 * j + nb;
+  const int c = c0_table_channel(idx);
   const float* wc = w + (long)b * w_clip_stride + (long)c * w_row;
   const float bv = bias ? bias[c] : (w_row == K0 + 1 ? wc[K0] : 0.f);
   const float tap_scale = tap_exp ? ldexpf(1.f, -tap_exp[b]) : 1.f;
-  bf16x8 o;
-#pragma unroll
-  for (int i = 0; i < 8; ++i) {
-    const int k = 8 * g + i;
-    const float src = k < 30 ? wc[k % 10] * tap_scale : bv;
-    const bf16_t hi = (bf16_t)src;
-    const bf16_t lo = (bf16_t)(src - (float)hi);
-    o[i] = (k < 20 || k == 30) ? hi : lo;
-  }
-  *(bf16x8*)(table + ((long)b * TBL16 + idx) * 8) = o;
+  *(bf16x8*)(table + ((long)b * TBL16 + idx) * 8) = c0_table_entry<PK>(wc, bv, tap_scale, (idx & 63) >> 4);
+}
+
+template <int PK>
+__global__ __launch_bounds__(C0) void conv0_coef_table_kernel(const double* __restrict__ wav_mom, int64_t n_wav, const double* __restrict__ wm,
+                                                               int64_t T1, const float* __restrict__ w0, const float* __restrict__ b0,
+                                                               const float* __restrict__ gamma, const float* __restrict__ beta, float eps_wav,
+                                                               float eps_gn, int cpg, float* __restrict__ coef, void* __restrict__ table_,
+                                                               int* __restrict__ exps) {
+  typedef typename C0T<PK>::piece bf16_t;
+  typedef bf16_t bf16x8 __attribute__((ext_vector_type(8)));
+  __shared__ float cf[C0 * (K0 + 1)];
+  __shared__ float part[C0 / 64];
+  const int b = blockIdx.x, c = threadIdx.x;
+  if (wav_mom) wav_mom += 2 * (b / cpg);
+  float o[K0 + 1];
+  conv0_group_coef_channel(wav_mom, n_wav, wm + b * NWM, T1, c, w0, b0, gamma, beta, eps_wav, eps_gn, o);
+  float* dst = coef + ((long)b * C0 + c) * (K0 + 1);
+  float mx = 0.f;
+  for (int j = 0; j <= K0; ++j) { cf[c * (K0 + 1) + j] = o[j]; dst[j] = o[j]; }
+  for (int j = 0; j < K0; ++j) mx = fmaxf(mx, fabsf(o[j]));
+  mx = wave_max(mx);
+  if ((c & 63) == 0) part[c >> 6] = mx;
+  __syncthreads();
+  mx = part[0];
+  for (int i = 1; i < C0 / 64; ++i) mx = fmaxf(mx, part[i]);
+  int e = 0;
+  if (mx > 0.f && mx < 3e38f) (void)frexpf(mx, &e);
+  e = e > 100 ? 100 : (e < -100 ? -100 : e);
+  if (c == 0) exps[b] = e;
+  const float tap_scale = ldexpf(1.f, -e);
+  bf16_t* table = (bf16_t*)table_;
+  for (int idx = c; idx < TBL16; idx += C0) {
+    const float* wc = cf + c0_table_channel(idx) * (K0 + 1);
+    *(bf16x8*)(table + ((long)b * TBL16 + idx) * 8) = c0_table_entry<PK>(wc, wc[K0], tap_scale, (idx & 63) >> 4);
+  }
 }
 
 template <int MODE, int PK = 0>
@@ -250,6 +295,26 @@
   return 0;
 }
 
+int g_conv0_chain_fused = 1;
+int launch_conv0_mfma_group_stats(const float* wav, int B, int64_t L, int stride, int64_t T1, const double* wav_moments, int64_t n_wav,
+                                  const double* wm, const float* w0, const float* b0, const float* gamma, const float* beta, float eps_wav,
+                                  float eps_gn, int cpg, float* coef, void* table_ws, void* out, hipStream_t s, int pair_kind) {
+  if (!g_conv0_chain_fused) {
+    if (int r = launch_conv0_group_coef(wav_moments, n_wav, wm, B, T1, C0, K0, w0, b0, gamma, beta, eps_wav, eps_gn, coef, s, cpg)) return r;
+    return launch_conv0_mfma_group(wav, B, L, stride, T1, coef, table_ws, out, s, pair_kind);
+  }
+  if (((uintptr_t)table_ws & 15) || ((uintptr_t)out & 127)) { set_error("conv0_mfma: alignment"); return -1; }
+  dim3 grid((unsigned)((T1 + 255) / 256), B);
+  int* exps = (int*)((char*)table_ws + (size_t)B * TBL16 * 16);
+  SVT_C0_DISPATCH(pair_kind,
+    hipLaunchKernelGGL((conv0_coef_table_kernel<PK_>), dim3(B), dim3(C0), 0, s, wav_moments, n_wav, wm, T1, w0, b0, gamma, beta, eps_wav, eps_gn,
+                       cpg, coef, table_ws, exps);
+    hipLaunchKernelGGL((conv0_mfma_kernel<0, PK_>), grid, dim3(256), 0, s, wav, L, stride, T1, (const void*)table_ws, (long)TBL16 * 8,
+                       (const double*)nullptr, (int64_t)1, 0.f, (const float*)nullptr, (const float*)nullptr, 0.f, 1, out, (const int*)exps);)
+  SVT_LAUNCH_CHECK();
+  return 0;
+}
+
 int launch_conv0_mfma_layer(const float* wav, int B, int64_t L, int stride, int64_t T1, const double* wav_moments, int64_t n_wav,
                             float eps_wav, const float* w0, const float* b0, const float* gamma, const float* beta, float eps, void* table_ws,
                             void* out, hipStream_t s, int cpg, int pair_kind) {
diff --git a/svt_speechbrain_amd/csrc/device_util.h b/svt_speechbrain_amd/csrc/device_util.h
--- a/svt_speechbrain_amd/csrc/device_util.h
+++ b/svt_speechbrain_amd/csrc/device_util.h
@@ -53,6 +53,39 @@
 
 constexpr int K0 = 10;
 constexpr int NWM = K0 + K0 * (K0 + 1) / 2;
+__device__ __forceinline__ void conv0_group_coef_channel(const double* wav_mom, int64_t n_wav, const double* m, int64_t T1, int c,
+                                                         const float* w0, const float* b0, const float* gamma, const float* beta,
+                                                         float eps_wav, float eps_gn, float (&o)[K0 + 1]) {
+  double mu = 0.0, r = 1.0;
+  if (wav_mom) {
+    mu = wav_mom[0] / (double)n_wav;
+    const double var = wav_mom[1] / (double)n_wav - mu * mu;
+    r = 1.0 / sqrt(var + (double)eps_wav);
+  }
+  const double invT = 1.0 / (double)T1;
+  double w[K0], mn[K0];
+  double wsum = 0.0;
+  for (int j = 0; j < K0; ++j) { w[j] = (double)w0[c * K0 + j]; wsum += w[j]; mn[j] = r * (m[j] * invT - mu); }
+  const double bias = b0 ? (double)b0[c] : 0.0;
+  double dot = 0.0;
+  for (int j = 0; j < K0; ++j) dot += w[j] * mn[j];
+  double quad = 0.0;
+  int idx = K0;
+  for (int j = 0; j < K0; ++j)
+    for (int j2 = j; j2 < K0; ++j2) {
+      const double R = r * r * (m[idx] * invT - mu * m[j] * invT - mu * m[j2] * invT + mu * mu);
+      quad += (j == j2 ? 1.0 : 2.0) * w[j] * w[j2] * R;
+      ++idx;
+    }
+  const double mean = dot + bias;
+  const double e2 = quad + 2.0 * bias * dot + bias * bias;
+  double var = e2 - mean * mean;
+  if (var < 0.0) var = 0.0;
+  const double a = (double)gamma[c] / sqrt(var + (double)eps_gn);
+  const double shift = (double)beta[c] - mean * a;
+  for (int j = 0; j < K0; ++j) o[j] = (float)(a * r * w[j]);
+  o[K0] = (float)(a * (bias - r * mu * wsum) + shift);
+}
 
 inline int grid_for(int64_t n, int block = 256, int cap = 8192) {
   int64_t g = (n + block - 1) / block;
diff --git a/svt_speechbrain_amd/csrc/layernorm.hip b/svt_speechbrain_amd/csrc/layernorm.hip
--- a/svt_speechbrain_amd/csrc/layernorm.hip
+++ b/svt_speechbrain_amd/csrc/layernorm.hip
@@ -215,7 +215,7 @@
 }
 
 namespace {
-template <int VPT>
+template <int VPT, bool PLANES = true>
 __global__ __launch_bounds__(256) void layernorm_hilo_kernel(const bf16_t* branch, const bf16_t* rh, const bf16_t* rl,
                                                              int64_t rows, const float* gamma, const float* beta, float eps,
                                                              bf16_t* yh, bf16_t* yl, float* yF) {
@@ -248,16 +248,18 @@
     const float4 g = *(const float4*)(gamma + c), b = *(const float4*)(beta + c);
     const float o[4] = {fmaf(v[4 * j] * rstd, g.x, b.x), fmaf(v[4 * j + 1] * rstd, g.y, b.y),
                         fmaf(v[4 * j + 2] * rstd, g.z, b.z), fmaf(v[4 * j + 3] * rstd, g.w, b.w)};
-    bf16x4 oh, ol;
-#pragma unroll
-    for (int i = 0; i < 4; ++i) { oh[i] = (bf16_t)o[i]; ol[i] = (bf16_t)(o[i] - (float)oh[i]); }
-    *(bf16x4*)(yh + row * D + c) = oh;
-    *(bf16x4*)(yl + row * D + c) = ol;
-    if (yF) *(float4*)(yF + row * D + c) = float4{o[0], o[1], o[2], o[3]};
-  }
-}
-
-template <int D, bool PARTS = false>
+    if constexpr (PLANES) {
+      bf16x4 oh, ol;
+#pragma unroll
+      for (int i = 0; i < 4; ++i) { oh[i] = (bf16_t)o[i]; ol[i] = (bf16_t)(o[i] - (float)oh[i]); }
+      *(bf16x4*)(yh + row * D + c) = oh;
+      *(bf16x4*)(yl + row * D + c) = ol;
+    }
+    if (!PLANES || yF) *(float4*)(yF + row * D + c) = float4{o[0], o[1], o[2], o[3]};
+  }
+}
+
+template <int D, bool PARTS = false, bool PLANES = true>
 __global__ __launch_bounds__(256) void layernorm_hilo2_kernel(const bf16_t* branch, const bf16_t* rh, const bf16_t* rl,
                                                               int64_t rows, const float* gamma, const float* beta, float eps,
                                                               bf16_t* yh, bf16_t* yl, float* yF, const float* parts = nullptr, int nparts = 0,
@@ -314,19 +316,44 @@
     const float4 b0 = *(const float4*)(beta + c), b1 = *(const float4*)(beta + c + 4);
     const float gg[8] = {g0.x, g0.y, g0.z, g0.w, g1.x, g1.y, g1.z, g1.w}, bb[8] = {b0.x, b0.y, b0.z, b0.w, b1.x, b1.y, b1.z, b1.w};
     float o[8];
-    bf16x8 oh, ol;
-#pragma unroll
-    for (int i = 0; i < 8; ++i) {
-      o[i] = fmaf(v[j][i] * rstd, gg[i], bb[i]);
-      oh[i] = (bf16_t)o[i];
-      ol[i] = (bf16_t)(o[i] - (float)oh[i]);
-    }
-    *(bf16x8*)(yh + row * D + c) = oh;
-    *(bf16x8*)(yl + row * D + c) = ol;
-    if (yF) {
+#pragma unroll
+    for (int i = 0; i < 8; ++i) o[i] = fmaf(v[j][i] * rstd, gg[i], bb[i]);
+    if constexpr (PLANES) {
+      bf16x8 oh, ol;
+#pragma unroll
+      for (int i = 0; i < 8; ++i) {
+        oh[i] = (bf16_t)o[i];
+        ol[i] = (bf16_t)(o[i] - (float)oh[i]);
+      }
+      *(bf16x8*)(yh + row * D + c) = oh;
+      *(bf16x8*)(yl + row * D + c) = ol;
+    }
+    if (!PLANES || yF) {
       *(float4*)(yF + row * D + c) = float4{o[0], o[1], o[2], o[3]};
       *(float4*)(yF + row * D + c + 4) = float4{o[4], o[5], o[6], o[7]};
     }
+  }
+}
+template <int VPT>
+__device__ __forceinline__ void f32_row_to_hilo(float (&v)[VPT], float s, int lane, int64_t row, const float* gamma, const float* beta,
+                                                float eps, bf16_t* yh, bf16_t* yl) {
+  constexpr int D = 64 * VPT, NV = VPT / 4;
+  const float mean = wave_sum(s) * (1.f / D);
+  float q = 0.f;
+#pragma unroll
+  for (int i = 0; i < VPT; ++i) { v[i] -= mean; q = fmaf(v[i], v[i], q); }
+  const float rstd = rsqrtf(wave_sum(q) * (1.f / D) + eps);
+#pragma unroll
+  for (int j = 0; j < NV; ++j) {
+    const int c = (lane + 64 * j) * 4;
+    const float4 g = *(const float4*)(gamma + c), b = *(const float4*)(beta + c);
+    const float o[4] = {fmaf(v[4 * j] * rstd, g.x, b.x), fmaf(v[4 * j + 1] * rstd, g.y, b.y),
+                        fmaf(v[4 * j + 2] * rstd, g.z, b.z), fmaf(v[4 * j + 3] * rstd, g.w, b.w)};
+    bf16x4 oh, ol;
+#pragma unroll
+    for (int i = 0; i < 4; ++i) { oh[i] = (bf16_t)o[i]; ol[i] = (bf16_t)(o[i] - (float)oh[i]); }
+    *(bf16x4*)(yh + row * D + c) = oh;
+    *(bf16x4*)(yl + row * D + c) = ol;
   }
 }
 template <int VPT>
@@ -344,49 +371,87 @@
     v[4 * j] = t.x; v[4 * j + 1] = t.y; v[4 * j + 2] = t.z; v[4 * j + 3] = t.w;
     s += (t.x + t.y) + (t.z + t.w);
   }
-  const float mean = wave_sum(s) * (1.f / D);
-  float q = 0.f;
-#pragma unroll
-  for (int i = 0; i < VPT; ++i) { v[i] -= mean; q = fmaf(v[i], v[i], q); }
-  const float rstd = rsqrtf(wave_sum(q) * (1.f / D) + eps);
-#pragma unroll
-  for (int j = 0; j < NV; ++j) {
-    const int c = (lane + 64 * j) * 4;
-    const float4 g = *(const float4*)(gamma + c), b = *(const float4*)(beta + c);
-    const float o[4] = {fmaf(v[4 * j] * rstd, g.x, b.x), fmaf(v[4 * j + 1] * rstd, g.y, b.y),
-                        fmaf(v[4 * j + 2] * rstd, g.z, b.z), fmaf(v[4 * j + 3] * rstd, g.w, b.w)};
-    bf16x4 oh, ol;
-#pragma unroll
-    for (int i = 0; i < 4; ++i) { oh[i] = (bf16_t)o[i]; ol[i] = (bf16_t)(o[i] - (float)oh[i]); }
-    *(bf16x4*)(yh + row * D + c) = oh;
-    *(bf16x4*)(yl + row * D + c) = ol;
-  }
+  f32_row_to_hilo<VPT>(v, s, lane, row, gamma, beta, eps, yh, yl);
+}
+template <int VPT>
+__global__ __launch_bounds__(256) void posconv_add_ln_to_hilo_kernel(const float* h, const bf16_t* y, int B, int T, int G, int P, int Tq,
+                                                                     const float* gamma, const float* beta, float eps, bf16_t* yh, bf16_t* yl) {
+  constexpr int D = 64 * VPT, NV = VPT / 4;
+  const int lane = threadIdx.x & 63;
+  const int64_t row = (int64_t)blockIdx.x * 4 + (threadIdx.x >> 6);
+  if (row >= (int64_t)B * T) return;
+  const int cg = D / G;
+  const int t = (int)(row % T), b = (int)(row / T);
+  const int q = t / P, jf = t - q * P;
+  float v[VPT];
+  float s = 0.f;
+#pragma unroll
+  for (int j = 0; j < NV; ++j) {
+    const int ch = (lane + 64 * j) * 4;
+    const int g = ch / cg, c = ch - g * cg;
+    const bf16x4 yb = *(const bf16x4*)(y + (((int64_t)g * B + b) * Tq + q) * (P * cg) + jf * cg + c);
+    const float4 hv = ((const float4*)(h + row * D))[lane + 64 * j];
+    const float4 t4 = float4{hv.x + (float)yb[0], hv.y + (float)yb[1], hv.z + (float)yb[2], hv.w + (float)yb[3]};
+    v[4 * j] = t4.x; v[4 * j + 1] = t4.y; v[4 * j + 2] = t4.z; v[4 * j + 3] = t4.w;
+    s += (t4.x + t4.y) + (t4.z + t4.w);
+  }
+  f32_row_to_hilo<VPT>(v, s, lane, row, gamma, beta, eps, yh, yl);
 }
 }
 bool layernorm_hilo_ok(int D) { return D == 512 || D == 768 || D == 1024; }
+static bool hilo_outputs_ok(const bf16_t* yh, const bf16_t* yl, const float* yF, const float* x32) {
+  if ((yh == nullptr) != (yl == nullptr) || (!yh && (!yF || x32))) { set_error("layernorm (hi, lo): yh and yl together, or neither and an fp32 result"); return false; }
+  return true;
+}
 int launch_layernorm_hilo_parts(const float* parts, int nparts, long part_stride, const float* pbias, const bf16_t* rh, const bf16_t* rl, int64_t rows,
                                 int D, const float* gamma, const float* beta, float eps, bf16_t* yh, bf16_t* yl, float* yF, hipStream_t s) {
   if (!parts || nparts < 1 || !pbias || !(D == 512 || D == 768 || D == 1024) || (part_stride & 3) || !aligned(15, parts, pbias, rh, rl, yh, yl, yF, gamma, beta)) { set_error("layernorm (K-split branch): D in {512, 768, 1024} and 16-byte aligned buffers"); return -1; }
+  if (!hilo_outputs_ok(yh, yl, yF, nullptr)) return -1;
   const dim3 grid2((unsigned)((rows + 7) / 8)), block(256);
-  g_ln_kernel_id = 5001;
+  g_ln_kernel_id = yh ? 5001 : 5011;
   ln_width(D, [&](auto vpt) {
-    hipLaunchKernelGGL((layernorm_hilo2_kernel<64 * decltype(vpt)::value, true>), grid2, block, 0, s, nullptr, rh, rl, rows, gamma, beta, eps, yh, yl, yF, parts, nparts, part_stride, pbias);
+    constexpr int W = 64 * decltype(vpt)::value;
+    if (yh) hipLaunchKernelGGL((layernorm_hilo2_kernel<W, true>), grid2, block, 0, s, nullptr, rh, rl, rows, gamma, beta, eps, yh, yl, yF, parts, nparts, part_stride, pbias);
+    else hipLaunchKernelGGL((layernorm_hilo2_kernel<W, true, false>), grid2, block, 0, s, nullptr, rh, rl, rows, gamma, beta, eps, yh, yl, yF, parts, nparts, part_stride, pbias);
   });
   SVT_LAUNCH_CHECK();
   return 0;
 }
 int launch_layernorm_hilo(const bf16_t* branch, const bf16_t* rh, const bf16_t* rl, const float* x32, int64_t rows, int D,
                           const float* gamma, const float* beta, float eps, bf16_t* yh, bf16_t* yl, float* yF, hipStream_t s) {
+  if (!hilo_outputs_ok(yh, yl, yF, x32)) return -1;
   const dim3 grid((unsigned)((rows + 3) / 4)), grid2((unsigned)((rows + 7) / 8)), block(256);
-  g_ln_kernel_id = x32 ? 6000 : g_ln_two_rows && aligned(15, branch, rh, rl, yh, yl, yF, gamma, beta) ? 5000 : 4000;
+  const bool two = g_ln_two_rows && aligned(15, branch, rh, rl, yh, yl, yF, gamma, beta);
+  g_ln_kernel_id = x32 ? 6000 : (two ? 5000 : 4000) + (yh ? 0 : 10);
   ln_width(D, [&](auto vpt) {
     constexpr int VPT = decltype(vpt)::value;
     if (x32) hipLaunchKernelGGL((layernorm_f32_to_hilo_kernel<VPT>), grid, block, 0, s, x32, rows, gamma, beta, eps, yh, yl);
-    else if (g_ln_two_rows && aligned(15, branch, rh, rl, yh, yl, yF, gamma, beta)) hipLaunchKernelGGL((layernorm_hilo2_kernel<64 * VPT>), grid2, block, 0, s, branch, rh, rl, rows, gamma, beta, eps, yh, yl, yF);
-    else hipLaunchKernelGGL((layernorm_hilo_kernel<VPT>), grid, block, 0, s, branch, rh, rl, rows, gamma, beta, eps, yh, yl, yF);
+    else if (two && yh) hipLaunchKernelGGL((layernorm_hilo2_kernel<64 * VPT>), grid2, block, 0, s, branch, rh, rl, rows, gamma, beta, eps, yh, yl, yF);
+    else if (two) hipLaunchKernelGGL((layernorm_hilo2_kernel<64 * VPT, false, false>), grid2, block, 0, s, branch, rh, rl, rows, gamma, beta, eps, yh, yl, yF);
+    else if (yh) hipLaunchKernelGGL((layernorm_hilo_kernel<VPT>), grid, block, 0, s, branch, rh, rl, rows, gamma, beta, eps, yh, yl, yF);
+    else hipLaunchKernelGGL((layernorm_hilo_kernel<VPT, false>), grid, block, 0, s, branch, rh, rl, rows, gamma, beta, eps, yh, yl, yF);
   });
   SVT_LAUNCH_CHECK();
   return 0;
 }
 
-}
+int g_pos_ln_fused = 1;
+int launch_posconv_add_layernorm_hilo(const float* h, const bf16_t* y, int B, int T, int D, int G, int P, int Tq, float* pre,
+                                      const float* gamma, const float* beta, float eps, bf16_t* yh, bf16_t* yl, hipStream_t s) {
+  if (!layernorm_hilo_ok(D) || G < 1 || D % G || (D / G) % 8 || P < 1 || (int64_t)Tq * P < T || !aligned(15, h, y, pre, gamma, beta, yh, yl) || !yh || !yl) {
+    set_error("positional add + layernorm: D in {512, 768, 1024}, D / G a multiple of 8, Tq * P >= T and 16-byte aligned buffers"); return -1; }
+  const int64_t rows = (int64_t)B * T;
+  if (!g_pos_ln_fused) {
+    if (!pre) { set_error("positional add + layernorm: the two-kernel form needs the fp32 scratch"); return -1; }
+    if (int r = launch_posconv_scatter_add(h, y, B, T, D, G, P, Tq, pre, s, 0)) return r;
+    return launch_layernorm_hilo(nullptr, nullptr, nullptr, pre, rows, D, gamma, beta, eps, yh, yl, nullptr, s);
+  }
+  g_ln_kernel_id = 7000;
+  ln_width(D, [&](auto vpt) {
+    hipLaunchKernelGGL((posconv_add_ln_to_hilo_kernel<decltype(vpt)::value>), dim3((unsigned)((rows + 3) / 4)), dim3(256), 0, s, h, y, B, T, G, P, Tq, gamma, beta, eps, yh, yl);
+  });
+  SVT_LAUNCH_CHECK();
+  return 0;
+}
+
+}
diff --git a/svt_speechbrain_amd/csrc/stats.hip b/svt_speechbrain_amd/csrc/stats.hip
--- a/svt_speechbrain_amd/csrc/stats.hip
+++ b/svt_speechbrain_amd/csrc/stats.hip
@@ -30,16 +30,32 @@
 }
 
 namespace {
-__global__ __launch_bounds__(256) void moments_kernel(const float* x, int64_t n, double* mom, double* part, unsigned* ticket) {
+template <bool AHEAD>
+__device__ __forceinline__ void moments_body(const float* x, int64_t n, double* mom, double* part, unsigned* ticket, unsigned bx, unsigned by,
+                                             unsigned gx) {
   __shared__ double sh[2][4];
-  x += (int64_t)blockIdx.y * n;
-  mom += 2 * blockIdx.y;
-  part += (size_t)blockIdx.y * gridDim.x * 2;
+  x += (int64_t)by * n;
+  mom += 2 * by;
+  part += (size_t)by * gx * 2;
   double s = 0.0, ss = 0.0;
   const int64_t n4 = n >> 2;
   const float4* x4 = (const float4*)x;
-  int64_t i = (int64_t)blockIdx.x * blockDim.x + threadIdx.x;
-  const int64_t stride = (int64_t)gridDim.x * blockDim.x;
+  int64_t i = (int64_t)bx * 256 + threadIdx.x;
+  const int64_t stride = (int64_t)gx * 256;
+  if constexpr (AHEAD) {
+    for (; i + 3 * stride < n4; i += 4 * stride) {
+      float4 v[4];
+#pragma unroll
+      for (int u = 0; u < 4; ++u) v[u] = x4[i + u * stride];
+#pragma unroll
+      for (int u = 0; u < 4; ++u) {
+        const float a = (v[u].x + v[u].y) + (v[u].z + v[u].w);
+        const float b = (v[u].x * v[u].x + v[u].y * v[u].y) + (v[u].z * v[u].z + v[u].w * v[u].w);
+        s += (double)a;
+        ss += (double)b;
+      }
+    }
+  }
   for (; i < n4; i += stride) {
     const float4 v = x4[i];
     const float a = (v.x + v.y) + (v.z + v.w);
@@ -47,7 +63,7 @@
     s += (double)a;
     ss += (double)b;
   }
-  if (blockIdx.x == 0 && threadIdx.x == 0) {
+  if (bx == 0 && threadIdx.x == 0) {
     for (int64_t j = n4 << 2; j < n; ++j) { s += (double)x[j]; ss += (double)x[j] * (double)x[j]; }
   }
   s = wave_sum(s);
@@ -56,12 +72,12 @@
   if (lane == 0) { sh[0][wave] = s; sh[1][wave] = ss; }
   __syncthreads();
   if (threadIdx.x == 0) {
-    st_partial(part + blockIdx.x * 2, sh[0][0] + sh[0][1] + sh[0][2] + sh[0][3]);
-    st_partial(part + blockIdx.x * 2 + 1, sh[1][0] + sh[1][1] + sh[1][2] + sh[1][3]);
-  }
-  if (!last_workgroup(ticket + blockIdx.y, gridDim.x)) return;
+    st_partial(part + bx * 2, sh[0][0] + sh[0][1] + sh[0][2] + sh[0][3]);
+    st_partial(part + bx * 2 + 1, sh[1][0] + sh[1][1] + sh[1][2] + sh[1][3]);
+  }
+  if (!last_workgroup(ticket + by, gx)) return;
   s = 0.0; ss = 0.0;
-  for (unsigned b = threadIdx.x; b < gridDim.x; b += 256) { s += ld_partial(part + b * 2); ss += ld_partial(part + b * 2 + 1); }
+  for (unsigned b = threadIdx.x; b < gx; b += 256) { s += ld_partial(part + b * 2); ss += ld_partial(part + b * 2 + 1); }
   s = wave_sum(s);
   ss = wave_sum(ss);
   if (lane == 0) { sh[0][wave] = s; sh[1][wave] = ss; }
@@ -70,6 +86,9 @@
     mom[0] = sh[0][0] + sh[0][1] + sh[0][2] + sh[0][3];
     mom[1] = sh[1][0] + sh[1][1] + sh[1][2] + sh[1][3];
   }
+}
+__global__ __launch_bounds__(256) void moments_kernel(const float* x, int64_t n, double* mom, double* part, unsigned* ticket) {
+  moments_body<false>(x, n, mom, part, ticket, blockIdx.x, blockIdx.y, gridDim.x);
 }
 
 __global__ void global_norm_kernel(const float* x, float* y, int64_t n, const double* mom, float eps, double n_stat) {
@@ -122,16 +141,15 @@
 }
 
 namespace {
-__global__ __launch_bounds__(256) void conv0_window_moments_kernel(const float* wav, int64_t L, int stride, int64_t T1,
-                                                                   double* wm, double* part, unsigned* ticket) {
+__device__ __forceinline__ void window_moments_body(const float* wav, int64_t L, int stride, int64_t T1, double* wm, double* part,
+                                                    unsigned* ticket, unsigned bx, int b, unsigned gx) {
   __shared__ double sh[4][NWM];
-  const int b = blockIdx.y;
   const float* x = wav + (int64_t)b * L;
   double acc[NWM];
 #pragma unroll
   for (int i = 0; i < NWM; ++i) acc[i] = 0.0;
   constexpr int WPT = 8;
-  const int64_t t0 = ((int64_t)blockIdx.x * blockDim.x + threadIdx.x) * WPT;
+  const int64_t t0 = ((int64_t)bx * 256 + threadIdx.x) * WPT;
   for (int w = 0; w < WPT; ++w) {
     const int64_t t = t0 + w;
     if (t >= T1) break;
@@ -153,22 +171,36 @@
     if (lane == 0) sh[wave][i] = r;
   }
   __syncthreads();
-  part += (size_t)b * gridDim.x * NWM;
+  part += (size_t)b * gx * NWM;
   if (threadIdx.x < NWM)
-    st_partial(part + blockIdx.x * NWM + threadIdx.x, sh[0][threadIdx.x] + sh[1][threadIdx.x] + sh[2][threadIdx.x] + sh[3][threadIdx.x]);
-  if (!last_workgroup(ticket + b, gridDim.x)) return;
+    st_partial(part + bx * NWM + threadIdx.x, sh[0][threadIdx.x] + sh[1][threadIdx.x] + sh[2][threadIdx.x] + sh[3][threadIdx.x]);
+  if (!last_workgroup(ticket + b, gx)) return;
   if (threadIdx.x < NWM) {
     double t = 0.0;
     unsigned k = 0;
-    for (; k + 8 <= gridDim.x; k += 8) {
+    for (; k + 8 <= gx; k += 8) {
       double v[8];
 #pragma unroll
       for (int j = 0; j < 8; ++j) v[j] = ld_partial(part + (k + j) * NWM + threadIdx.x);
 #pragma unroll
       for (int j = 0; j < 8; ++j) t += v[j];
     }
-    for (; k < gridDim.x; ++k) t += ld_partial(part + k * NWM + threadIdx.x);
+    for (; k < gx; ++k) t += ld_partial(part + k * NWM + threadIdx.x);
     wm[b * NWM + threadIdx.x] = t;
+  }
+}
+__global__ __launch_bounds__(256) void conv0_window_moments_kernel(const float* wav, int64_t L, int stride, int64_t T1,
+                                                                   double* wm, double* part, unsigned* ticket) {
+  window_moments_body(wav, L, stride, T1, wm, part, ticket, blockIdx.x, blockIdx.y, gridDim.x);
+}
+__global__ __launch_bounds__(256) void waveform_stats_kernel(const float* wav, int64_t L, int stride, int64_t T1, double* wm, double* wpart,
+                                                             unsigned* wticket, unsigned win_gx, unsigned win_wgs, int64_t n, double* mom,
+                                                             double* mpart, unsigned* mticket, unsigned mom_gx) {
+  if (blockIdx.x < win_wgs) {
+    window_moments_body(wav, L, stride, T1, wm, wpart, wticket, blockIdx.x % win_gx, (int)(blockIdx.x / win_gx), win_gx);
+  } else {
+    const unsigned k = blockIdx.x - win_wgs;
+    moments_body<true>(wav, n, mom, mpart, mticket, k % mom_gx, k / mom_gx, mom_gx);
   }
 }
 
@@ -179,37 +211,10 @@
   if (wav_mom) wav_mom += 2 * (b / cpg);
   const int c = blockIdx.x * blockDim.x + threadIdx.x;
   if (c >= C) return;
-  double mu = 0.0, r = 1.0;
-  if (wav_mom) {
-    mu = wav_mom[0] / (double)n_wav;
-    const double var = wav_mom[1] / (double)n_wav - mu * mu;
-    r = 1.0 / sqrt(var + (double)eps_wav);
-  }
-  const double* m = wm + b * NWM;
-  const double invT = 1.0 / (double)T1;
-  double w[K0], mn[K0];
-  double wsum = 0.0;
-  for (int j = 0; j < K0; ++j) { w[j] = (double)w0[c * K0 + j]; wsum += w[j]; mn[j] = r * (m[j] * invT - mu); }
-  const double bias = b0 ? (double)b0[c] : 0.0;
-  double dot = 0.0;
-  for (int j = 0; j < K0; ++j) dot += w[j] * mn[j];
-  double quad = 0.0;
-  int idx = K0;
-  for (int j = 0; j < K0; ++j)
-    for (int j2 = j; j2 < K0; ++j2) {
-      const double R = r * r * (m[idx] * invT - mu * m[j] * invT - mu * m[j2] * invT + mu * mu);
-      quad += (j == j2 ? 1.0 : 2.0) * w[j] * w[j2] * R;
-      ++idx;
-    }
-  const double mean = dot + bias;
-  const double e2 = quad + 2.0 * bias * dot + bias * bias;
-  double var = e2 - mean * mean;
-  if (var < 0.0) var = 0.0;
-  const double a = (double)gamma[c] / sqrt(var + (double)eps_gn);
-  const double shift = (double)beta[c] - mean * a;
-  float* o = coef + ((int64_t)b * C + c) * (K0 + 1);
-  for (int j = 0; j < K0; ++j) o[j] = (float)(a * r * w[j]);
-  o[K0] = (float)(a * (bias - r * mu * wsum) + shift);
+  float o[K0 + 1];
+  conv0_group_coef_channel(wav_mom, n_wav, wm + b * NWM, T1, c, w0, b0, gamma, beta, eps_wav, eps_gn, o);
+  float* dst = coef + ((int64_t)b * C + c) * (K0 + 1);
+  for (int j = 0; j <= K0; ++j) dst[j] = o[j];
 }
 }
 size_t conv0_window_moments_scratch_bytes(int B, int64_t T1) {
@@ -226,6 +231,35 @@
   unsigned* ticket = (unsigned*)scratch;
   double* part = (double*)((char*)scratch + moments_ticket_bytes(B));
   hipLaunchKernelGGL(conv0_window_moments_kernel, grid, dim3(256), 0, s, wav, L, stride, T1, wm, part, ticket);
+  SVT_LAUNCH_CHECK();
+  return 0;
+}
+
+int launch_waveform_statistics(const float* wav, int B, int64_t L, int k, int stride, int64_t T1, double* wm, void* win_scratch, int64_t n,
+                               double* mom, void* mom_scratch, int groups_max, int groups, hipStream_t s) {
+  unsigned win_gx = 1, win_wgs = 0, mom_gx = 1, mom_wgs = 0;
+  unsigned *wticket = nullptr, *mticket = nullptr;
+  double *wpart = nullptr, *mpart = nullptr;
+  if (wm) {
+    if (k != K0) { set_error("conv layer 0 kernel size must be 10"); return -1; }
+    if (!win_scratch || ((uintptr_t)win_scratch & 7)) { set_error("conv0 window moments: scratch"); return -1; }
+    win_gx = (unsigned)((T1 + 2047) / 2048);
+    win_wgs = win_gx * (unsigned)B;
+    wticket = (unsigned*)win_scratch;
+    wpart = (double*)((char*)win_scratch + moments_ticket_bytes(B));
+  }
+  if (mom) {
+    if (groups > 1 && (n & 3)) { set_error("moments: per-group length must be a multiple of 4 elements"); return -1; }
+    if (groups > groups_max || !mom_scratch || ((uintptr_t)mom_scratch & 7)) { set_error("moments: scratch"); return -1; }
+    mom_gx = (unsigned)moments_grid(n, groups);
+    if (moments_ticket_bytes(groups_max) + (size_t)mom_gx * groups * 2 * sizeof(double) > moments_scratch_bytes(groups_max)) { set_error("moments: scratch too small"); return -1; }
+    mom_wgs = mom_gx * (unsigned)groups;
+    mticket = (unsigned*)mom_scratch;
+    mpart = (double*)((char*)mom_scratch + moments_ticket_bytes(groups_max));
+  }
+  if (!(win_wgs + mom_wgs)) return 0;
+  hipLaunchKernelGGL(waveform_stats_kernel, dim3(win_wgs + mom_wgs), dim3(256), 0, s, wav, L, stride, T1, wm, wpart, wticket, win_gx, win_wgs, n, mom,
+                     mpart, mticket, mom_gx);
   SVT_LAUNCH_CHECK();
   return 0;
 }
```

Result: no change. 6327 clips/s, median of 4 (+0.8%).
